# caomw/BundleAdjustmentMatlab

Hardware: AMD Instinct MI355X
Metric: LM iterations/sec + observations/sec, 1000-cam/500k-pt synthetic (higher is better)
Workload: dtype f64; 1 GPU; cfg3: 1000 cams x 500000 pts x 3000000 obs, fix_calibration (num_a=6), full LM pass per step, one linearisation per step; cameras=1000, points=500000, observations=3000000, parallelism=point-shard x1

## Files before the change

bundleadjustmentmatlab_amd/_lib.py:

```python
from __future__ import annotations

import ctypes
import os

_HERE = os.path.dirname(os.path.abspath(__file__))
LIB_PATH = os.environ.get("VLGBA_LIB") or os.path.join(_HERE, "libvlgba.so")

ABI_VERSION = 6

c_int, c_double, c_ll = ctypes.c_int, ctypes.c_double, ctypes.c_longlong
c_dp = ctypes.POINTER(ctypes.c_double)
c_ip = ctypes.POINTER(ctypes.c_int)
c_up = ctypes.POINTER(ctypes.c_ubyte)


class VlgbaProblem(ctypes.Structure):
    _fields_ = [("m", c_int), ("n", c_int), ("num_a", c_int), ("num_obs", c_ll),
                ("obs_pt", c_ip), ("obs_cam", c_ip), ("obs_x", c_dp), ("K", c_dp),
                ("num_vis", c_double), ("model", c_int)]


MODEL_EUCLIDEAN, MODEL_PROJECTIVE = 0, 1
LOSSES = {"none": 0, "huber": 1, "cauchy": 2}
JACOBIANS = {"fd": 0, "analytic": 1}
COV_METHODS = {"dense": 0, "selected": 1}


class VlgbaOptions(ctypes.Structure):
    _fields_ = [("fix_structure", c_int), ("fix_motion", c_int), ("pivot", c_up),
                ("verbose", c_int), ("max_iter", c_int), ("max_iter2", c_int),
                ("lambda0", c_double), ("device", c_int), ("rank", c_int),
                ("world_size", c_int), ("comm_id", ctypes.c_void_p), ("dense_solve", c_int),
                ("ordered", c_int), ("allreduce", ctypes.c_void_p),
                ("allreduce_user", ctypes.c_void_p), ("schur_kernel", c_int),
                ("semantics", c_int), ("stop_rel", c_double),
                ("on_pass", ctypes.c_void_p), ("on_pass_user", ctypes.c_void_p)]


NKERNELS = 18

ALLREDUCE_FN = ctypes.CFUNCTYPE(c_int, c_dp, c_ll, ctypes.c_void_p)


class VlgbaResectProblem(ctypes.Structure):
    _fields_ = [("nprob", c_int), ("num_a", c_int), ("obs_ptr", ctypes.POINTER(c_ll)),
                ("X", c_dp), ("x", c_dp), ("K", c_dp)]


class VlgbaStats(ctypes.Structure):
    _fields_ = [("iterations", c_int), ("accepted", c_int), ("num_error", c_int),
                ("lambda_", c_double), ("seconds", c_double), ("pinv_passes", c_int),
                ("spin_retries", c_int), ("nd_retries", c_int)]


class VlgbaStepInfo(ctypes.Structure):
    _fields_ = [("old_sse", c_double), ("new_sse", c_double), ("dpg", c_double),
                ("rho", c_double), ("lambda_", c_double), ("accepted", c_int),
                ("chol_failed", c_int), ("pinv", c_int), ("spin_retry", c_int),
                ("nd_retry", c_int)]


class VlgbaSceneSpec(ctypes.Structure):
    _fields_ = [("m", c_int), ("n", c_int), ("track", c_int), ("depth_lo", c_double),
                ("depth_hi", c_double), ("noise", c_double), ("seed", ctypes.c_ulonglong),
                ("keep_first_rotation", c_int), ("width", c_double), ("height", c_double)]


class VlgbaSceneOut(ctypes.Structure):
    _fields_ = [("K", c_dp), ("w", c_dp), ("T", c_dp), ("X", c_dp), ("w0", c_dp), ("T0", c_dp),
                ("X0", c_dp), ("obs_pt", c_ip), ("obs_cam", c_ip), ("obs_x", c_dp),
                ("num_obs_cap", c_ll), ("num_obs", c_ll), ("behind", c_ll)]


ON_PASS_FN = ctypes.CFUNCTYPE(None, c_int, c_int, ctypes.POINTER(VlgbaStepInfo), ctypes.c_void_p)


SIGNATURES = {
    "vlgba_solve": (c_int, [ctypes.POINTER(VlgbaProblem), ctypes.POINTER(VlgbaOptions), c_dp,
                            c_dp, c_dp, c_int, ctypes.POINTER(VlgbaStats)]),
    "vlgba_create": (c_int, [ctypes.POINTER(VlgbaProblem), ctypes.POINTER(VlgbaOptions),
                             ctypes.POINTER(ctypes.c_void_p)]),
    "vlgba_set_params": (c_int, [ctypes.c_void_p, c_dp, c_dp]),
    "vlgba_get_params": (c_int, [ctypes.c_void_p, c_dp, c_dp]),
    "vlgba_step": (c_int, [ctypes.c_void_p, c_int, c_int, ctypes.POINTER(VlgbaStepInfo)]),
    "vlgba_run": (c_int, [ctypes.c_void_p, c_dp, c_int, ctypes.POINTER(VlgbaStats)]),
    "vlgba_run_passes": (c_int, [ctypes.c_void_p, c_int, ctypes.POINTER(VlgbaStepInfo)]),
    "vlgba_get_step": (c_int, [ctypes.c_void_p, c_dp, c_dp]),
    "vlgba_get_reduced_system": (c_int, [ctypes.c_void_p, c_ip, c_dp, c_dp]),
    "vlgba_get_linearization": (c_int, [ctypes.c_void_p, c_dp, c_dp, c_dp, c_dp, c_dp]),
    "vlgba_covariance": (c_int, [ctypes.c_void_p, c_int, c_dp, c_dp, c_dp, c_dp]),
    "vlgba_set_loss": (c_int, [ctypes.c_void_p, c_int, c_double]),
    "vlgba_get_loss": (c_int, [ctypes.c_void_p, c_ip, c_dp]),
    "vlgba_set_covariance_method": (c_int, [ctypes.c_void_p, c_int]),
    "vlgba_get_covariance_method": (c_int, [ctypes.c_void_p, c_ip]),
    "vlgba_get_covariance_blocks": (c_int, [ctypes.c_void_p, c_ip, c_dp]),
    "vlgba_set_jacobian": (c_int, [ctypes.c_void_p, c_int]),
    "vlgba_get_jacobian": (c_int, [ctypes.c_void_p, c_ip]),
    "vlgba_get_residuals": (c_int, [ctypes.c_void_p, c_dp, c_dp, c_dp]),
    "vlgba_sync": (c_int, [ctypes.c_void_p]),
    "vlgba_destroy": (None, [ctypes.c_void_p]),
    "vlgba_set_timing": (c_int, [ctypes.c_void_p, c_int]),
    "vlgba_phase_ms": (c_int, [ctypes.c_void_p, c_dp]),
    "vlgba_kernel_ms": (c_int, [ctypes.c_void_p, c_dp, ctypes.POINTER(c_ll), c_int]),
    "vlgba_kernel_name": (ctypes.c_char_p, [c_int]),
    "vlgba_kernel_flops": (c_int, [ctypes.c_void_p, c_dp]),
    "vlgba_plan_info": (c_int, [ctypes.c_void_p, ctypes.POINTER(c_ll), c_int]),
    "vlgba_mex_bundle_1": (c_int, [c_int, c_int, c_int] + [c_dp] * 14),
    "vlgba_mex_bundle_2": (c_int, [c_int, c_int, c_int] + [c_dp] * 7),
    "vlgba_mex_bundle_3": (c_int, [c_int, c_int, c_int] + [c_dp] * 13),
    "vlgba_mex_bundle_proj_1": (c_int, [c_int, c_int] + [c_dp] * 13),
    "vlgba_mex_bundle_proj_2": (c_int, [c_int, c_int] + [c_dp] * 7),
    "vlgba_mex_bundle_proj_3": (c_int, [c_int, c_int] + [c_dp] * 12),
    "vlgba_resect": (c_int, [ctypes.POINTER(VlgbaResectProblem), ctypes.POINTER(VlgbaOptions),
                             c_dp, c_dp, c_int, c_ip, ctypes.POINTER(VlgbaStats)]),
    "vlgba_triangulate": (c_int, [c_int, c_dp, c_dp, c_dp, c_ll, ctypes.POINTER(c_ll), c_ip, c_dp,
                                  c_int, c_dp, c_ip]),
    "vlgba_intersect": (c_int, [c_int, c_dp, c_dp, c_dp, c_ll, ctypes.POINTER(c_ll), c_ip, c_dp,
                                ctypes.POINTER(VlgbaOptions), c_dp, c_dp, c_int, c_ip,
                                ctypes.POINTER(VlgbaStats)]),
    "vlgba_resect_ex": (c_int, [ctypes.POINTER(VlgbaResectProblem), ctypes.POINTER(VlgbaOptions),
                                c_int, c_int, c_double, c_dp, c_dp, c_int, c_ip, c_dp, c_dp,
                                ctypes.POINTER(VlgbaStats)]),
    "vlgba_intersect_ex": (c_int, [c_int, c_dp, c_dp, c_dp, c_dp, c_ll, ctypes.POINTER(c_ll), c_ip,
                                   c_dp, ctypes.POINTER(VlgbaOptions), c_int, c_int, c_double,
                                   c_dp, c_dp, c_int, c_ip, c_dp, c_dp,
                                   ctypes.POINTER(VlgbaStats)]),
    "vlgba_triangulate_ex": (c_int, [c_int, c_dp, c_dp, c_dp, c_dp, c_ll, ctypes.POINTER(c_ll),
                                     c_ip, c_dp, c_int, c_dp, c_ip]),
    "vlgba_scene_banded": (c_int, [ctypes.POINTER(VlgbaSceneSpec), c_int,
                                   ctypes.POINTER(VlgbaSceneOut)]),
    "vlgba_version": (c_int, [ctypes.c_char_p, c_int]),
    "vlgba_abi_check": (c_int, [c_int, c_ll, c_ll, c_ll, c_ll, c_ll]),
    "vlgba_get_unique_id": (c_int, [ctypes.c_void_p]),
    "vlgba_comm_release": (c_int, [ctypes.c_void_p]),
    "vlgba_device_count": (c_int, []),
    "vlgba_debug_sincos": (c_int, [c_dp, c_dp, c_dp, c_ll]),
    "vlgba_debug_pinv_solve": (c_int, [c_int, c_dp, c_dp, c_dp]),
    "vlgba_debug_force_status": (c_int, [ctypes.c_void_p, c_int, c_int]),
    "vlgba_debug_nd_plan": (c_int, [c_int, c_int, c_ip, c_int, c_ip, c_ip]),
    "vlgba_debug_selinv_plan": (c_int, [c_int, c_ip, c_ip, c_ip]),
    "vlgba_debug_pcg_plan": (c_int, [c_int, c_ip, c_int, c_ip, c_ip]),
    "vlgba_set_pcg": (c_int, [ctypes.c_void_p, c_double, c_int]),
    "vlgba_get_pcg": (c_int, [ctypes.c_void_p, c_dp, c_ip]),
    "vlgba_get_pcg_stats": (c_int, [ctypes.c_void_p, c_ip, c_dp, c_ip, ctypes.POINTER(c_ll)]),
}

ERRORS = {-1001: "bad argument",
          -1002: "num_a must be 6, 7, 9 or 10 (Euclidean) or 12 (projective)",
          -1003: "duplicate (point, camera) observation", -1004: "out of host memory",
          -1005: "RCCL communicator failure",
          -1006: "library / header ABI mismatch",
          -1007: "the undamped reduced camera system is not positive definite (gauge not fixed)"}

_lib = None


class VlgbaError(RuntimeError):
    pass


def lib():
    global _lib
    if _lib is None:
        if not os.path.exists(LIB_PATH):
            raise VlgbaError(f"{LIB_PATH} not built: run __graft_entry__.build() or "
                             "make -C bundleadjustmentmatlab_amd/csrc")
        L = ctypes.CDLL(LIB_PATH)
        for name, (res, args) in SIGNATURES.items():
            if os.environ.get("VLGBA_LIB") and not hasattr(L, name):
                continue
            fn = getattr(L, name)
            fn.restype = res
            fn.argtypes = args
        if hasattr(L, "vlgba_abi_check") or not os.environ.get("VLGBA_LIB"):
            rc = L.vlgba_abi_check(ABI_VERSION, *(ctypes.sizeof(s) for s in (
                VlgbaProblem, VlgbaOptions, VlgbaStats, VlgbaStepInfo, VlgbaResectProblem)))
            if rc != 0:
                raise VlgbaError(f"{LIB_PATH} does not match this binding (ABI {ABI_VERSION}): "
                                 "rebuild it with __graft_entry__.build()")
        _lib = L
    return _lib


def check(rc: int, what: str = "vlgba"):
    if rc != 0:
        msg = ERRORS.get(rc, f"HIP error {-rc}" if -1000 < rc < 0 else f"code {rc}")
        raise VlgbaError(f"{what} failed: {msg} ({rc})")
```

bundleadjustmentmatlab_amd/bundle.py:

```python
from __future__ import annotations

import ctypes
import numpy as np

from ._lib import (ALLREDUCE_FN, COV_METHODS, JACOBIANS, LOSSES, MODEL_EUCLIDEAN, MODEL_PROJECTIVE, NKERNELS, ON_PASS_FN,
                   VlgbaOptions,
                   VlgbaProblem, VlgbaResectProblem, VlgbaStats,
                   VlgbaStepInfo, c_dp, c_ip, c_up, check, lib)

__all__ = ["bundle_euclid", "bundle_euclid_nomex", "bundle_euclid_obs", "BundleAdjuster",
           "bundle_euclid_resect", "bundle_euclid_intersect", "triangulate_points",
           "parse_options", "pivot_mask",
           "mex_bundle_1_XABeUVWeAeB", "mex_bundle_2_Se_", "mex_bundle_3_db_new"]


def _F(a):
    return np.asfortranarray(a, dtype=np.float64)


def _dp(a):
    return a.ctypes.data_as(c_dp)


def pivot_mask(pivot, m):
# ... 269 lines not shown
            pass

    def __enter__(self):
        return self

    def __exit__(self, *exc):
        self.close()

    def set_params(self, a, b):
        a = np.ascontiguousarray(_F(a).reshape(-1, order="F"))
        b = np.ascontiguousarray(_F(b).reshape(-1, order="F"))
        assert a.size == self.num_a * self.m and b.size == 3 * self.n
        check(self._L.vlgba_set_params(self._h, _dp(a), _dp(b)), "vlgba_set_params")

    def get_params(self):
        a = np.zeros(self.num_a * self.m)
        b = np.zeros(3 * self.n)
        check(self._L.vlgba_get_params(self._h, _dp(a), _dp(b)), "vlgba_get_params")
        return a.reshape(self.num_a, self.m, order="F"), b.reshape(3, self.n, order="F")

    def force_status(self, word, passes=1):
        check(self._L.vlgba_debug_force_status(self._h, int(word), int(passes)),
              "vlgba_debug_force_status")

    def step(self, relinearize=True, update_lm=True):
        info = VlgbaStepInfo()
        check(self._L.vlgba_step(self._h, int(relinearize), int(update_lm), ctypes.byref(info)),
              "vlgba_step")
        return info

    def passes(self, n):
        info = VlgbaStepInfo()
        check(self._L.vlgba_run_passes(self._h, int(n), ctypes.byref(info)), "vlgba_run_passes")
        return info

    def run(self):
        err = np.zeros(self.max_iter + 1)
        st = VlgbaStats()
        check(self._L.vlgba_run(self._h, _dp(err), err.size, ctypes.byref(st)), "vlgba_run")
        assert st.num_error <= err.size
        return err[: st.num_error].copy(), st

    def last_step(self):
        da = np.zeros(self.num_a * self.m)
        db = np.zeros(3 * self.n)
        check(self._L.vlgba_get_step(self._h, _dp(da), _dp(db)), "vlgba_get_step")
        return da.reshape(self.num_a, self.m, order="F"), db.reshape(3, self.n, order="F")

    def reduced_system(self, dense=True):
        nb = self.plan_info()["blocks"]
        na = self.num_a
        jk = np.zeros(2 * nb, dtype=np.int32)
        blocks = np.zeros(na * na * nb)
        e_ = np.zeros(na * self.m)
        check(self._L.vlgba_get_reduced_system(self._h, jk.ctypes.data_as(c_ip), _dp(blocks),
                                               _dp(e_)), "vlgba_get_reduced_system")
        jk = jk.reshape(nb, 2)
        blocks = blocks.reshape(nb, na, na).transpose(0, 2, 1)
        if not dense:
            return jk, blocks, e_
        S = np.zeros((na * self.m, na * self.m))
        for (j, k), B in zip(jk, blocks):
            if j == k:
                S[na * j:na * j + na, na * k:na * k + na] = np.tril(B)
            else:
                S[na * j:na * j + na, na * k:na * k + na] = B
        return S, e_

    def set_covariance_method(self, method="dense"):
        if method not in COV_METHODS:
            raise ValueError(f"method must be one of {sorted(COV_METHODS)}")
        check(self._L.vlgba_set_covariance_method(self._h, COV_METHODS[method]),
              "vlgba_set_covariance_method")

    def get_covariance_method(self):
        kind = ctypes.c_int()
        check(self._L.vlgba_get_covariance_method(self._h, ctypes.byref(kind)),
              "vlgba_get_covariance_method")
        return {v: k for k, v in COV_METHODS.items()}[kind.value]

    def covariance(self, scale=True, full=False, method=None, blocks=False):
        if method is not None and method not in COV_METHODS:
            raise ValueError(f"method must be one of {sorted(COV_METHODS)}")
        prev = None
        if method is not None and method != self.get_covariance_method():
            prev = self.get_covariance_method()
            self.set_covariance_method(method)
        try:
            na, ld = self.num_a, self.num_a * self.m
            cam = np.zeros((na, na, self.m), order="F")
            pts = np.zeros((3, 3, self.n), order="F")
            S = np.zeros((ld, ld), order="F") if full else None
            info = np.zeros(8)
            check(self._L.vlgba_covariance(self._h, int(bool(scale)), _dp(cam),
                                           _dp(S) if full else None, _dp(pts), _dp(info)),
                  "vlgba_covariance")
            out = dict(cam=cam, pts=pts, sse=float(info[0]), dof=float(info[1]),
                       sigma2=float(info[2]), fixed_rows=int(info[3]),
                       ms=(float(info[4]), float(info[5])), scratch_bytes=int(info[6]))
            if full:
                out["full"] = S
            if blocks:
                nb = self.plan_info()["blocks"]
                jk = np.zeros(2 * nb, dtype=np.int32)
                blk = np.zeros(na * na * nb)
                check(self._L.vlgba_get_covariance_blocks(self._h, jk.ctypes.data_as(c_ip),
                                                          _dp(blk)),
                      "vlgba_get_covariance_blocks")
                out["blk_jk"] = jk.reshape(nb, 2)
                out["blocks"] = blk.reshape(nb, na, na).transpose(0, 2, 1)
            return out
        finally:
            if prev is not None:
                self.set_covariance_method(prev)

    def sync(self):
        check(self._L.vlgba_sync(self._h), "vlgba_sync")

    def linearization(self):
        na, m, n, N = self.num_a, self.m, self.n, self.num_obs
        U = np.zeros((na, na, m), order="F")
        eA = np.zeros((na, m), order="F")
        V = np.zeros((3, 3, n), order="F")
        eB = np.zeros((3, n), order="F")
        W = np.zeros((na, 3, N), order="F")
        check(self._L.vlgba_get_linearization(self._h, _dp(U), _dp(eA), _dp(V), _dp(eB),
                                              _dp(W)), "vlgba_get_linearization")
        return dict(U=U, eA=eA, V=V, eB=eB, W=W)

    def set_timing(self, on=True):
        check(self._L.vlgba_set_timing(self._h, int(on)), "vlgba_set_timing")

    def kernel_ms(self, reset=True):
        n = NKERNELS
        ms = np.zeros(n)
        calls = (ctypes.c_longlong * n)()
        check(self._L.vlgba_kernel_ms(self._h, _dp(ms), calls, int(reset)), "vlgba_kernel_ms")
        return {self._L.vlgba_kernel_name(k).decode(): (float(ms[k]), int(calls[k]))
                for k in range(n) if calls[k] > 0}

    PLAN_KEYS = ("obs", "points", "cameras", "num_a", "chunks", "chunk_slots",
                 "chunk_eslots", "groups", "group_slots", "group_eslots", "blocks",
                 "tiles", "cr_levels", "cr_elim", "cr_keep", "ordered", "schur_terms",
                 "blob_words", "mfma", "cr_rows", "mfma_groups", "reordered", "long_points",
                 "nd_arcs", "nd_sep_tiles", "solve_flops_factor", "solve_flops_syrk",
                 "solve_flops_back", "env_runner_runs", "vinv_fold", "camupd_fold", "pcg",
                 "solve_bytes")

    def plan_info(self):
        n = len(self.PLAN_KEYS)
        buf = (ctypes.c_longlong * n)()
        rc = self._L.vlgba_plan_info(self._h, buf, n)
        check(min(rc, 0), "vlgba_plan_info")
        return dict(zip(self.PLAN_KEYS, [int(v) for v in buf]))

    def phase_ms(self):
        ms = np.zeros(7)
        check(self._L.vlgba_phase_ms(self._h, _dp(ms)), "vlgba_phase_ms")
        return dict(zip(["linearize", "camera_reduce", "damp_y", "schur", "assemble",
                         "cholesky_solve", "update"], ms.tolist()))


def euclid_obs_adjuster(K, m, n, obs_pt, obs_cam, obs_x, *varargin, num_vis=0.0, device=0,
                        rank=0, world_size=1, comm_id=None, semantics="mex", loss="none",
                        loss_scale=0.0, jacobian=None, radial=False, **solver):
    o = parse_options(m, n, varargin, nomex=semantics == "nomex")
    if radial:
        o["num_variableK"] = RADIAL_NVK
    ba = BundleAdjuster(K, obs_pt, obs_cam, obs_x, n, 6 + o["num_variableK"],
                        fix_structure=o["fix_structure"], fix_motion=o["fix_motion"],
                        pivot=o["pivot"] if o["fix_pivot"] else None, verbose=o["verbose"],
                        num_vis=num_vis, device=device, rank=rank, world_size=world_size,
                        comm_id=comm_id, semantics=semantics, loss=loss, loss_scale=loss_scale,
                        jacobian=jacobian, **solver)
    ba.fingerprint = _adjuster_fingerprint(K, m, n, obs_pt, obs_cam, obs_x, o, num_vis,
                                           semantics, rank, world_size, device, comm_id,
                                           loss, loss_scale, ba.get_jacobian())
    return ba


def _adjuster_fingerprint(K, m, n, obs_pt, obs_cam, obs_x, o, num_vis, semantics, rank,
                          world_size, device, comm_id, loss="none", loss_scale=0.0,
                          jacobian="fd"):
    try:
        import xxhash
        h = xxhash.xxh3_128()
    except ImportError:
        import hashlib
        h = hashlib.blake2b(digest_size=16)
    for arr, dt in ((obs_pt, np.int32), (obs_cam, np.int32), (obs_x, np.float64),
                    (K, np.float64)):
        h.update(memoryview(np.ascontiguousarray(arr, dtype=dt)).cast("B"))
    piv = o["pivot"] if o["fix_pivot"] else None
    if piv is not None:
        h.update(np.asarray(piv, dtype=bool).tobytes())
    if comm_id is not None:
        h.update(bytes(comm_id))
    return (int(m), int(n), int(o["num_variableK"]), bool(o["fix_structure"]),
            bool(o["fix_motion"]), bool(o["fix_pivot"]), bool(o["verbose"]), float(num_vis),
            semantics, int(rank), int(world_size), int(device), comm_id is not None,
            h.hexdigest(), str(loss), float(loss_scale) if loss != "none" else 0.0,
            str(jacobian))


def bundle_euclid_obs(K, Te, w, Xe, obs_pt, obs_cam, obs_x, *varargin, num_vis=0.0, device=0,
                      rank=0, world_size=1, comm_id=None, return_stats=False,
                      semantics="mex", adjuster=None, return_covariance=False, loss="none",
                      loss_scale=0.0, jacobian=None, covariance_method=None, radial=None,
                      **solver):
    K, Te, w, Xe = _F(K), _F(Te), _F(w), _F(Xe)
    m, n = w.shape[1], Xe.shape[1]
    nomex = semantics == "nomex"
    o = parse_options(m, n, varargin, nomex=nomex)
    if radial is not None:
        if jacobian == "fd":
            raise ValueError("radial distortion has analytic Jacobians only")
        o["num_variableK"] = RADIAL_NVK
    nvk = o["num_variableK"]
    a = pack_a(K, Te, w, nvk, radial)
    b = _F(Xe[0:3])
    if adjuster is not None:
        if solver:
            raise ValueError("bundle_euclid_obs: solver options belong to the prebuilt adjuster")
        ba = adjuster.result() if hasattr(adjuster, "result") else adjuster
        want = _adjuster_fingerprint(K, m, n, obs_pt, obs_cam, obs_x, o, num_vis, semantics,
                                     rank, world_size, device, comm_id, loss, loss_scale,
                                     jacobian if jacobian is not None else
                                     ba.get_jacobian())
        if getattr(ba, "fingerprint", None) != want:
            ba.close()
            raise ValueError("bundle_euclid_obs: the prebuilt adjuster is for another problem "
                             "or other options (make it with euclid_obs_adjuster)")
    else:
        ba = euclid_obs_adjuster(K, m, n, obs_pt, obs_cam, obs_x, *varargin, num_vis=num_vis,
                                 device=device, rank=rank, world_size=world_size,
                                 comm_id=comm_id, semantics=semantics, loss=loss,
                                 loss_scale=loss_scale, jacobian=jacobian,
                                 radial=radial is not None, **solver)
    with ba:
        ba.set_params(a, b)
        err, st = ba.run()
        a, b = ba.get_params()
        if return_covariance:
            ba.set_params(a, b)
            cov = ba.covariance(scale=loss == "none", method=covariance_method)
    out = unpack(K, a, b, np.ones((1, n)) if nomex else Xe[3:4], nvk) + (err,)
    out = out + (st,) if return_stats else out
    out = out + (cov,) if return_covariance else out
    return out + (a[7:9].copy(order="F"),) if radial is not None else out


def bundle_euclid(K, Te, w, Xe, x, *varargin, device=0, return_stats=False, semantics="mex",
                  return_covariance=False, loss="none", loss_scale=0.0, covariance_method=None,
                  **solver):
    x = _F(x)
    m, n = np.shape(w)[1], x.shape[1]
    o = parse_options(m, n, varargin, x=x, nomex=semantics == "nomex")
    vis = o["visible"]
    num_vis = float(vis.sum())
    pt, cam = np.nonzero(vis)
    obs_x = np.stack([x[0, pt, cam], x[1, pt, cam]], axis=1)
    rest, k = [], 0
    while k < len(varargin):
        nm = varargin[k].lower() if isinstance(varargin[k], str) else varargin[k]
        if nm == "visibility":
            k += 2
            continue
        if nm == "fix_pivot":
            rest += [varargin[k], varargin[k + 1]]
            k += 2
            continue
        rest.append(varargin[k])
        k += 1
    return bundle_euclid_obs(K, Te, w, Xe, pt, cam, obs_x, *rest, num_vis=num_vis,
                             device=device, return_stats=return_stats, semantics=semantics,
                             return_covariance=return_covariance, loss=loss,
                             loss_scale=loss_scale, covariance_method=covariance_method,
                             **solver)


def bundle_euclid_nomex(K, Te, w, Xe, x, *varargin, device=0, return_stats=False,
                        return_covariance=False, loss="none", loss_scale=0.0,
                        covariance_method=None, **solver):
    return bundle_euclid(K, Te, w, Xe, x, *varargin, device=device,
                         return_stats=return_stats, semantics="nomex",
                         return_covariance=return_covariance, loss=loss,
                         loss_scale=loss_scale, covariance_method=covariance_method, **solver)


def _block_mode(radial, jacobian, loss, loss_scale, return_residuals):
    if jacobian is None:
        jacobian = "fd" if radial is None else "analytic"
    if jacobian not in JACOBIANS:
        raise ValueError(f"jacobian must be one of {sorted(JACOBIANS)}, got {jacobian!r}")
    if loss not in LOSSES:
        raise ValueError(f"loss must be one of {sorted(LOSSES)}, got {loss!r}")
    ex = radial is not None or jacobian != "fd" or loss != "none" or bool(return_residuals)
    return ex, JACOBIANS[jacobian], LOSSES[loss], float(loss_scale)


def _block_solve(name, head, head_ex, mode, x, count, N, residuals, return_stats, device,
                 max_iter, max_iter2, lambda0, stop_rel):
    ex, jac, lk, ls = mode
    cap = (max_iter if max_iter > 0 else 20) + 1
    err = np.zeros((count, cap))
    nerr = np.zeros(count, dtype=np.int32)
    opt = VlgbaOptions()
# ... 146 lines not shown
```

bundleadjustmentmatlab_amd/csrc/ba_internal.h:

```cpp
#pragma once
#include <hip/hip_runtime.h>
#include <cstddef>
#include <cstdint>
#include "ba_limits.h"

struct ba_chol;
struct ba_pcg;

#define VLGBA_CHECK(x)                                                              \
    do {                                                                            \
        hipError_t err__ = (x);                                                     \
        if (err__ != hipSuccess) return -(int)err__;                                \
    } while (0)

enum {
    KT_ROT, KT_LIN, KT_CAMRED, KT_DAMP, KT_SCHUR, KT_SCHUR_CHUNK, KT_SCHUR_RED,
    KT_ASSEMBLE, KT_FACTOR, KT_SYRK, KT_BACKWARD, KT_CAMUPD, KT_PTUPD, KT_CR_FACTOR,
    KT_CR_UPDATE, KT_CR_BACK, KT_SCHUR_MF, KT_LIN_UPD, KT_N
};
#define KT_MAX_EV 8192
struct ba_ktimer {
    int on;
    int nev;
    int ncreated;
    hipEvent_t ev[KT_MAX_EV];
    int kid[KT_MAX_EV / 2];
    double ms[KT_N];
    long long calls[KT_N];
    double flops[KT_N];
};
void kt_begin(struct ba_ktimer *t, hipStream_t s);
void kt_end(struct ba_ktimer *t, hipStream_t s, int kid);

#define BA_PROJ_NA 12
#define BA_RAD_NA 9

struct ba_flags {
    int fix_structure;
    int fix_motion;
    int has_pivot;
};

struct ba_loss {
    int kind;
    double c;
};

struct ba_camred {
    const int *cam_eptr, *cam_eslots;
    const double *upart;
    int m;
    ba_flags f;
    const unsigned char *pivot;
    double *U, *eA;
    const double *chsse;
    int nch;
    double *sse_out, *sse_out2;
};

struct ba_dev {
    int m, n, na, N, js;
    int device, ncu;
    int *obs_cam, *pt_ptr, *cam_ptr, *cam_obs;
    double *obs_x, *K4;
    unsigned char *pivot;
    double *a, *b, *a_new, *b_new;
    double *rot, *rot_new;
    double *jrec, *W, *U, *eA, *V, *eB;
    double *Vinv, *Y, *t, *db;
    int nb;
    long long T;
    int *blk_jk, *blk_ptr, *term;
    double *sblk, *rhs, *da;
    long long ld;
    long long lds;
    ba_chol *chol;
    ba_pcg *pcg;
    int dense_solve;
    int asm_direct;
    int camupd_fold;
    double *part;
    double *scal;
    int ordered;
    int parity;
    int mfma;
    int no_mfma;
    int loss_kind;
    double loss_scale;
    int jac;
    int ndb;
    int nch;
    int *ch_pt;
    int *ch_eslot;
    int *eslot_optr;
    unsigned short *eslot_obs;
    int *cam_eptr, *cam_eslots;
    double *spart;
    double *epart;
    double *upart;
    double *chsse;
    int fused;
    double *W2, *V2, *eB2, *upart2, *chsse2;
    int ns, nes;
    int ch_max_terms, ch_max_slots;
    long long nterm_fast;
    long long blob_words;
    int ngrp, ngs, nge;
    int grp_max_s, grp_max_e;
    unsigned *blob;
    int *ch_blob, *ch_obase;
    int *ch_cam;
    unsigned char *obs_lpt;
    int max_blob;
    int ngrp_mf;
    int vinv_fold;
    int nch_reg, nl, p_long;
    int *seg_pt, *seg_long;
    int *long_pt, *long_o0, *long_seg0;
    int *long_ebase;
    int *cam_lptr, *cam_lobs, *cam_ltrk;
    int max_lcam;
    int long_o0_h;
    double *ylong;
    int *lpair_ptr;
    int2 *lpair;
    int *lblk;
    int nlb;
    double *vseg;
    double *dpg_long;
    int mf_max_s, mf_max_e, mf_max_blob;
    int *grp_ch, *grp_gs, *grp_ge;
    unsigned short *cs_g, *ce_g;
    int *blk_gptr, *blk_gslots;
    int *cam_gptr, *cam_gslots;
    double *xh_out;
    double *B_out;
    unsigned char *obs_vis;
    int schur_owner;
    int dpg_lambda;
    struct ba_ktimer *kt;
    hipStream_t stream;
    hipStream_t side;
    hipEvent_t ev_fork, ev_join;
    volatile double *hres;
    double *hres_dev;
    unsigned long long seq;
    unsigned *pub_cnt;
};

#define KT_B(d) \
    do { if ((d)->kt && (d)->kt->on) kt_begin((d)->kt, (d)->stream); } while (0)
#define KT_E(d, id) \
    do { if ((d)->kt && (d)->kt->on) kt_end((d)->kt, (d)->stream, (id)); } while (0)

#define BA_PART_MAX 65536

#define BA_DISPATCH(NAEXPR, CALL)                                                   \
    switch (NAEXPR) {                                                               \
    case 6: { constexpr int NA = 6; CALL; } break;                                  \
    case 7: { constexpr int NA = 7; CALL; } break;                                  \
    case BA_RAD_NA: { constexpr int NA = BA_RAD_NA; CALL; } break;                  \
    case 10: { constexpr int NA = 10; CALL; } break;                                \
    case BA_PROJ_NA: { constexpr int NA = BA_PROJ_NA; CALL; } break;                \
    default: return -1000;                                                          \
    }

int ba_launch_rotations(ba_dev *d, const double *a, double *rot);
int ba_launch_linearize(ba_dev *d, ba_flags f);
ba_camred ba_camred_args(const ba_dev *d, ba_flags f);
int ba_launch_camera_reduce(ba_dev *d, ba_flags f, hipStream_t s);
int ba_launch_damp_point(ba_dev *d, double lambda);
int ba_launch_schur(ba_dev *d, double lambda);
int ba_launch_assemble(ba_dev *d);
int ba_launch_update(ba_dev *d, double lambda, ba_flags f, bool cam_updated, bool publish,
                     bool *published);
int ba_launch_yeb(ba_dev *d);
int ba_launch_obs_residuals(ba_dev *d, double *e, double *w, double *rho);
int ba_launch_publish(ba_dev *d);
void *ba_dmalloc(size_t bytes);
int ba_ensure_dyn_lds(const void *fn, size_t bytes);
void ba_dfree(void *p);
template <typename T>
inline int dalloc(T **p, size_t count)
{
    *p = (T *)ba_dmalloc(sizeof(T) * (count ? count : 1));
    return *p ? 0 : -(int)hipErrorOutOfMemory;
}
template <typename T>
inline int upload(T *dst, const T *src, size_t count, hipStream_t s)
{
    if (count == 0) return 0;
    return -(int)hipMemcpyAsync(dst, src, sizeof(T) * count, hipMemcpyHostToDevice, s);
}
template <typename T>
inline int download(T *dst, const T *src, size_t count, hipStream_t s)
{
    if (count == 0) return 0;
    return -(int)hipMemcpyAsync(dst, src, sizeof(T) * count, hipMemcpyDeviceToHost, s);
}
template <typename T>
class ba_dbuf {
    T *p_ = nullptr;

public:
    ba_dbuf() = default;
    ba_dbuf(ba_dbuf &&o) noexcept : p_(o.p_) { o.p_ = nullptr; }
    ba_dbuf &operator=(ba_dbuf &&o) noexcept
    {
        if (this != &o) {
            ba_dfree(p_);
            p_ = o.p_;
            o.p_ = nullptr;
        }
        return *this;
    }
    ba_dbuf(const ba_dbuf &) = delete;
    ba_dbuf &operator=(const ba_dbuf &) = delete;
    ~ba_dbuf() { ba_dfree(p_); }
    int alloc(size_t count)
    {
        ba_dfree(p_);
        return dalloc(&p_, count);
    }
    T *get() const { return p_; }
    operator T *() const { return p_; }
};
int ba_env_runner_timed_out(ba_dev *d);
int ba_launch_schur_fast(ba_dev *d, double lambda, const ba_camred *fold, bool side_camred);
int ba_launch_long_pairs(ba_dev *d, int fill, int *cnt);
int ba_launch_assemble_plain(ba_dev *d, double *S, long long ld, int lower_only);
int ba_launch_parity_old_sse(ba_dev *d);
int ba_launch_parity_new_sums(ba_dev *d, double lambda);
int ba_chol_setup(ba_dev *d, const int *blk_jk_host, int nb);
void ba_chol_free(ba_dev *d);
int ba_chol_prepare(ba_dev *d);
int ba_assemble_tiles(ba_dev *d);
int ba_fix_diag_plain(ba_dev *d, double *S, long long ld);
int ba_chol_fix_diag(ba_dev *d);
int ba_chol_solve(ba_dev *d, bool *cam_updated, int nospin = 0);
int ba_cr32_factor(ba_dev *d);
int ba_cr32_selinv_sources(const ba_dev *d, int *src);
int ba_cr32_selinv(ba_dev *d, const int *src, double *sig);
int ba_pinv_apply(ba_dev *d, const double *V, const double *ev, long long ld, const double *rhs,
                  double *work, double *da);

int ba_pcg_setup(ba_dev *d, const int *blk_jk_host, int nb);
void ba_pcg_free(ba_dev *d);
int ba_pcg_solve(ba_dev *d);

#define BA_COV_T8 8
#define BA_COV_T64 32
#define BA_COV_LDS 65536
int ba_cov_mark_fixed(ba_dev *d, const double *S, long long ld, unsigned char *fixed);
int ba_cov_finish(ba_dev *d, double *S, long long ld, const unsigned char *fixed, double *blocks);
struct ba_cov_src {
    const double *Sa;
    long long ld;
    const int *rowptr, *col;
    const double *packed;
};
int ba_cov_pack(ba_dev *d, const double *S, long long ld, const int *bj, const int *bk, int nb,
                double *packed);
int ba_cov_mark_fixed_blocks(ba_dev *d, unsigned char *fixed);
int ba_cov_extract(ba_dev *d, const double *sig, const unsigned char *fixed, const int *bj,
// ... 10 lines not shown
```

bundleadjustmentmatlab_amd/csrc/ba_kernels.hip:

```cpp
#include "ba_internal.h"
#include "ba_chol.h"
#include "ba_camera.h"
#include "vlg_math.h"
#include "../../include/vlgba.h"

typedef double d4 __attribute__((ext_vector_type(4)));

#ifdef BA_STAMPS
__device__ unsigned long long g_stamp[32];
#define STAMP_DECL unsigned long long st_prev_ = __builtin_amdgcn_s_memtime()
#define STAMP(i)                                                                    \
    do {                                                                            \
        if (threadIdx.x == 0) {                                                     \
            const unsigned long long t_ = __builtin_amdgcn_s_memtime();             \
            atomicAdd(&g_stamp[i], t_ - st_prev_);                                  \
            st_prev_ = t_;                                                          \
        }                                                                           \
    } while (0)
extern "C" int vlgba_debug_stamps(unsigned long long *out, int reset)
{
    if (hipMemcpyFromSymbol(out, HIP_SYMBOL(g_stamp), sizeof(g_stamp)) != hipSuccess) return -1;
    if (reset) {
        unsigned long long z[32] = {};
        if (hipMemcpyToSymbol(HIP_SYMBOL(g_stamp), z, sizeof(z)) != hipSuccess) return -1;
    }
    return 0;
}
#define BA_MFST_WG 4096
__device__ unsigned long long g_mfst[BA_MFST_WG * 4 * 8];
#define MF_CLK(v)                                                                   \
    do {                                                                            \
        __builtin_amdgcn_sched_barrier(0);                                          \
        v = __builtin_amdgcn_s_memtime();                                           \
        __builtin_amdgcn_sched_barrier(0);                                          \
    } while (0)
extern "C" int vlgba_debug_mf_stamps(unsigned long long *out, int nwords)
{
    const size_t nb = sizeof(unsigned long long) * (size_t)nwords;
    if (nb > sizeof(g_mfst)) return -1;
    if (hipMemcpyFromSymbol(out, HIP_SYMBOL(g_mfst), nb) != hipSuccess) return -1;
    return 0;
}
#else
#define STAMP_DECL
#define STAMP(i)
#define MF_CLK(v)
#endif

typedef double v2d __attribute__((ext_vector_type(2)));

template <int BS>
__device__ __forceinline__ void block_sum_to(double v, double *out)
{
    __shared__ double red[BS / 64];
#pragma unroll
    for (int off = 32; off > 0; off >>= 1) v += __shfl_down(v, off, 64);
    const int lane = threadIdx.x & 63, wid = threadIdx.x >> 6;
    if (lane == 0) red[wid] = v;
    __syncthreads();
    if (threadIdx.x == 0) {
        double s = red[0];
#pragma unroll
        for (int k = 1; k < BS / 64; k++) s += red[k];
        *out = s;
    }
}


__device__ __forceinline__ void fd_columns_6(const cam_view<6> &cv, const double b[3],
                                             const double xh[2], int half, double *row)
{
    const double *t0 = cv.a0 + 3;
#pragma unroll
    for (int t = 0; t < 3; t++) {
        const double *Rs = cv.R + 9 * (half ? 0 : 1 + t);
        double Rk[9], tt[3], bb[3], x1[2], S[3];
#pragma unroll
        for (int q = 0; q < 9; q++) Rk[q] = Rs[q];
#pragma unroll
        for (int c = 0; c < 3; c++) {
            tt[c] = half ? t0[c] : t0[c] + H_FD * 0.0;
            bb[c] = half ? b[c] + H_FD * ((c == t) ? 1.0 : 0.0) : b[c];
        }
        vlg_rot_b(Rk, bb, S);
        vlg_project_s(cv.Kc, S, tt, x1);
        const int col = half ? 6 + t : t;
        row[2 * col] = vlg_fd_quot(x1[0] - xh[0]);
        row[2 * col + 1] = vlg_fd_quot(x1[1] - xh[1]);
    }
    double S[3], R4[9];
    const double *Rs4 = cv.R + 36;
#pragma unroll
    for (int q = 0; q < 9; q++) R4[q] = Rs4[q];
    vlg_rot_b(R4, b, S);
#pragma unroll
    for (int u = 0; u < 2; u++) {
        const int k = 3 + 2 * u + half;
        if (k < 6) {
            double tt[3], x1[2];
#pragma unroll
            for (int c = 0; c < 3; c++) tt[c] = t0[c] + H_FD * ((3 + c == k) ? 1.0 : 0.0);
            vlg_project_s(cv.Kc, S, tt, x1);
            row[2 * k] = vlg_fd_quot(x1[0] - xh[0]);
            row[2 * k + 1] = vlg_fd_quot(x1[1] - xh[1]);
        }
    }
}

template <int NA>
__global__ void k_rotations(const double *__restrict__ a, double *__restrict__ rot, int m)
{
    const int j = blockIdx.x * blockDim.x + threadIdx.x;
    if (j >= m) return;
    const double *aj = a + (size_t)NA * j;
    const double w[3] = {aj[0], aj[1], aj[2]};
    rotations5(w, rot + 45 * (size_t)j);
}

template <int NA>
__global__ void k_rotations_jac(const double *__restrict__ a, double *__restrict__ rot, int m)
{
    const int j = blockIdx.x * blockDim.x + threadIdx.x;
    if (j >= m) return;
    const double *aj = a + (size_t)NA * j;
    const double w[3] = {aj[0], aj[1], aj[2]};
    rotations5_jac(w, rot + 45 * (size_t)j);
}

__global__ void k_sincos(const double *__restrict__ x, double *__restrict__ s,
                         double *__restrict__ c, long long n)
{
    const long long i = (long long)blockIdx.x * blockDim.x + threadIdx.x;
    if (i >= n) return;
    const double v = x[i];
    s[i] = vlg_lm_sin(v);
    c[i] = vlg_lm_cos(v);
}

extern "C" int vlgba_debug_sincos(const double *x, double *s, double *c, long long n)
{
    if (n < 0 || (n > 0 && (!x || !s || !c))) return VLGBA_E_ARG;
    if (n == 0) return 0;
    double *d = nullptr;
    VLGBA_CHECK(hipMalloc(&d, sizeof(double) * 3 * (size_t)n));
    int rc = 0;
    do {
        if (hipMemcpy(d, x, sizeof(double) * n, hipMemcpyHostToDevice) != hipSuccess) { rc = -1; break; }
        const long long nb = (n + 255) / 256;
        hipLaunchKernelGGL(k_sincos, dim3((unsigned)nb), dim3(256), 0, 0, d, d + n, d + 2 * n, n);
        if (hipGetLastError() != hipSuccess) { rc = -1; break; }
        if (hipMemcpy(s, d + n, sizeof(double) * n, hipMemcpyDeviceToHost) != hipSuccess ||
            hipMemcpy(c, d + 2 * n, sizeof(double) * n, hipMemcpyDeviceToHost) != hipSuccess)
            rc = -1;
    } while (0);
    (void)hipFree(d);
    return rc;
}

template <int NA>
__global__ __launch_bounds__(256) void k_linearize(
    const int *__restrict__ pt_ptr, const int *__restrict__ obs_cam,
    const double *__restrict__ obs_x, const double *__restrict__ K4,
    const double *__restrict__ a, const double *__restrict__ rot,
    const double *__restrict__ b, int n, ba_flags f, const unsigned char *__restrict__ pivot,
    double *__restrict__ jrec, double *__restrict__ W, double *__restrict__ V,
    double *__restrict__ eB, double *__restrict__ part_sse, double *__restrict__ xh_out,
    double *__restrict__ B_out)
{
    constexpr int JS = 2 * NA + 2;
    double sse = 0.0;
    for (int i = blockIdx.x * blockDim.x + threadIdx.x; i < n; i += gridDim.x * blockDim.x) {
        const double bi[3] = {b[3 * (size_t)i], b[3 * (size_t)i + 1], b[3 * (size_t)i + 2]};
        double v[9], eb[3];
#pragma unroll
        for (int q = 0; q < 9; q++) v[q] = 0.0;
        eb[0] = eb[1] = eb[2] = 0.0;
        const int o_end = pt_ptr[i + 1];
        for (int o = pt_ptr[i]; o < o_end; o++) {
            const int j = obs_cam[o];
            cam_view<NA> cv(a, K4, rot, j);
            double xh[2];
            cv.project(bi, xh);
            double A[2 * NA], B[6];
#pragma unroll
            for (int k = 0; k < NA; k++) {
                double x1[2];
                cv.project_dcam(k, bi, x1);
                A[2 * k] = vlg_fd_quot(x1[0] - xh[0]);
                A[2 * k + 1] = vlg_fd_quot(x1[1] - xh[1]);
            }
#pragma unroll
            for (int k = 0; k < 3; k++) {
                double b1[3], x1[2];
#pragma unroll
                for (int c = 0; c < 3; c++) b1[c] = bi[c] + H_FD * ((c == k) ? 1.0 : 0.0);
                cv.project(b1, x1);
                B[2 * k] = vlg_fd_quot(x1[0] - xh[0]);
                B[2 * k + 1] = vlg_fd_quot(x1[1] - xh[1]);
            }
            const double e0 = obs_x[2 * (size_t)o] - xh[0];
            const double e1 = obs_x[2 * (size_t)o + 1] - xh[1];
            double *rec = jrec + (size_t)JS * o;
#pragma unroll
            for (int q = 0; q < 2 * NA; q += 2) {
                double2 p = {A[q], A[q + 1]};
                *reinterpret_cast<double2 *>(rec + q) = p;
            }
            *reinterpret_cast<double2 *>(rec + 2 * NA) = double2{e0, e1};
            if (xh_out) {
                xh_out[2 * (size_t)o] = xh[0];
                xh_out[2 * (size_t)o + 1] = xh[1];
            }
            if (B_out) {
#pragma unroll
                for (int q = 0; q < 6; q++) B_out[6 * (size_t)o + q] = B[q];
            }
            const bool wzero = f.fix_structure || f.fix_motion || (f.has_pivot && pivot[j]);
            double *wo = W + (size_t)3 * NA * o;
#pragma unroll
            for (int c = 0; c < 3; c++)
#pragma unroll
                for (int r = 0; r < NA; r++)
                    wo[r + NA * c] =
                        wzero ? 0.0 : 0.0 + (A[2 * r] * B[2 * c] + A[2 * r + 1] * B[2 * c + 1]);
#pragma unroll
            for (int c = 0; c < 3; c++)
#pragma unroll
                for (int r = 0; r < 3; r++)
                    v[r + 3 * c] += B[2 * r] * B[2 * c] + B[2 * r + 1] * B[2 * c + 1];
#pragma unroll
            for (int r = 0; r < 3; r++) eb[r] += B[2 * r] * e0 + B[2 * r + 1] * e1;
            sse += e0 * e0 + e1 * e1;
        }
        if (f.fix_structure) {
#pragma unroll
            for (int q = 0; q < 9; q++) v[q] = 0.0;
            eb[0] = eb[1] = eb[2] = 0.0;
        }
#pragma unroll
        for (int q = 0; q < 9; q++) V[9 * (size_t)i + q] = v[q];
#pragma unroll
        for (int q = 0; q < 3; q++) eB[3 * (size_t)i + q] = eb[q];
    }
    block_sum_to<256>(sse, part_sse + blockIdx.x);
}

#define BA_LIN_CAMS 10
#define BA_LIN_WAVES (BA_LIN_CAMS > 0 ? 6 : 7)

struct ba_upd {
    const double *W_old, *da, *eB_old, *Vinv, *b_old;
    int ndb;
    double lambda;
    double *db, *b_new, *part_dpg;
    const int *seg_long, *long_o0;
    const double *dpg_long;
};

template <int NA, bool UPD, bool LOSS, bool JAC = false>
__device__ __forceinline__ void linearize_chunk_body(
    const int *__restrict__ ch_pt, const int *__restrict__ ch_obase,
    const int *__restrict__ ch_eslot, const int *__restrict__ eslot_optr,
    const unsigned short *__restrict__ eslot_obs, const int *__restrict__ pt_ptr,
    const int *__restrict__ obs_cam, const unsigned char *__restrict__ obs_lpt,
    const double *__restrict__ obs_x, const double *__restrict__ K4,
    const double *__restrict__ a, const double *__restrict__ rot,
    const double *__restrict__ b, ba_flags f, const unsigned char *__restrict__ pivot,
    double *__restrict__ W, double *__restrict__ V, double *__restrict__ eB,
    double *__restrict__ upart, double *__restrict__ part_sse, int nch_reg,
    const int *__restrict__ seg_pt, double *__restrict__ vseg, const int *__restrict__ ch_cam,
    ba_upd u, int ch, ba_loss ls)
{
    constexpr int NC0 = (NA + 4) / 2;
    static_assert(!LOSS || 2 * BA_CH_OBS >= 256, "one lane pair per LDS row");
    constexpr int RS = 2 * NA + 8;
    constexpr int NU = NA * (NA + 1) / 2;
    static_assert(BA_CH_OBS + 1 <= 256 && BA_CH_PTS + 1 <= 256, "one metadata word per lane");
    constexpr int LW = BA_CH_OBS * 3 * NA;
    constexpr int NROWS = (UPD && LW + 3 * BA_CH_PTS > BA_CH_OBS * RS) ? LW + 3 * BA_CH_PTS
                                                                        : BA_CH_OBS * RS;
    static_assert(NA != 6 || NROWS == BA_CH_OBS * RS, "fused update must not grow NA = 6 LDS");
    __shared__ __attribute__((aligned(16))) double rows[NROWS];
    __shared__ int lptr_raw[64 * (BA_CH_PTS / 64 + 1)];
    __shared__ int eoff_raw[64 * (BA_CH_OBS / 64 + 1)];
    __shared__ unsigned short eobl[BA_CH_OBS];
    __shared__ unsigned char wz[BA_CH_OBS];
    __shared__ double dpl[UPD ? BA_CH_PTS : 1];
    static_assert(BA_CH_PTS <= 64, "the point lanes are wave 0");
    constexpr int NCAMS = (NA == 6 && BA_LIN_CAMS > 0) ? BA_LIN_CAMS : 0;
    __shared__ __attribute__((aligned(16))) double camr[NCAMS > 0 ? 45 * NCAMS : 1];
    const int tid = threadIdx.x;
    const bool seg = ch >= nch_reg;
    const int p0 = seg ? seg_pt[ch - nch_reg] : ch_pt[ch];
    const int np = seg ? 1 : ch_pt[ch + 1] - p0;
    const int obase = ch_obase[ch], nobs = ch_obase[ch + 1] - obase;
    const int e0 = ch_eslot[ch], nes = ch_eslot[ch + 1] - e0;
    STAMP_DECL;
    const int u0 = eslot_optr[e0], nu = eslot_optr[e0 + nes] - u0;
    {
        const int wv = tid >> 6;
        if (wv <= (nes >> 6))
            __builtin_amdgcn_global_load_lds(eslot_optr + e0 + min(tid, nes), eoff_raw + 64 * wv,
                                             4, 0, 0);
        if (!seg && wv <= (np >> 6))
            __builtin_amdgcn_global_load_lds(pt_ptr + p0 + min(tid, np), lptr_raw + 64 * wv, 4, 0,
                                             0);
    }
    const int cam_lo = ch_cam[2 * ch], cam_n = ch_cam[2 * ch + 1] - cam_lo + 1;
    const bool camst = NCAMS > 0 && nobs > 0 && cam_n <= NCAMS;
    if (NCAMS > 0 && camst) {
#if defined(__HIP_DEVICE_COMPILE__)
        const int lane = tid & 63;
        auto stage = [&](const double *src, int ndw, double *dst) {
            const char *s8 = reinterpret_cast<const char *>(src);
            for (int q = tid >> 6; 64 * q < ndw; q += 4)
                if (64 * q + lane < ndw)
                    __builtin_amdgcn_global_load_lds(s8 + 4 * (64 * q + lane),
                                                     reinterpret_cast<int *>(dst) + 64 * q, 4, 0,
                                                     0);
        };
        stage(rot + 45 * (size_t)cam_lo, 90 * cam_n, &camr[0]);
#endif
        if constexpr (!UPD) __syncthreads();
    }
    int m_eobl = 0;
    STAMP(16);
    double bu[3] = {0.0, 0.0, 0.0};
    if constexpr (UPD) {
        if (seg) {
            if (tid == 0)
                dpl[0] = obase == u.long_o0[u.seg_long[ch - nch_reg]]
                             ? __hip_atomic_load(u.dpg_long + u.seg_long[ch - nch_reg],
                                                 __ATOMIC_RELAXED, __HIP_MEMORY_SCOPE_AGENT)
                             : 0.0;
        } else {
            const int ne = nobs * 3 * NA;
            const double *wsrc = u.W_old + (size_t)3 * NA * obase;
            double dl[NA];
            const int ocam = nobs > 0 ? obs_cam[obase + min(tid, nobs - 1)] : 0;
            const int clo = cam_lo, span = cam_n;
            const bool dstage = NA == 6 && span * NA <= NROWS - LW;
            if (dstage && nobs > 0) {
#if defined(__HIP_DEVICE_COMPILE__)
                const int nb = 8 * NA * span;
                if ((tid >> 6) < ((nb + 1023) >> 10))
                    __builtin_amdgcn_global_load_lds(
                        reinterpret_cast<const char *>(u.da + (size_t)NA * clo) +
                            min((tid >> 6) * 1024 + 16 * (tid & 63), nb - 16),
                        &rows[LW + 128 * (tid >> 6)], 16, 0, 0);
#endif
            }
            if (nobs > 0) {
                if constexpr (NA == 6) {
#if defined(__HIP_DEVICE_COMPILE__)
                    const int nbytes = 8 * ne, ninst = (nbytes + 1023) >> 10;
                    const char *src = reinterpret_cast<const char *>(wsrc);
                    for (int q = tid >> 6; q < ninst; q += 4)
                        __builtin_amdgcn_global_load_lds(
                            src + min(q * 1024 + 16 * (tid & 63), nbytes - 16), &rows[128 * q],
                            16, 0, 2);
#endif
                } else {
                    constexpr int MAXE = (LW + 255) / 256;
#pragma unroll
                    for (int q = 0; q < MAXE; q++) {
                        const int e = tid + 256 * q;
                        if (e < ne) rows[e] = __builtin_nontemporal_load(wsrc + e);
                    }
                }
                if (!dstage) {
                    const double *dd = u.da + (size_t)NA * ocam;
#pragma unroll
                    for (int k = 0; k < NA; k++) dl[k] = dd[k];
                }
            }
            const int ip = np > 0 ? p0 + min(tid, np - 1) : 0;
            double pe[3] = {0.0, 0.0, 0.0}, pv[9] = {}, pb[3] = {0.0, 0.0, 0.0};
            if (__builtin_amdgcn_readfirstlane(tid >> 6) == 0) {
#pragma unroll
                for (int r = 0; r < 3; r++) pe[r] = u.eB_old[3 * (size_t)ip + r];
#pragma unroll
                for (int r = 0; r < 9; r++) pv[r] = u.Vinv[9 * (size_t)ip + r];
#pragma unroll
                for (int r = 0; r < 3; r++) pb[r] = u.b_old[3 * (size_t)ip + r];
            }
            __syncthreads();
            if (tid < nobs) {
                double *wo = rows + 3 * NA * tid;
                if (dstage) {
#pragma unroll
                    for (int k = 0; k < NA; k++) dl[k] = rows[LW + NA * (ocam - clo) + k];
                }
#pragma unroll
                for (int k = 0; k < NA; k++)
                    if (k >= u.ndb) dl[k] = 0.0;
#pragma unroll
                for (int r = 0; r < 3; r++) {
                    double *w = wo + NA * r;
                    double t = w[0] * dl[0] + w[1] * dl[1] + w[2] * dl[2] + w[3] * dl[3] +
                               w[4] * dl[4] + w[5] * dl[5];
#pragma unroll
                    for (int k = 6; k < NA; k++)
                        if (k < u.ndb) t = t + w[k] * dl[k];
                    w[0] = t;
                }
            }
            __syncthreads();
            if (tid < np) {
                const int i = p0 + tid;
                double rhs[3] = {pe[0], pe[1], pe[2]};
                const int lo1 = lptr_raw[tid + 1] - obase;
                for (int lo = lptr_raw[tid] - obase; lo < lo1; lo++) {
#pragma unroll
                    for (int r = 0; r < 3; r++) rhs[r] -= rows[3 * NA * lo + NA * r];
                }
                double dpg = 0.0;
#pragma unroll
                for (int r = 0; r < 3; r++) {
                    const double dbr = pv[r] * rhs[0] + pv[r + 3] * rhs[1] + pv[r + 6] * rhs[2];
                    const double bnr = pb[r] + dbr;
                    u.db[3 * (size_t)i + r] = dbr;
                    u.b_new[3 * (size_t)i + r] = bnr;
                    rows[LW + 3 * tid + r] = bnr;
                    dpg += dbr * (u.lambda * dbr + pe[r]);
                }
                dpl[tid] = dpg;
            }
        }
        __syncthreads();
        if (!seg && nobs > 0) {
            const int lp = obs_lpt[obase + min(min(tid >> 1, BA_CH_OBS - 1), nobs - 1)];
#pragma unroll
            for (int c = 0; c < 3; c++) bu[c] = rows[LW + 3 * lp + c];
        } else if (nobs > 0) {
#pragma unroll
            for (int c = 0; c < 3; c++) bu[c] = b[3 * (size_t)p0 + c];
        }
        __syncthreads();
        STAMP(23);
    }
    double sse = 0.0;
    if (nobs > 0) {
        m_eobl = __hip_atomic_load(eslot_obs + u0 + min(tid, nu - 1), __ATOMIC_RELAXED,
                                   __HIP_MEMORY_SCOPE_WORKGROUP);
        const int lo = min(tid >> 1, BA_CH_OBS - 1), half = tid & 1;
        const bool live = (tid >> 1) < nobs;
        {
            const int o = obase + min(lo, nobs - 1);
            const int j = obs_cam[o], i = p0 + obs_lpt[o];
            double bi[3];
#pragma unroll
            for (int c = 0; c < 3; c++) bi[c] = UPD ? bu[c] : b[3 * (size_t)i + c];
            double xh[2];
            double *row = rows + RS * lo;
            if constexpr (JAC && NA == 6) {
                auto proj6 = [&](const double *rt, int jr) {
                    cam_view<NA> cv6(a, K4, rt, jr, j);
                    cv6.project(bi, xh);
                    cv6.jac_columns(bi, half, row);
                };
                if (NCAMS > 0 && camst)
                    proj6(&camr[0], j - cam_lo);
                else
                    proj6(rot, j);
            } else if constexpr (JAC) {
                cam_view<NA> cv(a, K4, rot, j);
                cv.project(bi, xh);
                cv.jac_columns(bi, half, row);
            } else if constexpr (NA == 6) {
                auto proj6 = [&](const double *rt, int jr) {
                    cam_view<NA> cv6(a, K4, rt, jr, j);
                    cv6.project(bi, xh);
                    fd_columns_6(cv6, bi, xh, half, row);
                };
                if (NCAMS > 0 && camst)
                    proj6(&camr[0], j - cam_lo);
                else
                    proj6(rot, j);
            } else {
                cam_view<NA> cv(a, K4, rot, j);
                cv.project(bi, xh);
#pragma unroll 1
                for (int t = 0; t < NC0; t++) {
                    const int col = half ? NC0 + t : t;
                    if (col < NA + 3) {
                        double x1[2];
                        cv.project_col(col, bi, x1);
                        row[2 * col] = vlg_fd_quot(x1[0] - xh[0]);
                        row[2 * col + 1] = vlg_fd_quot(x1[1] - xh[1]);
                    }
                }
            }
            if constexpr (LOSS) {
                const double e0 = obs_x[2 * (size_t)o] - xh[0];
                const double e1 = obs_x[2 * (size_t)o + 1] - xh[1];
                double rho, sw;
                vlg_loss(ls.kind, ls.c, e0 * e0 + e1 * e1, &rho, &sw);
#pragma unroll
                for (int col = 0; col < NA + 3; col++) {
                    const bool lane1 = JAC      ? cam_view<NA>::jac_lane1(col)
                                       : NA == 6 ? (col == 4 || col > 5)
                                                 : col >= NC0;
                    if (lane1 == (half != 0)) {
                        row[2 * col] *= sw;
                        row[2 * col + 1] *= sw;
                    }
                }
                if (!half) {
                    row[2 * NA + 6] = e0 * sw;
                    row[2 * NA + 7] = e1 * sw;
                    if (live) sse = rho;
                    wz[lo] = f.fix_structure || f.fix_motion || (f.has_pivot && pivot[j]);
                }
            } else if (!half) {
                const double e0 = obs_x[2 * (size_t)o] - xh[0];
                const double e1 = obs_x[2 * (size_t)o + 1] - xh[1];
                row[2 * NA + 6] = e0;
                row[2 * NA + 7] = e1;
                if (live) sse = e0 * e0 + e1 * e1;
                wz[lo] = f.fix_structure || f.fix_motion || (f.has_pivot && pivot[j]);
            }
        }
    }
    if (tid < nu) eobl[tid] = (unsigned short)m_eobl;
    __syncthreads();
    STAMP(17);
    if constexpr (UPD) {
        if (tid == 0) {
            double acc = 0.0;
            const int k1 = seg ? 1 : np;
            for (int k = 0; k < k1; k++) acc += dpl[k];
            u.part_dpg[ch] = acc;
        }
    }
    if constexpr (NA % 2 == 0) {
        double2 *wdst = reinterpret_cast<double2 *>(W + (size_t)3 * NA * obase);
        constexpr int NP = 3 * NA / 2;
        for (int q = tid; q < nobs * NP; q += 256) {
            const int lo = q / NP, e = q - NP * lo, c = e / (NA / 2), r = 2 * (e - (NA / 2) * c);
            const double *row = rows + RS * lo;
            const double2 a0 = *reinterpret_cast<const double2 *>(row + 2 * r);
            const double2 a1 = *reinterpret_cast<const double2 *>(row + 2 * r + 2);
            const double2 bc = *reinterpret_cast<const double2 *>(row + 2 * NA + 2 * c);
            const long long keep = wz[lo] ? 0 : -1;
            const double v0 = 0.0 + (a0.x * bc.x + a0.y * bc.y);
            const double v1 = 0.0 + (a1.x * bc.x + a1.y * bc.y);
            const v2d w2 = {__builtin_bit_cast(double, __builtin_bit_cast(long long, v0) & keep),
                            __builtin_bit_cast(double, __builtin_bit_cast(long long, v1) & keep)};
            __builtin_nontemporal_store(w2, reinterpret_cast<v2d *>(wdst) + q);
        }
    } else {
        double *wdst = W + (size_t)3 * NA * obase;
        for (int q = tid; q < nobs * 3 * NA; q += 256) {
            const int lo = q / (3 * NA), e = q - 3 * NA * lo, c = e / NA, r = e - NA * c;
            const double *row = rows + RS * lo;
            const double2 ar = *reinterpret_cast<const double2 *>(row + 2 * r);
            const double2 bc = *reinterpret_cast<const double2 *>(row + 2 * NA + 2 * c);
            wdst[q] = wz[lo] ? 0.0 : 0.0 + (ar.x * bc.x + ar.y * bc.y);
        }
    }
    STAMP(18);
    for (int q = tid; q < np * 12; q += 256) {
        const int pl = q / 12, e = q % 12, i = p0 + pl;
        const int lo0 = seg ? 0 : lptr_raw[pl] - obase;
        const int lo1 = seg ? nobs : lptr_raw[pl + 1] - obase;
        const int r = (e < 9) ? e % 3 : e - 9, c = (e < 9) ? e / 3 : 3;
        double acc = 0.0;
        for (int lo = lo0; lo < lo1; lo++) {
            const double *B = rows + RS * lo + 2 * NA;
            acc += B[2 * r] * B[2 * c] + B[2 * r + 1] * B[2 * c + 1];
        }
        if (f.fix_structure) acc = 0.0;
        if (seg) vseg[12 * (size_t)(ch - nch_reg) + e] = acc;
        else if (e < 9) V[9 * (size_t)i + e] = acc;
        else eB[3 * (size_t)i + e - 9] = acc;
    }
    STAMP(19);
    for (int q = tid; q < nes * (NU + NA); q += 256) {
        const int s = q / (NU + NA), l = q % (NU + NA);
        int r, c;
        if (l < NU) {
            int t = l;
            c = 0;
            while (t >= NA - c) { t -= NA - c; c++; }
            r = c + t;
        } else {
            r = l - NU;
            c = NA;
        }
        const int cc = (c < NA) ? 2 * c : 2 * NA + 6;
        double acc = 0.0;
        int u = eoff_raw[s] - u0;
        const int u1 = eoff_raw[s + 1] - u0;
        for (; u + 3 < u1; u += 4) {
            double p[4];
#pragma unroll
            for (int k = 0; k < 4; k++) {
                const double *rw = rows + RS * eobl[u + k];
                p[k] = rw[2 * r] * rw[cc] + rw[2 * r + 1] * rw[cc + 1];
            }
#pragma unroll
            for (int k = 0; k < 4; k++) acc += p[k];
        }
        for (; u < u1; u++) {
            const double *row = rows + RS * eobl[u];
            acc += row[2 * r] * row[cc] + row[2 * r + 1] * row[cc + 1];
        }
        upart[(size_t)(NU + NA) * (e0 + s) + l] = acc;
    }
    STAMP(20);
    block_sum_to<256>(sse, part_sse + ch);
    STAMP(21);
#ifdef BA_STAMPS
    if (tid == 0) atomicAdd(&g_stamp[22], 1ull);
#endif
}

#define BA_LIN_ARGS                                                                        \
    const int *__restrict__ ch_pt, const int *__restrict__ ch_obase,                       \
        const int *__restrict__ ch_eslot, const int *__restrict__ eslot_optr,              \
        const unsigned short *__restrict__ eslot_obs, const int *__restrict__ pt_ptr,      \
        const int *__restrict__ obs_cam, const unsigned char *__restrict__ obs_lpt,        \
        const double *__restrict__ obs_x, const double *__restrict__ K4,                   \
        const double *__restrict__ a, const double *__restrict__ rot,                      \
        const double *__restrict__ b, ba_flags f, const unsigned char *__restrict__ pivot, \
        double *__restrict__ W, double *__restrict__ V, double *__restrict__ eB,           \
        double *__restrict__ upart, double *__restrict__ part_sse, int nch_reg,            \
        const int *__restrict__ seg_pt, double *__restrict__ vseg,                         \
        const int *__restrict__ ch_cam
#define BA_LIN_PASS                                                                        \
    ch_pt, ch_obase, ch_eslot, eslot_optr, eslot_obs, pt_ptr, obs_cam, obs_lpt, obs_x, K4, a, \
        rot, b, f, pivot, W, V, eB, upart, part_sse, nch_reg, seg_pt, vseg, ch_cam

template <int NA>
__global__ __launch_bounds__(256, (NA == 6) ? BA_LIN_WAVES : 1) void k_linearize_chunk(BA_LIN_ARGS)
{
    linearize_chunk_body<NA, false, false>(BA_LIN_PASS, ba_upd{}, blockIdx.x, ba_loss{});
}

template <int NA>
__global__ __launch_bounds__(256, (NA == 6) ? BA_LIN_WAVES : 1) void k_linearize_chunk_loss(
    BA_LIN_ARGS, ba_loss ls)
{
    linearize_chunk_body<NA, false, true>(BA_LIN_PASS, ba_upd{}, blockIdx.x, ls);
}

template <int NA>
__global__ __launch_bounds__(256, (NA == 6) ? BA_LIN_WAVES : 1) void k_update_linearize(BA_LIN_ARGS,
                                                                             ba_upd u)
{
    linearize_chunk_body<NA, true, false>(BA_LIN_PASS, u, blockIdx.x, ba_loss{});
}

template <int NA>
__global__ __launch_bounds__(256, (NA == 6) ? BA_LIN_WAVES : 1) void k_update_linearize_loss(
    BA_LIN_ARGS, ba_upd u, ba_loss ls)
{
    linearize_chunk_body<NA, true, true>(BA_LIN_PASS, u, blockIdx.x, ls);
}

template <int NA, bool LOSS>
__global__ __launch_bounds__(256, (NA == 6) ? BA_LIN_WAVES : 1) void k_linearize_chunk_jac(
    BA_LIN_ARGS, ba_loss ls)
{
    linearize_chunk_body<NA, false, LOSS, true>(BA_LIN_PASS, ba_upd{}, blockIdx.x, ls);
}

template <int NA, bool LOSS>
__global__ __launch_bounds__(256, (NA == 6) ? BA_LIN_WAVES : 1) void k_update_linearize_jac(
    BA_LIN_ARGS, ba_upd u, ba_loss ls)
{
    linearize_chunk_body<NA, true, LOSS, true>(BA_LIN_PASS, u, blockIdx.x, ls);
}

template <int NA>
__device__ __forceinline__ void camera_reduce_wg(int j, const ba_camred &a)
{
    const int *__restrict__ cam_eptr = a.cam_eptr;
    const int *__restrict__ cam_eslots = a.cam_eslots;
    const double *__restrict__ upart = a.upart;
    const int m = a.m, nch = a.nch;
    const ba_flags f = a.f;
    const unsigned char *__restrict__ pivot = a.pivot;
    double *__restrict__ U = a.U;
    double *__restrict__ eA = a.eA;
    const double *__restrict__ chsse = a.chsse;
    double *__restrict__ sse_out = a.sse_out;
    double *__restrict__ sse_out2 = a.sse_out2;
    constexpr int NU = NA * (NA + 1) / 2;
    constexpr int NT = NU + NA;
    constexpr int P = 256 / NT;
    __shared__ double part[P][NT];
    const int tid = threadIdx.x;
    if (j == m) {
        double v[8] = {0.0, 0.0, 0.0, 0.0, 0.0, 0.0, 0.0, 0.0};
        int q = tid;
        for (; q + 7 * 256 < nch; q += 8 * 256) {
#pragma unroll
            for (int u = 0; u < 8; u++) v[u] += chsse[q + 256 * u];
        }
        for (; q < nch; q += 256) v[0] += chsse[q];
        block_sum_to<256>(((v[0] + v[1]) + (v[2] + v[3])) + ((v[4] + v[5]) + (v[6] + v[7])),
                          sse_out);
        if (tid == 0) sse_out2[0] = sse_out[0];
        return;
    }
    const int l = tid % NT, p = tid / NT;
    if (p < P) {
        const int q0 = cam_eptr[j], q1 = cam_eptr[j + 1];
        double acc = 0.0;
        int q = q0 + p;
        for (; q + 3 * P < q1; q += 4 * P) {
            int ix[4];
            double v[4];
#pragma unroll
            for (int k = 0; k < 4; k++) ix[k] = cam_eslots[q + k * P];
#pragma unroll
            for (int k = 0; k < 4; k++) v[k] = upart[(size_t)NT * ix[k] + l];
#pragma unroll
            for (int k = 0; k < 4; k++) acc += v[k];
        }
        for (; q < q1; q += P) acc += upart[(size_t)NT * cam_eslots[q] + l];
        part[p][l] = acc;
    }
    __syncthreads();
    if (tid >= NT) return;
    double acc = 0.0;
#pragma unroll
    for (int k = 0; k < P; k++) acc += part[k][tid];
    if (f.fix_motion || (f.has_pivot && pivot[j])) acc = 0.0;
    if (tid < NU) {
        int t = tid, c = 0;
        while (t >= NA - c) { t -= NA - c; c++; }
        const int r = c + t;
        U[(size_t)NA * NA * j + r + NA * c] = acc;
        U[(size_t)NA * NA * j + c + NA * r] = acc;
    } else {
        eA[(size_t)NA * j + tid - NU] = acc;
    }
}

template <int NA>
__global__ __launch_bounds__(256) void k_camera_reduce_chunks(ba_camred a)
{
    camera_reduce_wg<NA>(blockIdx.x, a);
}

template <int NA>
__global__ void k_camera_reduce(const int *__restrict__ cam_ptr, const int *__restrict__ cam_obs,
                                const double *__restrict__ jrec, int m, ba_flags f,
                                const unsigned char *__restrict__ pivot, double *__restrict__ U,
                                double *__restrict__ eA)
{
    constexpr int JS = 2 * NA + 2;
    constexpr int NU = NA * (NA + 1) / 2;
    const int j = blockIdx.x;
    const int l = threadIdx.x;
    if (j >= m || l >= NU + NA) return;
    int r, c;
    if (l < NU) {
        int q = l;
        c = 0;
        while (q >= NA - c) { q -= NA - c; c++; }
        r = c + q;
// ... 235 lines not shown
#pragma unroll
            for (int c = 0; c < 3; c++)
                y[NA * c] = fma(w2, vi[2 + 3 * c], fma(w1, vi[1 + 3 * c], w0 * vi[3 * c]));
        }
        __syncthreads();
        STAMP(2);
        for (int q = tid; q < ns * IT * 2; q += 256) {
            const int par = q & 1, qq = q >> 1;
            const int s = qq / IT, rh = (qq % IT) / NCP, c0c = 2 * (qq % NCP);
            const int r0 = rh * NR, nr = (rh == 0) ? NR : NA - NR;
            const bool two = c0c + 1 < NA;
            const int c1c = two ? c0c + 1 : c0c;
            double acc0[NR], acc1[NR];
#pragma unroll
            for (int r = 0; r < NR; r++) acc0[r] = acc1[r] = 0.0;
            const int u1 = (int)soff[s + 1];
            for (int u = (int)soff[s] + par; u < u1; u += 2) {
                const unsigned tw = terml[u];
                const double *y = Yl + WS * (tw & 0xffffu) + r0;
                const double *w = Wl + WS * (tw >> 16);
                const double wa0 = w[c0c], wa1 = w[c0c + NA], wa2 = w[c0c + 2 * NA];
                const double wb0 = w[c1c], wb1 = w[c1c + NA], wb2 = w[c1c + 2 * NA];
#pragma unroll
                for (int r = 0; r < NR; r++) {
                    if (r < nr) {
                        const double y0 = y[r], y1 = y[r + NA], y2 = y[r + 2 * NA];
                        acc0[r] = fma(y2, wa2, fma(y1, wa1, fma(y0, wa0, acc0[r])));
                        acc1[r] = fma(y2, wb2, fma(y1, wb1, fma(y0, wb0, acc1[r])));
                    }
                }
            }
#pragma unroll
            for (int r = 0; r < NR; r++) {
                acc0[r] += __shfl_xor(acc0[r], 1, 64);
                acc1[r] += __shfl_xor(acc1[r], 1, 64);
            }
            if (par) continue;
            double *dst = direct ? spart + (size_t)NA * NA * (gs0 + s)
                                 : gacc + NA * NA * sgl[s];
#pragma unroll
            for (int r = 0; r < NR; r++) {
                if (r < nr) {
                    double *d0 = dst + (r0 + r) + NA * c0c;
                    *d0 = direct ? acc0[r] : *d0 + acc0[r];
                    if (two) {
                        double *d1 = dst + (r0 + r) + NA * (c0c + 1);
                        *d1 = direct ? acc1[r] : *d1 + acc1[r];
                    }
                }
            }
        }
        for (int q = 255 - tid; q < nes * NA; q += 256) {
            const int s = q / NA, r = q % NA;
            double acc = 0.0;
            const int u1 = (int)eoff[s + 1];
            for (int u = (int)eoff[s]; u < u1; u++) {
                const int lo = (int)eobl[u];
                const double *y = Yl + WS * lo;
                const double *eb = El + 3 * lpt[lo];
                acc = fma(y[r + 2 * NA], eb[2], fma(y[r + NA], eb[1], fma(y[r], eb[0], acc)));
            }
            if (direct) epart[(size_t)NA * (ge0 + s) + r] = acc;
            else geacc[NA * egl[s] + r] += acc;
        }
        STAMP(3);
        __syncthreads();
        STAMP(4);
    }
    if (!direct) {
        for (int q = tid; q < ngs * NA * NA; q += 256) spart[(size_t)NA * NA * gs0 + q] = gacc[q];
        for (int q = tid; q < nge * NA; q += 256) epart[(size_t)NA * ge0 + q] = geacc[q];
    }
    STAMP(5);
    if (tid == 0) {
#ifdef BA_STAMPS
        atomicAdd(&g_stamp[6], (unsigned long long)nc);
        atomicAdd(&g_stamp[7], 1ull);
#endif
    }
}

typedef __attribute__((address_space(3))) double lds_double;
__device__ __forceinline__ void point_vinv_range(const double *V, double *Vinv, int p0, int p1,
                                                 double lambda, lds_double *stage)
{
    const int tid = threadIdx.x;
    double t[9];
    auto rows = [&](int i0) {
        const int cnt = 9 * min(256, p1 - i0);
        const double *src = V + 9 * (size_t)i0;
#pragma unroll
        for (int u = 0; u < 9; u++) t[u] = tid + 256 * u < cnt ? src[tid + 256 * u] : 0.0;
    };
    if (p0 < p1) rows(p0);
    for (int i0 = p0; i0 < p1; i0 += 256) {
        const int cnt = 9 * min(256, p1 - i0);
#pragma unroll
        for (int u = 0; u < 9; u++) stage[tid + 256 * u] = t[u];
        __syncthreads();
        if (i0 + 256 < p1) rows(i0 + 256);
        if (i0 + tid < p1) {
            double vs[9], vi[9];
#pragma unroll
            for (int q = 0; q < 9; q++) vs[q] = stage[9 * tid + q];
#pragma unroll
            for (int c = 0; c < 3; c++) vs[4 * c] = (1 + lambda) * vs[4 * c];
            vlg_pinv3(vs, vi);
#pragma unroll
            for (int q = 0; q < 9; q++) stage[9 * tid + q] = vi[q];
        }
        __syncthreads();
        double *dst = Vinv + 9 * (size_t)i0;
#pragma unroll
        for (int u = 0; u < 9; u++)
            if (tid + 256 * u < cnt) dst[tid + 256 * u] = stage[tid + 256 * u];
        __syncthreads();
    }
}

template <int NA>
__global__ __launch_bounds__(256) void k_point_vinv(const double *__restrict__ V, int n,
                                                    double lambda, double *__restrict__ Vinv)
{
    __shared__ double vsh[256 * 9];
    const int i0 = blockIdx.x * 256;
    point_vinv_range(V, Vinv, i0, min(i0 + 256, n), lambda, (lds_double *)vsh);
}

#define BA_MF_KB 5
template <int RG> __device__ __forceinline__ double row4_bcast_c(double v)
{
    constexpr int pat = 0x13 | ((RG << 2) << 5);
    const long long u = __builtin_bit_cast(long long, v);
    const int lo = __builtin_amdgcn_ds_swizzle((int)(u & 0xffffffffLL), pat);
    const int hi = __builtin_amdgcn_ds_swizzle((int)(u >> 32), pat);
    return __builtin_bit_cast(double, ((long long)hi << 32) | (unsigned int)lo);
}
__device__ __forceinline__ double row4_bcast(double v, int rg)
{
    switch (rg) {
    case 0: return row4_bcast_c<0>(v);
    case 1: return row4_bcast_c<1>(v);
    case 2: return row4_bcast_c<2>(v);
    default: return row4_bcast_c<3>(v);
    }
}
template <int Q> __device__ __forceinline__ double row16_bcast_c(double v)
{
    const long long u = __builtin_bit_cast(long long, v);
    const long long r = __builtin_amdgcn_mov_dpp(u, 0x150 + Q, 0xf, 0xf, true);
    return __builtin_bit_cast(double, r);
}
#define BA_MF_WAVES 3
template <int NA>
__global__ __launch_bounds__(256, (NA == 6) ? BA_MF_WAVES : 1) void k_schur_mfma(
    const int *__restrict__ grp_ch, const int *__restrict__ grp_gs,
    const int *__restrict__ grp_ge, const int *__restrict__ ch_pt,
    const int *__restrict__ ch_obase, const int *__restrict__ ch_blob,
    const unsigned *__restrict__ blob, const double *__restrict__ W,
    double *Vinv, const double *__restrict__ eB, int nobs_all, int n_all,
    int gcap, int ecap, double *__restrict__ spart, double *__restrict__ epart, int ngrp,
    ba_camred cred, const double *__restrict__ Vdamp, double lambda)
{
    if ((int)blockIdx.x >= ngrp) {
        camera_reduce_wg<NA>((int)blockIdx.x - ngrp, cred);
        return;
    }
    constexpr int WS = 3 * NA;
    constexpr int RT = BA_MF_RT(NA);
    constexpr int NTL = RT * (RT + 1) / 2;
    extern __shared__ __attribute__((aligned(16))) double sm[];
    double *gacc = sm;
    double *geacc = gacc + gcap * NA * NA;
    unsigned *rec = (unsigned *)(geacc + ecap * NA);
    __shared__ int4 chd[BA_GROUP_CH + 1];
    const int g = ngrp - 1 - (int)blockIdx.x;
    const int tid = threadIdx.x, lane = tid & 63, wv = tid >> 6;
    const int li = lane & 15, lk = lane >> 4;
    const int c0 = grp_ch[g], nc = grp_ch[g + 1] - c0;
    const int gs0 = grp_gs[g], ngs = grp_gs[g + 1] - gs0;
    const int ge0 = grp_ge[g], nge = grp_ge[g + 1] - ge0;
    const int rb0 = ch_blob[c0], nrw = ch_blob[c0 + nc] - rb0;
    if (Vdamp) {
        point_vinv_range(Vdamp, Vinv, ch_pt[c0], ch_pt[c0 + nc], lambda, (lds_double *)sm);
    }
    for (int q = tid; q < ngs * NA * NA; q += 256) gacc[q] = 0.0;
    for (int q = tid; q < nge * NA; q += 256) geacc[q] = 0.0;
    for (int q = tid; q < nrw; q += 256) rec[q] = blob[rb0 + q];
    for (int q = tid; q <= nc; q += 256) {
        const int i0 = ch_pt[c0 + q], bo = ch_blob[c0 + q] - rb0;
        const int np = q < nc ? ch_pt[c0 + q + 1] - i0 : 0;
        chd[q] = int4{i0, ch_obase[c0 + q], bo, np << 16};
    }
    __syncthreads();
    for (int q = tid; q < nc; q += 256) {
        const unsigned *r = rec + chd[q].z;
        const unsigned h1 = r[1];
        const int C = (int)(h1 & 0xffu), np = chd[q].w >> 16;
        unsigned bad = np == BA_MF_PTS ? 0u : 1u;
        if (!bad) {
            const unsigned *tw = r + 2 + C + C * (C + 1) / 2;
            for (int c = 0; c < C; c++)
#pragma unroll
                for (int w = BA_MF_PTS / 4 * c; w < BA_MF_PTS / 4 * (c + 1); w++)
                    bad |= tw[w] ^ (0x03020100u + 0x04040404u * (unsigned)w);
        }
        chd[q].w |= (int)(h1 & 0xffffu) | (bad ? 0 : 1 << 24);
    }
    __syncthreads();
    int ccs[RT], crr[RT];
#pragma unroll
    for (int t = 0; t < RT; t++) {
        ccs[t] = (16 * t + li) / NA;
        crr[t] = (16 * t + li) % NA;
    }
    auto load = [&](int i0, int ob, int bo, unsigned hw, double (&wf)[4][RT], double &vg,
                    double &v4) {
        const int C = (int)(hw & 0xffu), np = (int)((hw >> 16) & 0xffu);
        const double *wbase = W + (size_t)WS * ob;
        const double *vbase = Vinv + 9 * (size_t)i0;
        const double *ebase = eB + 3 * (size_t)i0;
        const int wz = WS * (nobs_all - ob), vz = 9 * (n_all - i0), ez = 3 * (n_all - i0);
        const int pA = BA_MF_KB * wv + lk, p4 = BA_MF_KB * wv + 4;
        const bool pvA = pA < np, pv4 = lk < 3 && p4 < np;
        const int vo = li + (li >= 3 ? 1 : 0) + (li >= 5 ? 2 : 0);
        const double *src = li < 6   ? vbase + (pvA ? 9 * pA + vo : vz)
                            : li < 9 ? ebase + (pvA ? 3 * pA + li - 6 : ez)
                                     : ebase + (pv4 ? 3 * p4 + lk : ez);
        vg = *src;
        const bool dv = p4 < np && li < 3 && lk < 3;
        v4 = vbase[dv ? 9 * p4 + lk + 3 * li : vz];
        int oA[RT], o4[RT];
        if (hw >> 24) {
#pragma unroll
            for (int t = 0; t < RT; t++) {
                const bool cv = ccs[t] < C;
                oA[t] = (cv ? WS * (pA * C + ccs[t]) : wz) + crr[t];
                o4[t] = (cv && lk < 3 ? WS * (p4 * C + ccs[t]) + NA * lk : wz) + crr[t];
            }
        } else {
            const unsigned *r = rec + bo;
            const unsigned char *tab = (const unsigned char *)(r + 2 + C + C * (C + 1) / 2);
#pragma unroll
            for (int t = 0; t < RT; t++) {
                const bool cvA = pvA && ccs[t] < C, cv4 = pv4 && ccs[t] < C;
                const int iA = tab[cvA ? pA * C + ccs[t] : 0];
                const int i4 = tab[cv4 ? p4 * C + ccs[t] : 0];
                oA[t] = (cvA && iA != 0xff ? WS * iA : wz) + crr[t];
                o4[t] = (cv4 && i4 != 0xff ? WS * i4 + NA * lk : wz) + crr[t];
            }
        }
#pragma unroll
        for (int t = 0; t < RT; t++) {
#pragma unroll
            for (int s = 0; s < 3; s++) wf[s][t] = wbase[oA[t] + NA * s];
            wf[3][t] = wbase[o4[t]];
        }
    };
    d4 accS[NTL];
    double eacc[RT];
#pragma unroll
    for (int u = 0; u < NTL; u++) accS[u] = d4{0.0, 0.0, 0.0, 0.0};
#pragma unroll
    for (int t = 0; t < RT; t++) eacc[t] = 0.0;
#ifdef BA_STAMPS
    unsigned long long st_ph[4] = {0, 0, 0, 0}, st_fm[3] = {0, 0, 0}, st_t0, st_t1, st_t2, st_t3;
#endif
    auto process = [&](int bo, unsigned hw, const double (&wc)[4][RT], double vg, double v4) {
        const double vc[6] = {row16_bcast_c<0>(vg), row16_bcast_c<1>(vg), row16_bcast_c<2>(vg),
                              row16_bcast_c<3>(vg), row16_bcast_c<4>(vg), row16_bcast_c<5>(vg)};
        const double ec[4] = {row16_bcast_c<6>(vg), row16_bcast_c<7>(vg), row16_bcast_c<8>(vg),
                              row16_bcast_c<9>(vg)};
        const unsigned *r = rec + bo;
        const int C = (int)(hw & 0xffu), fl = (int)((hw >> 8) & 0xffu), Rc = NA * C;
        double y4[RT];
        const double va = row4_bcast(v4, 0);
        MF_CLK(st_t2);
#pragma unroll
        for (int ti = 0; ti < RT; ti++)
            y4[ti] = __builtin_amdgcn_mfma_f64_4x4x4f64(va, wc[3][ti], 0.0, 0, 0, 0);
#pragma unroll
        for (int ti = 0; ti < RT; ti++) {
            {
                double y[4];
                y[3] = y4[ti];
                y[0] = fma(wc[2][ti], vc[2], fma(wc[1][ti], vc[1], wc[0][ti] * vc[0]));
                y[1] = fma(wc[2][ti], vc[4], fma(wc[1][ti], vc[3], wc[0][ti] * vc[1]));
                y[2] = fma(wc[2][ti], vc[5], fma(wc[1][ti], vc[4], wc[0][ti] * vc[2]));
                eacc[ti] = fma(y[3], ec[3], fma(y[2], ec[2], fma(y[1], ec[1],
                                                                 fma(y[0], ec[0], eacc[ti]))));
                if (NA == 6 && ti == RT - 1) {
#pragma unroll
                    for (int rg = 0; rg < 4; rg++) {
                        if (16 * ti + 4 * rg >= Rc) continue;
                        double ya[4];
#pragma unroll
                        for (int s = 0; s < 4; s++) ya[s] = row4_bcast(y[s], rg);
                        __builtin_amdgcn_sched_barrier(0);
#pragma unroll
                        for (int s = 0; s < 4; s++) {
#pragma unroll
                            for (int tj = 0; tj <= ti; tj++) {
                                d4 &t = accS[ti * (ti + 1) / 2 + tj];
                                t[rg] = __builtin_amdgcn_mfma_f64_4x4x4f64(ya[s], wc[s][tj], t[rg],
                                                                           0, 0, 0);
                            }
                        }
                    }
                } else {
#pragma unroll
                    for (int s = 0; s < 4; s++) {
#pragma unroll
                        for (int tj = 0; tj <= ti; tj++)
                            accS[ti * (ti + 1) / 2 + tj] = __builtin_amdgcn_mfma_f64_16x16x4f64(
                                y[s], wc[s][tj], accS[ti * (ti + 1) / 2 + tj], 0, 0, 0);
                    }
                }
            }
        }
        MF_CLK(st_t3);
        if (fl & 2) {
            const unsigned *ge = r + 2;
            const unsigned *pair = ge + C;
            double ecol[RT];
#pragma unroll
            for (int t = 0; t < RT; t++) {
                const double v0 = __shfl(eacc[t], li, 64), v1 = __shfl(eacc[t], li + 16, 64);
                const double v2 = __shfl(eacc[t], li + 32, 64), v3 = __shfl(eacc[t], li + 48, 64);
                ecol[t] = ((v0 + v1) + v2) + v3;
                eacc[t] = 0.0;
            }
            int fi = li, fk = lk;
            asm volatile("" : "+v"(fi), "+v"(fk));
            lds_double *gp[NTL][4], *ep[RT];
            unsigned gm[(4 * NTL + 31) / 32] = {};
#pragma unroll
            for (int ti = 0; ti < RT; ti++)
#pragma unroll
                for (int tj = 0; tj <= ti; tj++) {
                    const int col = 16 * tj + fi;
#pragma unroll
                    for (int q = 0; q < 4; q++) {
                        const int u = ti * (ti + 1) / 2 + tj;
                        const int rr = 16 * ti + fk + 4 * q;
                        const bool in = rr < Rc && col < Rc && rr >= col;
                        const int cr = rr / NA, cc = col / NA;
                        const unsigned gsl = pair[in ? cr * (cr + 1) / 2 + cc : 0];
                        const bool ok = in && gsl != 0xffffffffu;
                        gp[u][q] = (lds_double *)gacc +
                                   (ok ? (int)gsl * (NA * NA) + (rr - NA * cr) + NA * (col - NA * cc)
                                       : 0);
                        gm[(4 * u + q) >> 5] |= ok ? 1u << ((4 * u + q) & 31) : 0u;
                    }
                }
#pragma unroll
            for (int t = 0; t < RT; t++) {
                const int col = 16 * t + fi;
                const bool ok = fk == 0 && col < Rc;
                const int cs = col / NA;
                const unsigned gel = ge[ok ? cs : 0];
                ep[t] = (lds_double *)geacc + (ok ? (int)gel * NA + col - NA * cs : 0);
            }
// ... 634 lines not shown
        }
    }
    block_sum_to<256>(sse, part_sse + ch);
    __syncthreads();
    block_sum_to<256>(dpg, part_dpg + ch);
}

template <int NA>
__global__ __launch_bounds__(256) void k_point_update_chunk(BA_PUC_ARGS)
{
    point_update_chunk_body<NA, false>(BA_PUC_PASS, ba_loss{});
}

template <int NA>
__global__ __launch_bounds__(256) void k_point_update_chunk_loss(BA_PUC_ARGS, ba_loss ls)
{
    point_update_chunk_body<NA, true>(BA_PUC_PASS, ls);
}

template <int NA>
__global__ __launch_bounds__(256) void k_obs_residuals(
    const int *__restrict__ pt_ptr, const int *__restrict__ obs_cam,
    const double *__restrict__ obs_x, const double *__restrict__ K4,
    const double *__restrict__ a, const double *__restrict__ rot,
    const double *__restrict__ b, int n, int N, ba_loss ls, double *__restrict__ e,
    double *__restrict__ w, double *__restrict__ rho)
{
    const int o = blockIdx.x * 256 + threadIdx.x;
    if (o >= N) return;
    int i = 0, hi = n;
    while (hi - i > 1) {
        const int mid = i + ((hi - i) >> 1);
        if (pt_ptr[mid] <= o) i = mid;
        else hi = mid;
    }
    const int j = obs_cam[o];
    double bi[3], xh[2];
#pragma unroll
    for (int c = 0; c < 3; c++) bi[c] = b[3 * (size_t)i + c];
    cam_view<NA> cv(a, K4, rot, j);
    cv.project(bi, xh);
    const double e0 = obs_x[2 * (size_t)o] - xh[0];
    const double e1 = obs_x[2 * (size_t)o + 1] - xh[1];
    double r, sw;
    vlg_loss(ls.kind, ls.c, e0 * e0 + e1 * e1, &r, &sw);
    if (e) {
        e[2 * (size_t)o] = e0;
        e[2 * (size_t)o + 1] = e1;
    }
    if (w) w[o] = sw * sw;
    if (rho) rho[o] = r;
}

__global__ void k_long_vsum(const int *__restrict__ long_pt, const int *__restrict__ long_seg0,
                            const double *__restrict__ vseg, double *__restrict__ V,
                            double *__restrict__ eB)
{
    const int l = blockIdx.x, e = threadIdx.x;
    if (e >= 12) return;
    const int i = long_pt[l];
    double acc = 0.0;
    for (int sg = long_seg0[l]; sg < long_seg0[l + 1]; sg++) acc += vseg[12 * (size_t)sg + e];
    if (e < 9) V[9 * (size_t)i + e] = acc;
    else eB[3 * (size_t)i + e - 9] = acc;
}

template <int NA>
__global__ __launch_bounds__(256) void k_long_y(const int *__restrict__ long_pt,
                                                const int *__restrict__ long_o0,
                                                const int *__restrict__ long_ebase,
                                                const double *__restrict__ W,
                                                const double *__restrict__ Vinv,
                                                const double *__restrict__ eB,
                                                double *__restrict__ ylong,
                                                double *__restrict__ epart)
{
    constexpr int WS = 3 * NA;
    const int tid = threadIdx.x, l = blockIdx.x;
    const int i = long_pt[l], o0 = long_o0[l], k = long_o0[l + 1] - o0, L0 = long_o0[0];
    double vi[9], eb[3];
#pragma unroll
    for (int q = 0; q < 9; q++) vi[q] = Vinv[9 * (size_t)i + q];
#pragma unroll
    for (int q = 0; q < 3; q++) eb[q] = eB[3 * (size_t)i + q];
    for (int q = tid; q < k * WS; q += 256) {
        const int lo = q / WS, e = q - WS * lo, r = e % NA, c = e / NA;
        const double *w = W + (size_t)WS * (o0 + lo);
        ylong[(size_t)WS * (o0 - L0 + lo) + e] =
            w[r] * vi[3 * c] + w[r + NA] * vi[1 + 3 * c] + w[r + 2 * NA] * vi[2 + 3 * c];
    }
    const long long eb0 = long_ebase[l];
    for (int q = tid; q < k * NA; q += 256) {
        const int al = q / NA, r = q - NA * al;
        const double *w = W + (size_t)WS * (o0 + al);
        double y[3];
#pragma unroll
        for (int c = 0; c < 3; c++)
            y[c] = w[r] * vi[3 * c] + w[r + NA] * vi[1 + 3 * c] + w[r + 2 * NA] * vi[2 + 3 * c];
        epart[(size_t)NA * (eb0 + al) + r] = y[0] * eb[0] + y[1] * eb[1] + y[2] * eb[2];
    }
}

template <int NA>
__global__ __launch_bounds__(256) void k_long_db(
    const int *__restrict__ long_pt, const int *__restrict__ long_o0,
    const int *__restrict__ obs_cam, const double *__restrict__ W,
    const double *__restrict__ da, const double *__restrict__ eB,
    const double *__restrict__ Vinv, const double *__restrict__ b, int ndb, double lambda,
    double *__restrict__ db, double *__restrict__ b_new, double *__restrict__ dpg_long)
{
    __shared__ double red[3][256];
    const int l = blockIdx.x, tid = threadIdx.x;
    const int i = long_pt[l], o0 = long_o0[l], o1 = long_o0[l + 1];
    double t[3] = {0.0, 0.0, 0.0};
    for (int o = o0 + tid; o < o1; o += 256) {
        const double *d = da + (size_t)NA * obs_cam[o];
        double dl[NA];
#pragma unroll
        for (int kk = 0; kk < NA; kk++) dl[kk] = kk < ndb ? d[kk] : 0.0;
#pragma unroll
        for (int r = 0; r < 3; r++) {
            const double *w = W + (size_t)3 * NA * o + NA * r;
            double v = w[0] * dl[0] + w[1] * dl[1] + w[2] * dl[2] + w[3] * dl[3] + w[4] * dl[4] +
                       w[5] * dl[5];
#pragma unroll
            for (int kk = 6; kk < NA; kk++)
                if (kk < ndb) v = v + w[kk] * dl[kk];
            t[r] += v;
        }
    }
#pragma unroll
    for (int r = 0; r < 3; r++) red[r][tid] = t[r];
    __syncthreads();
    for (int h = 128; h > 0; h >>= 1) {
        if (tid < h)
            for (int r = 0; r < 3; r++) red[r][tid] += red[r][tid + h];
        __syncthreads();
    }
    if (tid == 0) {
        const double rhs[3] = {eB[3 * (size_t)i] - red[0][0], eB[3 * (size_t)i + 1] - red[1][0],
                               eB[3 * (size_t)i + 2] - red[2][0]};
        const double *vi = Vinv + 9 * (size_t)i;
        double dpg = 0.0;
        for (int r = 0; r < 3; r++) {
            const double dbr = vi[r] * rhs[0] + vi[r + 3] * rhs[1] + vi[r + 6] * rhs[2];
            db[3 * (size_t)i + r] = dbr;
            b_new[3 * (size_t)i + r] = b[3 * (size_t)i + r] + dbr;
            dpg += dbr * (lambda * dbr + eB[3 * (size_t)i + r]);
        }
        dpg_long[l] = dpg;
    }
}

struct ba_sum3 {
    const double *part[3];
    int n[3];
    double *out[3];
    const double *scal;
    double *hres;
    double seq;
    unsigned *cnt;
    const double *cam_da, *cam_eA;
    double *cam_part;
    int cam_m, cam_na;
    double cam_lambda;
};

__global__ __launch_bounds__(1024) void k_sum_parts3(ba_sum3 a)
{
    const double *part = a.part[blockIdx.x];
    const int nparts = a.n[blockIdx.x];
    if (blockIdx.x == 2 && a.cam_da) {
        const int lane = threadIdx.x & 63;
        for (int g = threadIdx.x >> 6; g < nparts; g += 16) {
            const int j = 64 * g + lane;
            double acc = 0.0;
            if (j < a.cam_m) {
                for (int c = 0; c < a.cam_na; c++) {
                    const double d = a.cam_da[(size_t)a.cam_na * j + c];
                    acc += d * (a.cam_lambda * d + a.cam_eA[(size_t)a.cam_na * j + c]);
                }
            }
#pragma unroll
            for (int off = 32; off > 0; off >>= 1) acc += __shfl_down(acc, off, 64);
            if (lane == 0) a.cam_part[g] = acc;
        }
        __syncthreads();
    }
    double v0 = 0.0, v1 = 0.0, v2 = 0.0, v3 = 0.0;
    int q = threadIdx.x;
    for (; q + 3 * 1024 < nparts; q += 4 * 1024) {
        v0 += part[q];
        v1 += part[q + 1024];
        v2 += part[q + 2 * 1024];
        v3 += part[q + 3 * 1024];
    }
    for (; q < nparts; q += 1024) v0 += part[q];
    block_sum_to<1024>((v0 + v1) + (v2 + v3), a.out[blockIdx.x]);
    if (a.hres && threadIdx.x == 0) {
        __threadfence();
        if (atomicAdd(a.cnt, 1u) == 2u) {
            __threadfence();
            const volatile double *sc = a.scal;
            for (int k = 0; k < 6; k++) a.hres[k] = sc[k];
            __threadfence_system();
            *a.cnt = 0u;
            __atomic_store_n((unsigned long long *)(a.hres + 7), __double_as_longlong(a.seq),
                             __ATOMIC_RELEASE);
        }
    }
}

#define BA_SUM_BS 1024
__global__ __launch_bounds__(BA_SUM_BS) void k_sum_parts(const double *__restrict__ part,
                                                         int nparts, double *__restrict__ out)
{
    double v0 = 0.0, v1 = 0.0, v2 = 0.0, v3 = 0.0;
    int q = threadIdx.x;
    for (; q + 3 * BA_SUM_BS < nparts; q += 4 * BA_SUM_BS) {
        v0 += part[q];
        v1 += part[q + BA_SUM_BS];
        v2 += part[q + 2 * BA_SUM_BS];
        v3 += part[q + 3 * BA_SUM_BS];
    }
    for (; q < nparts; q += BA_SUM_BS) v0 += part[q];
    block_sum_to<BA_SUM_BS>((v0 + v1) + (v2 + v3), out);
}

static inline int grid_for(long long work, int bs, int cap)
{
    long long g = (work + bs - 1) / bs;
    if (g < 1) g = 1;
    if (g > cap) g = cap;
    return (int)g;
}

static const int PT_GRID_CAP = 8192;

int ba_launch_rotations(ba_dev *d, const double *a, double *rot)
{
    if (d->na == BA_PROJ_NA) return 0;
    const int g = grid_for(d->m, 64, 1 << 30);
    KT_B(d);
    if (d->jac) {
        BA_DISPATCH(d->na, (k_rotations_jac<NA><<<g, 64, 0, d->stream>>>(a, rot, d->m)));
    } else {
        BA_DISPATCH(d->na, (k_rotations<NA><<<g, 64, 0, d->stream>>>(a, rot, d->m)));
    }
    KT_E(d, KT_ROT);
    return -(int)hipGetLastError();
}

template <int NA>
static void lin_chunk_launch(ba_dev *d, ba_flags f, const double *a, const double *rot,
                             const double *b, double *W, double *V, double *eB, double *upart,
                             double *chsse, const ba_upd *u)
{
    const ba_loss ls{d->loss_kind, d->loss_scale};
#define LIN_GRID <<<d->nch, 256, 0, d->stream>>>
#define LIN_ARGS                                                                           \
    d->ch_pt, d->ch_obase, d->ch_eslot, d->eslot_optr, d->eslot_obs, d->pt_ptr, d->obs_cam, \
        d->obs_lpt, d->obs_x, d->K4, a, rot, b, f, d->pivot, W, V, eB, upart, chsse,       \
        d->nch_reg, d->seg_pt, d->vseg, d->ch_cam
    if (d->jac) {
        if (u && ls.kind) k_update_linearize_jac<NA, true> LIN_GRID(LIN_ARGS, *u, ls);
        else if (u) k_update_linearize_jac<NA, false> LIN_GRID(LIN_ARGS, *u, ls);
        else if (ls.kind) k_linearize_chunk_jac<NA, true> LIN_GRID(LIN_ARGS, ls);
        else k_linearize_chunk_jac<NA, false> LIN_GRID(LIN_ARGS, ls);
    } else if (u && ls.kind) k_update_linearize_loss<NA> LIN_GRID(LIN_ARGS, *u, ls);
    else if (u) k_update_linearize<NA> LIN_GRID(LIN_ARGS, *u);
    else if (ls.kind) k_linearize_chunk_loss<NA> LIN_GRID(LIN_ARGS, ls);
    else k_linearize_chunk<NA> LIN_GRID(LIN_ARGS);
#undef LIN_ARGS
#undef LIN_GRID
}

int ba_launch_linearize(ba_dev *d, ba_flags f)
{
    if (!d->ordered) {
        KT_B(d);
        if (d->nch > 0)
            BA_DISPATCH(d->na, (lin_chunk_launch<NA>(d, f, d->a, d->rot, d->b, d->W, d->V,
                                                     d->eB, d->upart, d->chsse, nullptr)));
        if (d->nl > 0)
            k_long_vsum<<<d->nl, 64, 0, d->stream>>>(d->long_pt, d->long_seg0, d->vseg, d->V,
                                                     d->eB);
        KT_E(d, KT_LIN);
        return -(int)hipGetLastError();
    }
    const int g = grid_for(d->n, 256, PT_GRID_CAP);
    KT_B(d);
    BA_DISPATCH(d->na, (k_linearize<NA><<<g, 256, 0, d->stream>>>(
                           d->pt_ptr, d->obs_cam, d->obs_x, d->K4, d->a, d->rot, d->b, d->n, f,
                           d->pivot, d->jrec, d->W, d->V, d->eB, d->part, d->xh_out,
                           d->B_out)));
    KT_E(d, KT_LIN);
    k_sum_parts<<<1, BA_SUM_BS, 0, d->stream>>>(d->part, g, d->scal + 0);
    return -(int)hipGetLastError();
}

ba_camred ba_camred_args(const ba_dev *d, ba_flags f)
{
    return ba_camred{d->cam_eptr, d->cam_eslots, d->upart, d->m, f, d->pivot,
                     d->U, d->eA, d->chsse, d->nch, d->scal + 0, d->eA + d->ld};
}

int ba_launch_camera_reduce(ba_dev *d, ba_flags f, hipStream_t s)
{
    const int bs = ((d->na * (d->na + 1) / 2 + d->na) + 63) / 64 * 64;
    KT_B(d);
    if (!d->ordered) {
        BA_DISPATCH(d->na, (k_camera_reduce_chunks<NA><<<d->m + 1, 256, 0, s>>>(
                               ba_camred_args(d, f))));
    } else {
        BA_DISPATCH(d->na, (k_camera_reduce<NA><<<d->m, bs, 0, s>>>(
                               d->cam_ptr, d->cam_obs, d->jrec, d->m, f, d->pivot, d->U,
                               d->eA)));
    }
    KT_E(d, KT_CAMRED);
    return -(int)hipGetLastError();
}

int ba_launch_damp_point(ba_dev *d, double lambda)
{
    const int g = grid_for(d->n, 256, PT_GRID_CAP);
    KT_B(d);
    BA_DISPATCH(d->na, (k_damp_point<NA><<<g, 256, 0, d->stream>>>(
                           d->pt_ptr, d->V, d->eB, d->W, d->n, lambda, d->Vinv, d->Y, d->t)));
    KT_E(d, KT_DAMP);
    return -(int)hipGetLastError();
}

int ba_launch_schur(ba_dev *d, double lambda)
{
    const int bs = ((d->na * d->na + d->na) + 63) / 64 * 64;
    KT_B(d);
    BA_DISPATCH(d->na, (k_schur<NA><<<d->nb, bs, 0, d->stream>>>(
                           d->blk_jk, d->blk_ptr, d->term, d->Y, d->W, d->t, d->U, d->eA, d->nb,
                           lambda, d->schur_owner, d->sblk, d->rhs)));
    KT_E(d, KT_SCHUR);
    return -(int)hipGetLastError();
}

template <int NA>
static int launch_schur_fast(ba_dev *d, double lambda, const ba_camred *fold, bool side_camred)
{
    const bool two = d->ngrp_mf > 0 && d->ngrp > d->ngrp_mf && d->side &&
                     !(d->kt && d->kt->on);
    if (d->ngrp_mf > 0) {
        if (!d->vinv_fold) {
            KT_B(d);
            k_point_vinv<NA><<<(d->n + 255) / 256, 256, 0, d->stream>>>(d->V, d->n, lambda,
                                                                        d->Vinv);
            KT_E(d, KT_DAMP);
        }
        if (two) VLGBA_CHECK(hipEventRecord(d->ev_fork, d->stream));
        size_t sm2 = sizeof(double) * (d->mf_max_s * NA * NA + d->mf_max_e * NA) +
                     sizeof(unsigned) * (size_t)d->mf_max_blob;
        if (d->vinv_fold && sm2 < sizeof(double) * 256 * 9)
            sm2 = sizeof(double) * 256 * 9;
        TRY_RC(ba_ensure_dyn_lds((const void *)k_schur_mfma<NA>, sm2));
        const int ncr = fold ? d->m + 1 : 0;
        KT_B(d);
        k_schur_mfma<NA><<<d->ngrp_mf + ncr, 256, sm2, d->stream>>>(
            d->grp_ch, d->grp_gs, d->grp_ge, d->ch_pt, d->ch_obase, d->ch_blob, d->blob, d->W,
            d->Vinv, d->eB, d->N, d->n, d->mf_max_s, d->mf_max_e, d->spart, d->epart,
            d->ngrp_mf, fold ? *fold : ba_camred{}, d->vinv_fold ? d->V : nullptr, lambda);
        KT_E(d, KT_SCHUR_MF);
    }
    if (d->ngrp > d->ngrp_mf) {
        const int gcap = d->grp_max_s, ecap = d->grp_max_e, bcap = d->max_blob;
        size_t smem = sizeof(double) * (2 * BA_CH_OBS * 3 * NA + BA_CH_PTS * 12 +
                                        gcap * NA * NA + ecap * NA) +
                      sizeof(unsigned) * bcap;
        smem = (smem + 15) & ~(size_t)15;
        TRY_RC(ba_ensure_dyn_lds((const void *)k_schur_group<NA>, smem));
        if (two) VLGBA_CHECK(hipStreamWaitEvent(d->side, d->ev_fork, 0));
        KT_B(d);
        k_schur_group<NA><<<d->ngrp - d->ngrp_mf, 256, smem, two ? d->side : d->stream>>>(
            d->grp_ch + d->ngrp_mf, d->grp_gs + d->ngrp_mf, d->grp_ge + d->ngrp_mf, d->ch_pt,
            d->ch_obase, d->ch_blob, d->blob, d->V, d->eB, d->W, lambda, bcap, gcap, ecap,
            d->Vinv, d->spart, d->epart);
        KT_E(d, KT_SCHUR_CHUNK);
        if (two) VLGBA_CHECK(hipEventRecord(d->ev_join, d->side));
    }
    if (d->nl > 0) {
        KT_B(d);
        if (d->ngrp_mf == 0)
            k_point_vinv<NA><<<(d->n - d->p_long + 255) / 256, 256, 0, d->stream>>>(
                d->V + 9 * (size_t)d->p_long, d->n - d->p_long, lambda,
                d->Vinv + 9 * (size_t)d->p_long);
        k_long_y<NA><<<d->nl, 256, 0, d->stream>>>(d->long_pt, d->long_o0, d->long_ebase, d->W,
                                                   d->Vinv, d->eB, d->ylong, d->epart);
        KT_E(d, KT_SCHUR_CHUNK);
    }
    const int bs = ((NA * NA + NA) + 63) / 64 * 64;
    if (side_camred || two) VLGBA_CHECK(hipStreamWaitEvent(d->stream, d->ev_join, 0));
    KT_B(d);
    ba_longs lg{};
    if (d->nl > 0 && !d->nlb) {
        lg.pair_ptr = d->lpair_ptr;
        lg.pair = d->lpair;
        lg.ylong = d->ylong;
        lg.W = d->W;
        lg.L0 = d->long_o0_h;
    }
    ba_direct dir{nullptr, 0, nullptr};
    if (d->asm_direct) dir = ba_direct{d->chol->S, d->lds, d->scal + 4};
    const size_t lsh = lg.pair_ptr ? sizeof(double) * 2 * BA_LMATCH_BATCH * 3 * NA : 0;
    k_schur_reduce<NA><<<d->nb, bs, lsh, d->stream>>>(
        d->blk_jk, d->blk_gptr, d->blk_gslots, d->cam_gptr, d->cam_gslots, d->spart, d->epart,
        d->U, d->eA, d->nb, lambda, d->schur_owner, d->sblk, d->rhs, lg, dir);
    if (d->nl > 0 && d->nlb)
        k_schur_long_acc<NA><<<(4 * d->nlb + 255) / 256, 256, 0, d->stream>>>(
            d->lblk, d->nlb, d->lpair_ptr, d->lpair, d->ylong, d->W, d->long_o0_h, d->sblk);
    KT_E(d, KT_SCHUR_RED);
    return -(int)hipGetLastError();
}

int ba_launch_long_pairs(ba_dev *d, int fill, int *cnt)
{
    k_long_pairs<<<d->nb, 64, 0, d->stream>>>(d->blk_jk, d->nb, d->cam_lptr, d->cam_lobs,
                                              d->cam_ltrk, fill, cnt, d->lpair_ptr, d->lpair);
    return -(int)hipGetLastError();
}

int ba_launch_schur_fast(ba_dev *d, double lambda, const ba_camred *fold, bool side_camred)
{
    if (fold && d->ngrp_mf <= 0) return -1000;
    int rc = 0;
    BA_DISPATCH(d->na, rc = launch_schur_fast<NA>(d, lambda, fold, side_camred));
    return rc;
}

__global__ void k_publish(const double *__restrict__ scal, double *hres, double seq)
{
    if (threadIdx.x < 6) hres[threadIdx.x] = scal[threadIdx.x];
    __threadfence_system();
    __syncthreads();
    if (threadIdx.x == 0) {
        __atomic_store_n((unsigned long long *)(hres + 7), __double_as_longlong(seq),
                         __ATOMIC_RELEASE);
    }
}

int ba_launch_publish(ba_dev *d)
{
    d->seq++;
    k_publish<<<1, 64, 0, d->stream>>>(d->scal, d->hres_dev, (double)d->seq);
    return -(int)hipGetLastError();
}

int ba_launch_yeb(ba_dev *d)
{
    const int g = grid_for(d->n, 256, 1 << 30);
    BA_DISPATCH(d->na, (k_point_yeb<NA><<<g, 256, 0, d->stream>>>(d->pt_ptr, d->Y, d->eB, d->n,
                                                                    d->t)));
    return -(int)hipGetLastError();
}

int ba_launch_assemble(ba_dev *d)
{
    if (d->asm_direct) return 0;
    KT_B(d);
    TRY_RC(ba_assemble_tiles(d));
    KT_E(d, KT_ASSEMBLE);
    return 0;
}

static int launch_camera_update(ba_dev *d, int gc, double lam_dpg, bool folded)
{
    if (folded) return 0;
    KT_B(d);
    if (d->jac) {
        BA_DISPATCH(d->na, (k_camera_update_jac<NA><<<gc, 320, 0, d->stream>>>(
                               d->a, d->da, d->eA, d->m, lam_dpg, d->a_new, d->rot_new,
                               d->part)));
    } else {
        BA_DISPATCH(d->na, (k_camera_update<NA><<<gc, 320, 0, d->stream>>>(
                               d->a, d->da, d->eA, d->m, lam_dpg, d->a_new, d->rot_new,
                               d->part)));
    }
    KT_E(d, KT_CAMUPD);
    return 0;
}

static int launch_long_db(ba_dev *d, double lambda)
{
    if (d->nl > 0)
        BA_DISPATCH(d->na, (k_long_db<NA><<<d->nl, 256, 0, d->stream>>>(
                               d->long_pt, d->long_o0, d->obs_cam, d->W, d->da, d->eB,
                               d->Vinv, d->b, d->ndb, lambda, d->db, d->b_new,
                               d->dpg_long)));
    return 0;
}

static int launch_final_sums(ba_dev *d, const double *sse_part, const double *dpg_part, int gc,
                             double lam_dpg, bool folded, bool publish)
{
    ba_sum3 s3 = {{sse_part, dpg_part, d->part},
                  {d->nch, d->nch, gc},
                  {d->scal + 1, d->scal + 3, d->scal + 2},
                  d->scal, nullptr, 0.0, d->pub_cnt};
    if (folded) {
        s3.cam_da = d->da;
        s3.cam_eA = d->eA;
        s3.cam_part = d->part;
        s3.cam_m = d->m;
        s3.cam_na = d->na;
        s3.cam_lambda = lam_dpg;
    }
    if (publish) {
        d->seq++;
        s3.hres = d->hres_dev;
        s3.seq = (double)d->seq;
    }
    k_sum_parts3<<<3, 1024, 0, d->stream>>>(s3);
    return -(int)hipGetLastError();
}

int ba_launch_update(ba_dev *d, double lambda, ba_flags f, bool cam_updated, bool publish,
                     bool *published)
{
    const bool chunked = !d->ordered && d->nch > 0 && !d->obs_vis && !d->xh_out;
    const bool folded = cam_updated && (d->fused || chunked);
    publish = publish && (d->fused || chunked);
    if (published) *published = publish;
    const int gc = (d->m + 63) / 64;
    const double lam_dpg = d->dpg_lambda ? lambda : 0.0;
    TRY_RC(launch_camera_update(d, gc, lam_dpg, folded));
    if (d->fused) {
        KT_B(d);
        TRY_RC(launch_long_db(d, lambda));
        const ba_upd u{d->W, d->da, d->eB, d->Vinv, d->b, d->ndb, lambda, d->db, d->b_new,
                       d->chsse2 + 2 * (size_t)d->nch, d->seg_long, d->long_o0, d->dpg_long};
        BA_DISPATCH(d->na, (lin_chunk_launch<NA>(d, f, d->a_new, d->rot_new, d->b_new, d->W2,
                                                 d->V2, d->eB2, d->upart2, d->chsse2, &u)));
        if (d->nl > 0)
            k_long_vsum<<<d->nl, 64, 0, d->stream>>>(d->long_pt, d->long_seg0, d->vseg, d->V2,
                                                     d->eB2);
        KT_E(d, KT_LIN_UPD);
        return launch_final_sums(d, d->chsse2, d->chsse2 + 2 * (size_t)d->nch, gc, lam_dpg,
                                 folded, publish);
    }
    if (chunked) {
        KT_B(d);
        TRY_RC(launch_long_db(d, lambda));
        if (d->loss_kind) {
            const ba_loss ls{d->loss_kind, d->loss_scale};
            BA_DISPATCH(d->na, (k_point_update_chunk_loss<NA><<<d->nch, 256, 0, d->stream>>>(
                                   d->ch_pt, d->ch_obase, d->pt_ptr, d->obs_cam, d->obs_lpt,
                                   d->obs_x, d->K4, d->W, d->da, d->eB, d->Vinv, d->b,
                                   d->a_new, d->rot_new, d->ndb, lambda, d->db, d->b_new,
                                   d->chsse + d->nch, d->chsse + 2 * (size_t)d->nch,
                                   d->nch_reg, d->seg_pt, d->seg_long, d->long_o0,
                                   d->dpg_long, ls)));
        } else {
            BA_DISPATCH(d->na, (k_point_update_chunk<NA><<<d->nch, 256, 0, d->stream>>>(
                                   d->ch_pt, d->ch_obase, d->pt_ptr, d->obs_cam, d->obs_lpt,
                                   d->obs_x, d->K4, d->W, d->da, d->eB, d->Vinv, d->b,
                                   d->a_new, d->rot_new, d->ndb, lambda, d->db, d->b_new,
                                   d->chsse + d->nch, d->chsse + 2 * (size_t)d->nch,
                                   d->nch_reg, d->seg_pt, d->seg_long, d->long_o0,
                                   d->dpg_long)));
        }
        KT_E(d, KT_PTUPD);
        return launch_final_sums(d, d->chsse + d->nch, d->chsse + 2 * (size_t)d->nch, gc,
                                 lam_dpg, folded, publish);
    }
    k_sum_parts<<<1, BA_SUM_BS, 0, d->stream>>>(d->part, gc, d->scal + 2);
    const int g = grid_for(d->n, 256, PT_GRID_CAP);
    KT_B(d);
    BA_DISPATCH(d->na, (k_point_update<NA><<<g, 256, 0, d->stream>>>(
                           d->pt_ptr, d->obs_cam, d->obs_x, d->K4, d->W, d->da, d->eB, d->Vinv,
                           d->b, d->a_new, d->rot_new, d->n, d->ndb, lambda, d->db, d->b_new,
                           d->part + BA_PART_MAX, d->part + 2 * BA_PART_MAX, d->obs_vis,
                           d->xh_out)));
    KT_E(d, KT_PTUPD);
    k_sum_parts<<<1, BA_SUM_BS, 0, d->stream>>>(d->part + BA_PART_MAX, g, d->scal + 1);
    k_sum_parts<<<1, BA_SUM_BS, 0, d->stream>>>(d->part + 2 * BA_PART_MAX, g, d->scal + 3);
    return -(int)hipGetLastError();
}

int ba_launch_obs_residuals(ba_dev *d, double *e, double *w, double *rho)
{
    if (d->N <= 0) return 0;
    const ba_loss ls{d->loss_kind, d->loss_scale};
    BA_DISPATCH(d->na, (k_obs_residuals<NA><<<(d->N + 255) / 256, 256, 0, d->stream>>>(
                           d->pt_ptr, d->obs_cam, d->obs_x, d->K4, d->a, d->rot, d->b, d->n,
                           d->N, ls, e, w, rho)));
    return -(int)hipGetLastError();
}

template <int NA>
__global__ void k_seq_old_sse(const int *__restrict__ cam_ptr, const int *__restrict__ cam_obs,
                              const double *__restrict__ jrec, int m, double *__restrict__ out)
{
    if (threadIdx.x != 0) return;
    constexpr int JS = 2 * NA + 2;
    double s = 0.0;
    for (int j = 0; j < m; j++)
        for (int q = cam_ptr[j]; q < cam_ptr[j + 1]; q++) {
            const double *e = jrec + (size_t)JS * cam_obs[q] + 2 * NA;
            s = s + e[0] * e[0];
            s = s + e[1] * e[1];
        }
    *out = s;
}

__global__ void k_seq_new_sums(const int *__restrict__ cam_ptr, const int *__restrict__ cam_obs,
                               const double *__restrict__ obs_x, const double *__restrict__ xh,
                               int m, const double *__restrict__ da,
                               const double *__restrict__ eA, long long ld,
                               const double *__restrict__ db, const double *__restrict__ eB,
                               int n, double lambda, double *__restrict__ scal)
{
    if (threadIdx.x != 0) return;
    double s = 0.0;
    for (int j = 0; j < m; j++)
        for (int q = cam_ptr[j]; q < cam_ptr[j + 1]; q++) {
            const int o = cam_obs[q];
            const double d0 = obs_x[2 * (size_t)o] - xh[2 * (size_t)o];
            const double d1 = obs_x[2 * (size_t)o + 1] - xh[2 * (size_t)o + 1];
            s = s + d0 * d0;
            s = s + d1 * d1;
        }
    double g = 0.0;
    for (long long k = 0; k < ld; k++) g = g + da[k] * (lambda * da[k] + eA[k]);
    for (long long k = 0; k < 3 * (long long)n; k++) g = g + db[k] * (lambda * db[k] + eB[k]);
    scal[1] = s;
    scal[2] = g;
    scal[3] = 0.0;
}

int ba_launch_parity_old_sse(ba_dev *d)
{
    BA_DISPATCH(d->na, (k_seq_old_sse<NA><<<1, 64, 0, d->stream>>>(d->cam_ptr, d->cam_obs,
                                                                   d->jrec, d->m, d->scal + 0)));
    return -(int)hipGetLastError();
}

int ba_launch_parity_new_sums(ba_dev *d, double lambda)
{
    k_seq_new_sums<<<1, 64, 0, d->stream>>>(d->cam_ptr, d->cam_obs, d->obs_x, d->xh_out, d->m,
                                            d->da, d->eA, d->ld, d->db, d->eB, d->n, lambda,
                                            d->scal);
    return -(int)hipGetLastError();
}

int ba_launch_assemble_plain(ba_dev *d, double *S, long long ld, int lower_only)
{
    VLGBA_CHECK(hipMemsetAsync(S, 0, sizeof(double) * ld * ld, d->stream));
    const long long work = (long long)d->nb * d->na * d->na;
    const int g = (int)((work + 255) / 256);
    if (g > 0)
        BA_DISPATCH(d->na, (k_assemble<NA><<<g, 256, 0, d->stream>>>(d->blk_jk, d->sblk, d->nb,
                                                                       ld, lower_only, S)));
    return -(int)hipGetLastError();
}
```

bundleadjustmentmatlab_amd/csrc/ba_limits.h:

```cpp
#pragma once

#define BA_TILE 64
#define BA_TILE32 32
#ifndef BA_ND_MAX
#define BA_ND_MAX 8
#endif
#define BA_ND_MAX_PAIRS 16384LL
#define BA_ND_MAX_SETUP (1LL << 26)
#define BA_CR_MAXLEV 30

#ifndef BA_CH_OBS
#define BA_CH_OBS 128
#endif
#define BA_CH_PTS 64
#define BA_CH_TERMS 4096
#define BA_GACC 4096
#define BA_GE_CAP 128
#define BA_GROUPS 2048
#define BA_MF_GROUPS 768
#define BA_GROUP_CH 64
#define BA_MF_PTS 20
#define BA_MF_RT(na) ((na) == 6 ? 3 : 4)
#define BA_MF_CMAX(na) ((16 * BA_MF_RT(na)) / (na))
#define BA_MF_GACC 1536
#define BA_MF_GE_CAP 24
#define BA_LONG_OBS 65535
#define BA_LONG_TERMS (1LL << 26)
#define BA_LCAM_LDS 256
#define BA_LMATCH_BATCH 48
```

bundleadjustmentmatlab_amd/csrc/ba_plan.cpp:

```cpp
#include "ba_plan.h"

#include <unistd.h>

#include <algorithm>
#include <chrono>
#include <climits>
#include <condition_variable>
#include <cstdio>
#include <cstdlib>
#include <functional>
#include <mutex>
#include <numeric>
#include <thread>
#include <vector>

int sort_obs(const vlgba_problem *p, host_obs &h)
{
    const long long N = p->num_obs;
    bool sorted = true;
    for (long long o = 0; o < N && sorted; o++) {
        const int i = p->obs_pt[o], j = p->obs_cam[o];
        if (i < 0 || i >= p->n || j < 0 || j >= p->m) return VLGBA_E_ARG;
        if (o > 0) {
            const int i0 = p->obs_pt[o - 1], j0 = p->obs_cam[o - 1];
// ... 766 lines not shown
                *B++ = (unsigned)(t1 - t0);
                *B++ = (unsigned)(u1 - u0);
                for (int s = s0; s <= s1; s++) *B++ = (unsigned)(P.slot_tptr[s] - t0);
                for (int e = e0; e <= e1; e++) *B++ = (unsigned)(P.eslot_optr[e] - u0);
                for (int s = s0; s < s1; s++) *B++ = P.cs_g[s];
                for (int e = e0; e < e1; e++) *B++ = P.ce_g[e];
                for (int i = p0; i < p1; i++)
                    for (int o = lptr[i]; o < lptr[i + 1]; o++) *B++ = (unsigned)(i - p0);
                for (int t = t0; t < t1; t++)
                    *B++ = (unsigned)P.slot_term[2 * t] | ((unsigned)P.slot_term[2 * t + 1] << 16);
                for (int u = u0; u < u1; u++) *B++ = P.eslot_obs[u];
            }
        }, &boff);
    }
    PLAN_T("blobs");
    for (size_t l = 0; l < P.long_pt.size(); l++)
        for (int o = P.long_o0[l]; o < P.long_o0[l + 1]; o += BA_CH_OBS) {
            P.ch_blob.push_back(P.ch_blob.back());
            P.ch_obase.push_back(std::min(o + BA_CH_OBS, P.long_o0[l + 1]));
        }
    return true;
}
}

int track_kind(long long k, int cmax)
{
    if (k <= cmax) return 0;
    if (k <= BA_CH_OBS && k * (k + 1) / 2 <= BA_CH_TERMS) return 1;
    return 2;
}

void order_points_by_kind(int cmax, host_obs &h, std::vector<int> &pt_ptr, int p0, int p1,
                          std::vector<int> &pperm, std::vector<int> &operm)
{
    const int n = p1 - p0;
    int cnt[3] = {0, 0, 0};
    long long lterms = 0;
    for (int i = p0; i < p1; i++) {
        const long long k = pt_ptr[i + 1] - pt_ptr[i];
        const int kind = track_kind(k, cmax);
        cnt[kind]++;
        if (kind == 2) {
            if (k > BA_LONG_OBS) return;
            lterms += k * (k + 1) / 2;
        }
    }
    if (lterms > BA_LONG_TERMS) return;
    if ((cnt[0] == 0) + (cnt[1] == 0) + (cnt[2] == 0) >= 2) return;
    pperm.assign(n, 0);
    {
        int at[3] = {0, cnt[0], cnt[0] + cnt[1]};
        for (int i = 0; i < n; i++) pperm[at[track_kind(pt_ptr[p0 + i + 1] - pt_ptr[p0 + i], cmax)]++] = i;
    }
    const int o0 = pt_ptr[p0];
    const size_t N = (size_t)(pt_ptr[p1] - o0);
    std::vector<int> cam2(N);
    std::vector<double> x2(2 * N);
    operm.resize(N);
    std::vector<int> ptr2(n + 1, 0);
    size_t q = 0;
    for (int i2 = 0; i2 < n; i2++) {
        const int i = p0 + pperm[i2];
        for (int o = pt_ptr[i]; o < pt_ptr[i + 1]; o++, q++) {
            cam2[q] = h.cam[o];
            x2[2 * q] = h.x[2 * (size_t)o];
            x2[2 * q + 1] = h.x[2 * (size_t)o + 1];
            operm[q] = o - o0;
        }
        ptr2[i2 + 1] = (int)q;
    }
    if (o0 == 0 && N == h.cam.size()) {
        h.cam.swap(cam2);
        h.x.swap(x2);
    } else {
        std::copy(cam2.begin(), cam2.end(), h.cam.begin() + o0);
        std::copy(x2.begin(), x2.end(), h.x.begin() + 2 * (size_t)o0);
    }
    for (int i2 = 0; i2 < n; i2++) {
        pt_ptr[p0 + i2 + 1] = o0 + ptr2[i2 + 1];
        for (int o = ptr2[i2]; o < ptr2[i2 + 1]; o++) h.pt[o0 + o] = p0 + i2;
    }
}

void plan_host(int m, int na, int n, const std::vector<int> &lptr, const std::vector<int> &lcam,
               const std::vector<int> &pt_ptr_all, const std::vector<int> &cam_all, int p0,
               int p1, long long o0, bool lower_blocks, bool all_diag, bool no_mfma, bool &fast,
               int &p_long, host_blocks &hb, host_plan &plan, void (*mark)(const char *))
{
    p_long = n;
    if (fast) {
        while (p_long > 0 && track_kind(lptr[p_long] - lptr[p_long - 1], BA_MF_CMAX(na)) == 2)
            p_long--;
        long long lterms = 0;
        for (int i = 0; fast && i < n; i++) {
            const long long k = lptr[i + 1] - lptr[i];
            const bool lng = track_kind(k, BA_MF_CMAX(na)) == 2;
            if (lng != (i >= p_long) || k > BA_LONG_OBS) fast = false;
            if (lng) lterms += k * (k + 1) / 2;
        }
        if (lterms > BA_LONG_TERMS) fast = false;
    }
    build_blocks(m, pt_ptr_all, cam_all, p0, p1, o0, lower_blocks, all_diag, !fast, hb);
    if (mark) mark("blocks");
    if (fast) {
        int p_split = 0;
        if (!no_mfma)
            while (p_split < p_long && lptr[p_split + 1] - lptr[p_split] <= BA_MF_CMAX(na))
                p_split++;
        if (!build_plan(m, na, lptr, lcam, hb, plan, BA_MF_CMAX(na), p_split, p_long)) {
            fast = false;
            hb = host_blocks();
            build_blocks(m, pt_ptr_all, cam_all, p0, p1, o0, lower_blocks, all_diag, true, hb);
        }
    }
}
bool plan_mfma_groups_tile_points(const host_plan &plan, int n)
{
    const int ngrp = (int)plan.grp_ch.size() - 1;
    bool tile = plan.ngrp_mf > 0 && ngrp == plan.ngrp_mf && plan.long_pt.empty();
    int at = 0;
    for (int g = 0; tile && g < plan.ngrp_mf; g++) {
        tile = plan.ch_pt[plan.grp_ch[g]] == at &&
               plan.ch_pt[plan.grp_ch[g + 1]] >= at;
        at = plan.ch_pt[plan.grp_ch[g + 1]];
    }
    return tile && at == n;
}

void plan_obs_local_point(const host_plan &plan, const std::vector<int> &lptr,
                          std::vector<unsigned char> &lpt)
{
    lpt.assign(std::max(lptr.back(), 1), 0);
    for (size_t ch = 0; ch + 1 < plan.ch_pt.size(); ch++)
        for (int i = plan.ch_pt[ch]; i < plan.ch_pt[ch + 1]; i++)
            for (int o = lptr[i]; o < lptr[i + 1]; o++)
                lpt[o] = (unsigned char)(i - plan.ch_pt[ch]);
}

void plan_chunk_cameras(const host_plan &plan, const std::vector<int> &lcam,
                        std::vector<int> &ccam)
{
    const size_t nchk = plan.ch_obase.size() - 1;
    ccam.assign(2 * std::max<size_t>(nchk, 1), 0);
    for (size_t ch = 0; ch < nchk; ch++) {
        int lo = INT_MAX, hi = -1;
        for (int o = plan.ch_obase[ch]; o < plan.ch_obase[ch + 1]; o++) {
            lo = std::min(lo, lcam[o]);
            hi = std::max(hi, lcam[o]);
        }
        ccam[2 * ch] = hi < 0 ? 0 : lo;
        ccam[2 * ch + 1] = hi < 0 ? 0 : hi;
    }
}
```

bundleadjustmentmatlab_amd/csrc/ba_plan.h:

```cpp
#pragma once
#include "ba_limits.h"
#include "../../include/vlgba.h"

#include <stddef.h>
#include <utility>
#include <vector>

#pragma GCC visibility push(hidden)

struct host_obs {
    std::vector<int> pt, cam;
    std::vector<double> x;
};
int sort_obs(const vlgba_problem *p, host_obs &h);

struct host_blocks {
    std::vector<int> jk, ptr, term;
    int m = 0;
    bool dense_tab = true;
    std::vector<int> tab;
    std::vector<std::vector<std::pair<int, int>>> rows;
    void reset()
    {
        if (dense_tab && !tab.empty())
            for (size_t q = 0; q + 1 < jk.size(); q += 2) tab[(size_t)jk[q] * m + jk[q + 1]] = -1;
        jk.clear();
        ptr.clear();
        term.clear();
        m = 0;
        dense_tab = true;
        rows.clear();
    }
    int find(int j, int k) const
    {
        if (dense_tab) return tab[(size_t)j * m + k];
        for (auto &pr : rows[j])
            if (pr.first == k) return pr.second;
        return -1;
    }
    int insert(int j, int k)
    {
        int id = find(j, k);
        if (id >= 0) return id;
        id = (int)jk.size() / 2;
        jk.push_back(j);
        jk.push_back(k);
        if (dense_tab) tab[(size_t)j * m + k] = id;
        else rows[j].push_back({k, id});
        return id;
    }
};
void build_blocks(int m, const std::vector<int> &pt_ptr_all, const std::vector<int> &cam_all,
                  int p0, int p1, long long obs_base, bool lower, bool all_diag, bool need_terms,
                  host_blocks &hb);

struct host_plan {
    std::vector<int> ch_pt, ch_slot, ch_eslot, slot_blk, slot_tptr, eslot_optr;
    std::vector<unsigned short> slot_term, eslot_obs;
    std::vector<int> cam_eptr, cam_eslots;
    int max_terms = 0, max_slots = 0;
    long long n_terms = 0;
    std::vector<int> grp_ch, grp_gs, grp_ge;
    std::vector<unsigned short> cs_g, ce_g;
    std::vector<int> gslot_blk, gecam;
    std::vector<int> blk_gptr, blk_gslots, cam_gptr, cam_gslots;
    int grp_max_s = 0, grp_max_e = 0;
    int mf_max_s = 0, mf_max_e = 0;
    int nch_mf = 0, ngrp_mf = 0;
    int nch_reg = 0, nseg = 0;
    std::vector<int> seg_pt, seg_long;
    std::vector<int> long_pt, long_o0, long_seg0;
    std::vector<int> long_ebase;
    std::vector<int> cam_lptr, cam_lobs, cam_ltrk;
    int max_lcam = 0;
    std::vector<unsigned> blob;
    std::vector<int> ch_blob, ch_obase;
    int max_blob = 0;
    int mf_max_blob = 0;
    void reset()
    {
        for (std::vector<int> *v :
             {&ch_pt, &ch_slot, &ch_eslot, &slot_blk, &slot_tptr, &eslot_optr,
              &cam_eptr, &cam_eslots, &grp_ch, &grp_gs, &grp_ge, &gslot_blk, &gecam,
              &blk_gptr, &blk_gslots, &cam_gptr, &cam_gslots, &seg_pt, &seg_long, &long_pt,
              &long_o0, &long_seg0, &long_ebase, &cam_lptr, &cam_lobs, &cam_ltrk, &ch_blob,
              &ch_obase})
            v->clear();
        for (std::vector<unsigned short> *v : {&slot_term, &eslot_obs, &cs_g, &ce_g}) v->clear();
        blob.clear();
        max_terms = max_slots = 0;
        n_terms = 0;
        grp_max_s = grp_max_e = mf_max_s = mf_max_e = nch_mf = ngrp_mf = 0;
        nch_reg = nseg = max_lcam = max_blob = mf_max_blob = 0;
    }
};
int track_kind(long long k, int cmax);
void order_points_by_kind(int cmax, host_obs &h, std::vector<int> &pt_ptr, int p0, int p1,
                          std::vector<int> &pperm, std::vector<int> &operm);
void plan_host(int m, int na, int n, const std::vector<int> &lptr, const std::vector<int> &lcam,
               const std::vector<int> &pt_ptr_all, const std::vector<int> &cam_all, int p0,
               int p1, long long o0, bool lower_blocks, bool all_diag, bool no_mfma, bool &fast,
               int &p_long, host_blocks &hb, host_plan &plan,
               void (*mark)(const char *) = nullptr);

bool plan_mfma_groups_tile_points(const host_plan &plan, int n);
void plan_obs_local_point(const host_plan &plan, const std::vector<int> &lptr,
                          std::vector<unsigned char> &lpt);
void plan_chunk_cameras(const host_plan &plan, const std::vector<int> &lcam,
                        std::vector<int> &ccam);

#pragma GCC visibility pop
```

bundleadjustmentmatlab_amd/csrc/ba_solver.cpp:

```cpp
#include "ba_internal.h"
#include "ba_plan.h"
#include "ba_chol.h"
#include "ba_pcg.h"
#include "../../include/vlgba.h"

#include <rccl/rccl.h>
#include <rocsolver/rocsolver.h>

#include <dlfcn.h>
#include <cstdlib>
#include <string>

#include <algorithm>
#include <atomic>
#include <chrono>
#include <cmath>
#include <cstdio>
#include <cstring>
#include <mutex>
#include <unordered_map>
#include <map>
#include <new>
#include <numeric>
#include <vector>
// ... 383 lines not shown
    size_t total = 0;
    template <typename T> void add(T **dst, const std::vector<T> &v)
    {
        items.push_back({(void **)dst, v.data(), sizeof(T) * v.size(), total});
        total += (sizeof(T) * std::max<size_t>(v.size(), 1) + 255) & ~(size_t)255;
    }
    int commit(vlgba_ctx *c, hipStream_t s)
    {
        if (items.empty()) return 0;
        char *dev = nullptr;
        TRY(ctx_alloc(c, &dev, total));
        ba_aux &x = c->aux;
        const size_t need = (total + sizeof(double) - 1) / sizeof(double);
        if (x.pin_cap < need) {
            if (x.pin) (void)hipHostFree(x.pin);
            size_t cap = 1 << 16;
            while (cap < need) cap <<= 1;
            x.pin = nullptr;
            x.pin_cap = 0;
            if (hipHostMalloc((void **)&x.pin, sizeof(double) * cap, hipHostMallocDefault) ==
                hipSuccess)
                x.pin_cap = cap;
        }
        char *stage = x.pin_cap >= need ? (char *)x.pin : nullptr;
        for (const item &it : items) {
            *it.dst = dev + it.off;
            if (it.bytes == 0) continue;
            if (stage)
                std::memcpy(stage + it.off, it.src, it.bytes);
            else
                VLGBA_CHECK(hipMemcpyAsync(dev + it.off, it.src, it.bytes,
                                           hipMemcpyHostToDevice, s));
        }
        if (stage)
            VLGBA_CHECK(hipMemcpyAsync(dev, stage, total, hipMemcpyHostToDevice, s));
        VLGBA_CHECK(hipStreamSynchronize(s));
        return 0;
    }
};

static int ctx_setup(vlgba_ctx *c, const vlgba_problem *p, const host_obs &h,
                     const std::vector<int> &pt_ptr_all, bool lower_blocks, bool all_diag,
                     bool stage_mode)
{
    ba_dev &d = c->d;
    const int na = p->num_a;
    d.device = c->aux.device;
    VLGBA_CHECK(hipDeviceGetAttribute(&d.ncu, hipDeviceAttributeMultiprocessorCount, d.device));
    d.m = p->m;
    d.na = na;
    d.js = 2 * na + 2;
    d.n = c->p1 - c->p0;
    const long long o0 = pt_ptr_all[c->p0], o1 = pt_ptr_all[c->p1];
    d.N = (int)(o1 - o0);
    d.ld = (long long)na * p->m;
    d.lds = ((d.ld + 63) / 64) * 64;
    d.schur_owner = 1;
    d.dpg_lambda = c->rank == 0;
    hipStream_t s = d.stream;

    std::vector<int> lptr(d.n + 1), lcam(h.cam.begin() + o0, h.cam.begin() + o1);
    for (int i = 0; i <= d.n; i++) lptr[i] = pt_ptr_all[c->p0 + i] - (int)o0;
    std::vector<int> cptr(p->m + 1, 0), cobs(d.N);
    for (int o = 0; o < d.N; o++) cptr[lcam[o] + 1]++;
    for (int j = 0; j < p->m; j++) cptr[j + 1] += cptr[j];
    {
        std::vector<int> pos(cptr.begin(), cptr.end() - 1);
        for (int o = 0; o < d.N; o++) cobs[pos[lcam[o]]++] = o;
    }
    bool fast = !d.ordered && !stage_mode;
    int p_long = d.n;
    static thread_local host_blocks hb;
    static thread_local host_plan plan;
    hb.reset();
    plan.reset();
    ST_MARK("lists");
    plan_host(p->m, na, d.n, lptr, lcam, pt_ptr_all, h.cam, c->p0, c->p1, o0, lower_blocks,
              all_diag, d.no_mfma != 0, fast, p_long, hb, plan,
              [](const char *w) { ST_MARK(w); });
    d.mfma = fast && plan.nch_mf > 0;
    if (!fast) d.ordered = 1;
    if (d.ordered) d.jac = VLGBA_JAC_FD;
    ST_MARK("plan");
    d.nb = (int)hb.jk.size() / 2;
    d.T = (long long)hb.term.size() / 2;

    TRY(ctx_alloc(c, &d.obs_cam, d.N));
    TRY(ctx_alloc(c, &d.pt_ptr, d.n + 1));
    TRY(ctx_alloc(c, &d.cam_ptr, p->m + 1));
    TRY(ctx_alloc(c, &d.cam_obs, d.N));
    TRY(ctx_alloc(c, &d.obs_x, 2 * (size_t)d.N));
    TRY(ctx_alloc(c, &d.K4, 4 * (size_t)p->m));
    TRY(ctx_alloc(c, &d.a, (size_t)d.ld));
    TRY(ctx_alloc(c, &d.a_new, (size_t)d.ld));
    TRY(ctx_alloc(c, &d.b, 3 * (size_t)d.n));
    TRY(ctx_alloc(c, &d.b_new, 3 * (size_t)d.n));
    TRY(ctx_alloc(c, &d.rot, 45 * (size_t)p->m));
    TRY(ctx_alloc(c, &d.rot_new, 45 * (size_t)p->m));
    TRY(ctx_alloc(c, &d.W, (size_t)3 * na * (d.N + 1)));
    VLGBA_CHECK(hipMemsetAsync(d.W + (size_t)3 * na * d.N, 0, sizeof(double) * 3 * na, s));
    if (!fast) {
        TRY(ctx_alloc(c, &d.jrec, (size_t)d.js * d.N));
        TRY(ctx_alloc(c, &d.Y, (size_t)3 * na * d.N));
        TRY(ctx_alloc(c, &d.t, (size_t)na * d.N));
    } else {
        d.nch_reg = plan.nch_reg;
        d.nch = plan.nch_reg + plan.nseg;
        d.nl = (int)plan.long_pt.size();
        d.max_lcam = plan.max_lcam;
        d.long_o0_h = plan.long_o0.empty() ? 0 : plan.long_o0[0];
        d.p_long = p_long;
        plan_batch pb;
        if (d.nl > 0) {
            pb.add(&d.seg_pt, plan.seg_pt);
            pb.add(&d.seg_long, plan.seg_long);
            pb.add(&d.long_pt, plan.long_pt);
            pb.add(&d.long_o0, plan.long_o0);
            pb.add(&d.long_seg0, plan.long_seg0);
            pb.add(&d.long_ebase, plan.long_ebase);
            pb.add(&d.cam_lptr, plan.cam_lptr);
            pb.add(&d.cam_lobs, plan.cam_lobs);
            pb.add(&d.cam_ltrk, plan.cam_ltrk);
            TRY(ctx_alloc(c, &d.ylong, (size_t)3 * na * plan.cam_lobs.size()));
            TRY(ctx_alloc(c, &d.vseg, 12 * (size_t)plan.nseg));
            TRY(ctx_alloc(c, &d.dpg_long, (size_t)d.nl));
        }
        d.ns = (int)plan.slot_blk.size();
        d.nes = (int)plan.eslot_optr.size() - 1;
        d.ch_max_terms = plan.max_terms;
        d.ch_max_slots = plan.max_slots;
        d.nterm_fast = plan.n_terms;
        d.blob_words = (long long)plan.blob.size();
        d.ngrp = (int)plan.grp_ch.size() - 1;
        d.ngrp_mf = plan.ngrp_mf;
        d.max_blob = plan.max_blob;
        d.mf_max_blob = plan.mf_max_blob;
        d.mf_max_s = plan.mf_max_s;
        d.mf_max_e = plan.mf_max_e;
        const char *vf = std::getenv("VLGBA_VINV_FOLD");
        d.vinv_fold = plan_mfma_groups_tile_points(plan, d.n) && !(vf && vf[0] == '0');
        pb.add(&d.blob, plan.blob);
        pb.add(&d.ch_blob, plan.ch_blob);
        pb.add(&d.ch_obase, plan.ch_obase);
        std::vector<unsigned char> lpt;
        std::vector<int> ccam;
        plan_obs_local_point(plan, lptr, lpt);
        plan_chunk_cameras(plan, lcam, ccam);
        const char *dse = std::getenv("VLGBA_DA_STAGE");
        if (dse && dse[0] == '0')
            for (size_t ch = 0; ch + 1 < plan.ch_obase.size(); ch++)
                ccam[2 * ch + 1] = ccam[2 * ch] + (1 << 20);
        pb.add(&d.obs_lpt, lpt);
        pb.add(&d.ch_cam, ccam);
        d.grp_max_s = plan.grp_max_s;
        d.grp_max_e = plan.grp_max_e;
        d.ngs = (int)plan.gslot_blk.size();
        d.nge = (int)plan.gecam.size();
        TRY(ctx_alloc(c, &d.spart, (size_t)na * na * d.ngs));
        TRY(ctx_alloc(c, &d.epart, (size_t)na * d.nge));
        pb.add(&d.grp_ch, plan.grp_ch);
        pb.add(&d.grp_gs, plan.grp_gs);
        pb.add(&d.grp_ge, plan.grp_ge);
        pb.add(&d.cs_g, plan.cs_g);
        pb.add(&d.ce_g, plan.ce_g);
        pb.add(&d.blk_gptr, plan.blk_gptr);
        pb.add(&d.blk_gslots, plan.blk_gslots);
        pb.add(&d.cam_gptr, plan.cam_gptr);
        pb.add(&d.cam_gslots, plan.cam_gslots);
        TRY(ctx_alloc(c, &d.upart, (size_t)(na * (na + 1) / 2 + na) * d.nes));
        TRY(ctx_alloc(c, &d.chsse, 3 * (size_t)d.nch));
        pb.add(&d.ch_pt, plan.ch_pt);
        pb.add(&d.ch_eslot, plan.ch_eslot);
        pb.add(&d.eslot_optr, plan.eslot_optr);
        pb.add(&d.eslot_obs, plan.eslot_obs);
        pb.add(&d.cam_eptr, plan.cam_eptr);
        pb.add(&d.cam_eslots, plan.cam_eslots);
        TRY(pb.commit(c, s));
        ST_MARK("plan_upload");
    }
    TRY(ctx_alloc(c, &d.U, (size_t)na * na * p->m + na * (size_t)p->m + 1));
    d.eA = d.U + (size_t)na * na * p->m;
    TRY(ctx_alloc(c, &d.V, 9 * (size_t)d.n));
    TRY(ctx_alloc(c, &d.eB, 3 * (size_t)(d.n + 1)));
    TRY(ctx_alloc(c, &d.Vinv, 9 * (size_t)(d.n + 1)));
    VLGBA_CHECK(hipMemsetAsync(d.eB + 3 * (size_t)d.n, 0, sizeof(double) * 3, s));
    VLGBA_CHECK(hipMemsetAsync(d.Vinv + 9 * (size_t)d.n, 0, sizeof(double) * 9, s));
    TRY(ctx_alloc(c, &d.db, 3 * (size_t)d.n));
    const char *fused_env = std::getenv("VLGBA_FUSED");
    const bool fused_on = !(fused_env && fused_env[0] == '0');
    if (fast && d.nch > 0 && fused_on) {
        TRY(ctx_alloc(c, &d.W2, (size_t)3 * na * (d.N + 1)));
        VLGBA_CHECK(hipMemsetAsync(d.W2 + (size_t)3 * na * d.N, 0, sizeof(double) * 3 * na, s));
        TRY(ctx_alloc(c, &d.V2, 9 * (size_t)d.n));
        TRY(ctx_alloc(c, &d.eB2, 3 * (size_t)(d.n + 1)));
        VLGBA_CHECK(hipMemsetAsync(d.eB2 + 3 * (size_t)d.n, 0, sizeof(double) * 3, s));
        TRY(ctx_alloc(c, &d.upart2, (size_t)(na * (na + 1) / 2 + na) * d.nes));
        TRY(ctx_alloc(c, &d.chsse2, 3 * (size_t)d.nch));
        d.fused = 1;
    }
    TRY(ctx_alloc(c, &d.blk_jk, 2 * (size_t)d.nb));
    TRY(ctx_alloc(c, &d.blk_ptr, (size_t)d.nb + 1));
    TRY(ctx_alloc(c, &d.term, 2 * (size_t)d.T));
    TRY(upload(d.blk_jk, hb.jk.data(), hb.jk.size(), s));
    int *lp_cnt = nullptr;
    if (fast && d.nl > 0) {
        TRY(ctx_alloc(c, &lp_cnt, (size_t)d.nb + 1));
        TRY(ctx_alloc(c, &d.lpair_ptr, (size_t)d.nb + 1));
        TRY(ba_launch_long_pairs(&d, 0, lp_cnt));
    }
    TRY(ctx_alloc(c, &d.sblk, (size_t)na * na * d.nb + d.lds + 1));
    d.rhs = d.sblk + (size_t)na * na * d.nb;
    if (!stage_mode && d.dense_solve == 5) {
        TRY(ctx_alloc(c, &d.da, (size_t)d.lds));
        ST_MARK("allocs");
        TRY(ba_pcg_setup(&d, hb.jk.data(), d.nb));
        ST_MARK("pcg_setup");
    } else if (!stage_mode) {
        TRY(ctx_alloc(c, &d.da, (size_t)d.lds));
        ST_MARK("allocs");
        TRY(ba_chol_setup(&d, hb.jk.data(), d.nb));
        ST_MARK("chol_setup");
        const chol_plan &P = d.chol->plan;
        const char *ad = std::getenv("VLGBA_ASM_DIRECT");
        d.asm_direct = P.asm_direct_ok && !(ad && ad[0] == '0') && fast && !d.ordered &&
                       c->world == 1 && !c->comm && d.nl == 0 && P.cr_nlev > 0 && P.cr32 &&
                       P.nd_np == 0;
        const char *cf = std::getenv("VLGBA_CAMUPD_FOLD");
        d.camupd_fold = !(cf && cf[0] == '0') && fast && !d.ordered && d.nch > 0 &&
                        P.cr_nlev > 0 && P.cr32 && P.cr_fused && d.chol->crflag && P.nd_np == 0 &&
                        na != BA_PROJ_NA && na <= 10 && P.tb32 % na == 0 &&
                        d.ld == (long long)na * p->m;
    } else {
        TRY(ctx_alloc(c, &d.da, (size_t)d.lds));
    }
    TRY(ctx_alloc(c, &d.part, 3 * (size_t)BA_PART_MAX));
    TRY(ctx_alloc(c, &d.scal, 8));
    TRY(upload(d.obs_cam, lcam.data(), d.N, s));
    TRY(upload(d.pt_ptr, lptr.data(), d.n + 1, s));
    TRY(upload(d.cam_ptr, cptr.data(), p->m + 1, s));
    TRY(upload(d.cam_obs, cobs.data(), d.N, s));
    TRY(upload(d.obs_x, h.x.data() + 2 * o0, 2 * (size_t)d.N, s));
    if (p->K) TRY(upload(d.K4, p->K, 4 * (size_t)p->m, s));
    else VLGBA_CHECK(hipMemsetAsync(d.K4, 0, sizeof(double) * 4 * p->m, s));
    TRY(upload(d.blk_ptr, hb.ptr.data(), hb.ptr.size(), s));
    TRY(upload(d.term, hb.term.data(), hb.term.size(), s));
    ST_MARK("uploads");
    if (fast && d.nl > 0) {
        std::vector<int> h((size_t)d.nb + 1, 0);
        TRY(download(h.data(), lp_cnt, (size_t)d.nb, s));
        VLGBA_CHECK(hipStreamSynchronize(s));
        long long tot = 0;
        for (int b = 0; b < d.nb; b++) {
            const int v = h[b];
            h[b] = (int)tot;
            tot += v;
        }
        h[d.nb] = (int)tot;
        if (tot > 0x7fffffffLL) return VLGBA_E_ARG;
        TRY(ctx_alloc(c, &d.lpair, (size_t)tot + 1));
        TRY(upload(d.lpair_ptr, h.data(), (size_t)d.nb + 1, s));
        TRY(ba_launch_long_pairs(&d, 1, nullptr));
        const char *la = std::getenv("VLGBA_LONG_ACC");
        if (!(la && la[0] == '0')) {
            std::vector<int> lb;
            for (int b = 0; b < d.nb; b++)
                if (h[b + 1] > h[b]) lb.push_back(b);
            std::stable_sort(lb.begin(), lb.end(), [&](int x, int y) {
                return h[x + 1] - h[x] > h[y + 1] - h[y];
            });
            d.nlb = (int)lb.size();
            if (d.nlb > 0) {
                TRY(ctx_alloc(c, &d.lblk, lb.size()));
                TRY(upload(d.lblk, lb.data(), lb.size(), s));
            }
        }
        ST_MARK("long_pairs");
    }
    VLGBA_CHECK(hipMemsetAsync(d.scal, 0, 8 * sizeof(double), s));
    TRY(ctx_alloc(c, &d.pub_cnt, 1));
    VLGBA_CHECK(hipMemsetAsync(d.pub_cnt, 0, sizeof(unsigned), s));
    VLGBA_CHECK(hipStreamSynchronize(s));
    return 0;
}

static int ctx_create(const vlgba_problem *p, const vlgba_options *o, vlgba_ctx **out,
                      bool lower_blocks, bool all_diag, bool stage_mode,
                      std::vector<int> *pt_ptr_out = nullptr, host_obs *h_out = nullptr)
{
    *out = nullptr;
    if (!p || p->m < 1 || p->n < 0 || p->num_obs < 0) return VLGBA_E_ARG;
    if (p->model == VLGBA_MODEL_EUCLIDEAN) {
        if (!p->K) return VLGBA_E_ARG;
        if (p->num_a != 6 && p->num_a != 7 && p->num_a != 10 && p->num_a != BA_RAD_NA)
            return VLGBA_E_NUMA;
        if (p->num_a == BA_RAD_NA && stage_mode) return VLGBA_E_NUMA;
        if (p->num_a == BA_RAD_NA && o && o->ordered != 0) return VLGBA_E_ARG;
    } else if (p->model == VLGBA_MODEL_PROJECTIVE) {
        if (p->num_a != BA_PROJ_NA) return VLGBA_E_NUMA;
    } else {
        return VLGBA_E_ARG;
    }
    if (p->num_obs > 0x7fffffffLL) return VLGBA_E_ARG;
    vlgba_ctx *c = new (std::nothrow) vlgba_ctx();
    if (!c) return VLGBA_E_NOMEM;
    std::memset(&c->d, 0, sizeof(c->d));
    vlgba_options defaults;
    std::memset(&defaults, 0, sizeof defaults);
    if (!o) o = &defaults;
    int rc = 0;
    setup_trace trace;
    g_st = &trace;
    struct st_reset { ~st_reset() { g_st = nullptr; } } st_reset_;
    do {
        if (hipSetDevice(o->device) != hipSuccess) { rc = VLGBA_E_ARG; break; }
        if (aux_acquire(o->device, c->aux)) {
            rc = -1;
            break;
        }
        c->has_aux = true;
        c->d.stream = c->aux.stream;
        c->d.side = c->aux.side;
        c->d.ev_fork = c->aux.ev_fork;
        c->d.ev_join = c->aux.ev_join;
        c->d.hres = c->aux.hres_host;
        c->d.hres_dev = c->aux.hres_dev;
        ST_MARK("aux");
        host_obs h;
        rc = sort_obs(p, h);
        if (rc) break;
        ST_MARK("sort");
        std::vector<int> pt_ptr_all(p->n + 1, 0);
        for (size_t q = 0; q < h.pt.size(); q++) pt_ptr_all[h.pt[q] + 1]++;
        for (int i = 0; i < p->n; i++) pt_ptr_all[i + 1] += pt_ptr_all[i];
        c->world = o->world_size > 1 ? o->world_size : 1;
        c->rank = c->world > 1 ? o->rank : 0;
        if (c->world > 1) {
            const long long N = p->num_obs;
            auto bound = [&](int r) -> int {
                const long long target = (N * r) / c->world;
                return (int)(std::lower_bound(pt_ptr_all.begin(), pt_ptr_all.end(), (int)target) -
                             pt_ptr_all.begin());
            };
            c->p0 = c->rank == 0 ? 0 : std::min(bound(c->rank), p->n);
            c->p1 = c->rank == c->world - 1 ? p->n : std::min(bound(c->rank + 1), p->n);
            if (o->comm_id) {
                if (comm_acquire(&c->comm, c->world, o->comm_id, c->rank) != ncclSuccess) {
                    rc = VLGBA_E_COMM;
                    break;
                }
            } else if (o->allreduce) {
                c->host_allreduce = o->allreduce;
                c->host_user = o->allreduce_user;
            } else {
                rc = VLGBA_E_COMM;
                break;
            }
        } else {
            c->p0 = 0;
            c->p1 = p->n;
            if (o->comm_id) {
                if (comm_acquire(&c->comm, 1, o->comm_id, 0) != ncclSuccess) {
                    rc = VLGBA_E_COMM;
                    break;
                }
            }
        }
        if (o->ordered == 0 && !stage_mode)
            order_points_by_kind(o->schur_kernel == 1 ? 0 : BA_MF_CMAX(p->num_a), h, pt_ptr_all,
                                 c->p0, c->p1, c->pperm, c->operm);
        ST_MARK("order");
        c->n_global = p->n;
        c->N_global = p->num_obs;
        c->num_vis = p->num_vis > 0 ? p->num_vis : (double)p->num_obs;
        c->flags.fix_structure = o->fix_structure;
        c->flags.fix_motion = o->fix_motion;
        if (o->semantics != 0 && o->semantics != 1) { rc = VLGBA_E_ARG; break; }
        c->flags.has_pivot = o->pivot != nullptr && o->semantics == 0 &&
                             p->model == VLGBA_MODEL_EUCLIDEAN;
        c->model = p->model;
        c->max_iter = o->max_iter > 0 ? o->max_iter : 20;
        c->max_iter2 = o->max_iter2 > 0 ? o->max_iter2 : 10;
        c->lambda0 = c->lambda = o->lambda0 > 0 ? o->lambda0 : 1e-3;
        c->verbose = o->verbose;
        c->d.dense_solve = o->dense_solve;
        c->d.ordered = o->ordered != 0;
        if (o->dense_solve == 5 && (o->ordered != 0 || stage_mode)) { rc = VLGBA_E_ARG; break; }
        if (o->ordered == 2) {
            if (c->world > 1) { rc = VLGBA_E_ARG; break; }
            c->d.parity = 1;
            c->d.dense_solve = 3;
        } else if (o->ordered < 0 || o->ordered > 2 || o->dense_solve < 0 ||
                   o->dense_solve > 5) {
            rc = VLGBA_E_ARG;
            break;
        }
        c->stop_rel = o->stop_rel > 0 ? o->stop_rel : 1e-3;
        if (const char *ev = std::getenv("VLGBA_DEBUG_SPIN_TIMEOUT")) {
            int r = -1, k = 0;
            if (std::sscanf(ev, "%d:%d", &r, &k) == 2 && r == c->rank) c->debug_timeouts = k;
            if (c->debug_timeouts > 0)
                std::fprintf(stderr, "[vlgba] VLGBA_DEBUG_SPIN_TIMEOUT=%s: rank %d's first %d "
                             "passes report a hand-off timeout (test hook)\n", ev, r, k);
        }
        c->on_pass = o->on_pass;
        c->on_pass_user = o->on_pass_user;
        c->d.no_mfma = o->schur_kernel == 1;
        c->d.ndb = o->semantics == 1 || p->num_a == BA_RAD_NA ? p->num_a : 6;
        c->d.loss_kind = VLGBA_LOSS_NONE;
        c->d.loss_scale = 0.0;
        c->d.jac = VLGBA_JAC_FD;
        if (const char *ev = std::getenv("VLGBA_JACOBIAN")) {
            if (!std::strcmp(ev, "analytic") && o->ordered == 0 && !stage_mode)
                c->d.jac = VLGBA_JAC_ANALYTIC;
        }
        if (p->num_a == BA_RAD_NA) c->d.jac = VLGBA_JAC_ANALYTIC;
        rc = ctx_setup(c, p, h, pt_ptr_all, lower_blocks, all_diag, stage_mode);
        if (rc) break;
        if (p->num_a == BA_RAD_NA && c->d.ordered) { rc = VLGBA_E_ARG; break; }
        if (c->d.pcg && c->d.ordered) { rc = VLGBA_E_ARG; break; }
        ST_MARK("setup_end");
        if (c->d.parity) {
            rc = ctx_alloc(c, &c->d.xh_out, 2 * (size_t)c->d.N + 2);
            if (rc) break;
        }
        if (c->flags.has_pivot) {
            rc = ctx_alloc(c, &c->d.pivot, (size_t)p->m);
            if (rc) break;
            rc = upload(c->d.pivot, o->pivot, (size_t)p->m, c->d.stream);
            if (rc) break;
        }
        if (std::getenv("VLGBA_KTIME_ALL")) {
            rc = vlgba_set_timing(c, 1);
            if (rc) break;
// ... 963 lines not shown
}

int vlgba_get_step(vlgba_ctx *c, double *da, double *db)
{
    if (!c) return VLGBA_E_ARG;
    TRY(ctx_enter(c));
    if (da) TRY(download(da, c->d.da, (size_t)c->d.ld, c->d.stream));
    if (db) TRY(download_points(c, db, c->d.db, 3));
    VLGBA_CHECK(hipStreamSynchronize(c->d.stream));
    return 0;
}

int vlgba_debug_force_status(vlgba_ctx *c, int word, int passes)
{
    if (!c || word < 4 || word > 6 || passes < 0) return VLGBA_E_ARG;
    if (word == 6) {
        if (c->d.chol) c->d.chol->debug_runner_fail = passes;
    } else
        (word == 4 ? c->debug_pivots : c->debug_timeouts) = passes;
    return 0;
}

int vlgba_set_pcg(vlgba_ctx *c, double tol, int max_iter)
{
    if (!c || !c->d.pcg || !std::isfinite(tol) || tol >= 1.0) return VLGBA_E_ARG;
    if (tol > 0.0) c->d.pcg->tol = tol;
    if (max_iter > 0) c->d.pcg->max_iter = max_iter;
    return 0;
}

int vlgba_get_pcg(vlgba_ctx *c, double *tol, int *max_iter)
{
    if (!c || !c->d.pcg) return VLGBA_E_ARG;
    if (tol) *tol = c->d.pcg->tol;
    if (max_iter) *max_iter = c->d.pcg->max_iter;
    return 0;
}

int vlgba_get_pcg_stats(vlgba_ctx *c, int *iterations, double *relres, int *converged,
                        long long *total)
{
    if (!c || !c->d.pcg) return VLGBA_E_ARG;
    const ba_pcg &P = *c->d.pcg;
    if (iterations) *iterations = P.iters;
    if (relres) *relres = P.relres;
    if (converged) *converged = P.conv;
    if (total) *total = P.total;
    return 0;
}

int vlgba_set_timing(vlgba_ctx *c, int on)
{
    if (!c) return VLGBA_E_ARG;
    TRY(ctx_enter(c));
    if (on && !c->ev[0])
        for (auto &e : c->ev) VLGBA_CHECK(hipEventCreate(&e));
    if (on && !c->d.kt) {
        c->d.kt = new (std::nothrow) ba_ktimer();
        if (!c->d.kt) return VLGBA_E_NOMEM;
    }
    c->timing = on;
    if (c->d.kt) c->d.kt->on = on;
    return 0;
}

static std::mutex g_kt_mu;
static double g_kt_ms[KT_N], g_kt_flops[KT_N];
static long long g_kt_calls[KT_N];

static void kt_retire(const ba_ktimer *kt)
{
    std::lock_guard<std::mutex> lk(g_kt_mu);
    for (int k = 0; k < KT_N; k++) {
        g_kt_ms[k] += kt->ms[k];
        g_kt_calls[k] += kt->calls[k];
        g_kt_flops[k] += kt->flops[k];
    }
}

int vlgba_kernel_ms(vlgba_ctx *c, double *ms, long long *calls, int reset)
{
    if (!c) {
        std::lock_guard<std::mutex> lk(g_kt_mu);
        for (int k = 0; k < KT_N; k++) {
            if (ms) ms[k] = g_kt_ms[k];
            if (calls) calls[k] = g_kt_calls[k];
            if (reset) {
                g_kt_ms[k] = 0.0;
                g_kt_calls[k] = 0;
                g_kt_flops[k] = 0.0;
            }
        }
        return 0;
    }
    if (!c->d.kt) return VLGBA_E_ARG;
    for (int k = 0; k < KT_N; k++) {
        if (ms) ms[k] = c->d.kt->ms[k];
        if (calls) calls[k] = c->d.kt->calls[k];
        if (reset) {
            c->d.kt->ms[k] = 0.0;
            c->d.kt->calls[k] = 0;
            c->d.kt->flops[k] = 0.0;
        }
    }
    return 0;
}

int vlgba_kernel_flops(vlgba_ctx *c, double *flops)
{
    if (!flops) return VLGBA_E_ARG;
    if (!c) {
        std::lock_guard<std::mutex> lk(g_kt_mu);
        for (int k = 0; k < KT_N; k++) flops[k] = g_kt_flops[k];
        return 0;
    }
    if (!c->d.kt) return VLGBA_E_ARG;
    for (int k = 0; k < KT_N; k++) flops[k] = c->d.kt->flops[k];
    return 0;
}

const char *vlgba_kernel_name(int k)
{
    static const char *names[KT_N] = {
        "k_rotations", "k_linearize", "k_camera_reduce", "k_damp_point", "k_schur",
        "k_schur_group", "k_schur_reduce", "k_assemble", "k_factor_step", "k_syrk",
        "k_backward", "k_camera_update", "k_point_update", "k_cr_factor", "k_cr_update",
        "k_cr_back", "k_schur_mfma", "k_update_linearize"};
    return (k >= 0 && k < KT_N) ? names[k] : "";
}

int vlgba_plan_info(vlgba_ctx *c, long long *info, int len)
{
    if (!c || !info) return VLGBA_E_ARG;
    const ba_dev &d = c->d;
    static const chol_plan no_plan;
    const chol_plan &P = d.chol ? d.chol->plan : no_plan;
    const long long ne = P.cr_nlev ? P.eptr[P.cr_nlev] : 0;
    const long long nk = P.cr_nlev ? P.kptr[P.cr_nlev] : 0;
    const long long v[VLGBA_NPLAN] = {d.N,   d.n,    d.m,   d.na,         d.nch,  d.ns,
                                      d.nes, d.ngrp, d.ngs, d.nge,        d.nb,   P.nt,
                                      P.cr_nlev, ne, nk,    d.ordered,    d.ordered ? d.T : d.nterm_fast,
                                      d.blob_words, d.mfma,
                                      P.cr_nlev ? (P.cr32 ? P.tb32 : 64) : 0,
                                      d.ngrp_mf, c->pperm.empty() ? 0 : 1, d.nl, P.nd_np,
                                      P.nd_np ? P.nt - P.nd_a0[P.nd_np] : 0,
                                      (long long)P.fl_factor, (long long)P.fl_syrk,
                                      (long long)P.fl_back, d.chol ? d.chol->runner_runs : 0,
                                      d.vinv_fold, d.camupd_fold, d.pcg ? 1 : 0,
                                      d.pcg ? d.pcg->bytes : d.chol ? d.chol->bytes : 0};
    for (int k = 0; k < len && k < VLGBA_NPLAN; k++) info[k] = v[k];
    return VLGBA_NPLAN;
}

int vlgba_phase_ms(vlgba_ctx *c, double *ms7)
{
    if (!c || !ms7) return VLGBA_E_ARG;
    for (int q = 0; q < 7; q++) ms7[q] = c->phase_ms[q];
    return 0;
}

int vlgba_sync(vlgba_ctx *c)
{
    if (!c) return VLGBA_E_ARG;
    TRY(ctx_enter(c));
    VLGBA_CHECK(hipStreamSynchronize(c->d.stream));
    return 0;
}

int vlgba_step(vlgba_ctx *c, int relinearize, int update_lm, vlgba_step_info *info)
{
    if (!c) return VLGBA_E_ARG;
    TRY(ctx_enter(c));
    vlgba_step_info tmp;
    if (!info) info = &tmp;
    TRY(lm_pass(c, relinearize, info));
    if (update_lm) lm_apply(c, info);
    return 0;
}

int vlgba_run_passes(vlgba_ctx *c, int npass, vlgba_step_info *info)
{
    if (!c || npass < 0) return VLGBA_E_ARG;
    TRY(ctx_enter(c));
    vlgba_step_info tmp;
    if (!info) info = &tmp;
    std::memset(info, 0, sizeof *info);
    for (int q = 0; q < npass; q++) TRY(lm_pass(c, 1, info));
    return 0;
}

int vlgba_run(vlgba_ctx *c, double *error_out, int error_cap, vlgba_stats *stats)
{
    if (!c || (error_out && error_cap < 0)) return VLGBA_E_ARG;
    TRY(ctx_enter(c));
    auto t0 = std::chrono::steady_clock::now();
    c->lambda = c->lambda0;
    c->nu = 2.0;
    c->lin_valid = 0;
    std::vector<double> err;
    int iter = 1, iter2 = 0, passes = 0, acc = 0;
    const int pinv0 = c->pinv_used, retry0 = c->spin_retries, nd0 = c->nd_retries;
    for (;;) {
        if (!(iter < c->max_iter && iter2 < c->max_iter2)) break;
        if (iter >= 3) {
            const double e1 = err[iter - 1], e0 = err[iter - 2];
            if (!(e1 > 1e-20 && e0 - e1 > c->stop_rel * e0)) break;
        }
        vlgba_step_info info;
        TRY(lm_pass(c, 0, &info));
        passes++;
        if (info.accepted) {
            const bool proj = c->model == VLGBA_MODEL_PROJECTIVE;
            const double olde = proj ? 1 / c->num_vis * info.old_sse : info.old_sse / c->num_vis;
            const double newe = proj ? 1 / c->num_vis * info.new_sse : info.new_sse / c->num_vis;
            if (c->verbose && c->rank == 0)
                std::printf("iter %d: error= %.5g -> %.5g\n", iter, olde, newe);
            if ((int)err.size() < iter) err.push_back(olde);
            else err[iter - 1] = olde;
            iter++;
            err.push_back(newe);
            iter2 = 0;
            acc++;
        } else {
            iter2++;
        }
        lm_apply(c, &info);
        if (c->on_pass && c->rank == 0) c->on_pass(passes, iter, &info, c->on_pass_user);
    }
    VLGBA_CHECK(hipStreamSynchronize(c->d.stream));
    if (error_out)
        for (size_t q = 0; q < err.size() && q < (size_t)error_cap; q++) error_out[q] = err[q];
    if (stats) {
        stats->iterations = passes;
        stats->accepted = acc;
        stats->num_error = (int)err.size();
        stats->lambda = c->lambda;
        stats->pinv_passes = c->pinv_used - pinv0;
        stats->spin_retries = c->spin_retries - retry0;
        stats->nd_retries = c->nd_retries - nd0;
        stats->seconds =
            std::chrono::duration<double>(std::chrono::steady_clock::now() - t0).count();
    }
    return 0;
}

int vlgba_solve(const vlgba_problem *prob, const vlgba_options *opt, double *a, double *b,
                double *error_out, int error_cap, vlgba_stats *stats)
{
    if (!a || !b) return VLGBA_E_ARG;
    vlgba_ctx *c = nullptr;
    TRY(vlgba_create(prob, opt, &c));
    int rc = vlgba_set_params(c, a, b);
    if (!rc) rc = vlgba_run(c, error_out, error_cap, stats);
    if (!rc) rc = vlgba_get_params(c, a, b);
    vlgba_destroy(c);
    return rc;
}

static void obs_from_vis(int m, int n, const double *vis, std::vector<int> &pt,
                         std::vector<int> &cam)
{
    for (int i = 0; i < n; i++)
        for (int j = 0; j < m; j++)
            if (vis[i + (size_t)n * j] != 0.0) {
                pt.push_back(i);
                cam.push_back(j);
            }
}

static int mex1_impl(int model, int m, int n, int num_a, const double *K, const double *a,
                     const double *b, const double *X, const double *vis, double *X_hat,
                     double *A, double *B, double *e, double *U, double *V, double *W,
                     double *eA, double *eB)
{
    if (m < 1 || n < 0 || (!K && model == VLGBA_MODEL_EUCLIDEAN) || !a || !b || !X || !vis)
        return VLGBA_E_ARG;
    std::vector<int> pt, cam;
    obs_from_vis(m, n, vis, pt, cam);
    const long long N = (long long)pt.size();
    std::vector<double> ox(2 * N);
    for (long long q = 0; q < N; q++) {
        const size_t p = (size_t)pt[q] + (size_t)n * cam[q];
        ox[2 * q] = X[2 * p];
        ox[2 * q + 1] = X[2 * p + 1];
    }
    vlgba_problem pr = {m, n, num_a, N, pt.data(), cam.data(), ox.data(), K, 0.0, model};
    vlgba_ctx *c = nullptr;
    TRY(ctx_create(&pr, nullptr, &c, true, true, true));
    ba_dev &d = c->d;
    int rc = 0;
    std::vector<double> jr((size_t)d.js * N), hW((size_t)3 * num_a * N), xh(2 * N), hB(6 * N);
    do {
        if ((rc = ctx_alloc(c, &d.xh_out, 2 * (size_t)N))) break;
        if ((rc = ctx_alloc(c, &d.B_out, 6 * (size_t)N))) break;
        if ((rc = upload(d.a, a, (size_t)d.ld, d.stream))) break;
        if ((rc = upload(d.b, b, 3 * (size_t)n, d.stream))) break;
        ba_flags f = {0, 0, 0};
        if ((rc = ba_launch_rotations(&d, d.a, d.rot))) break;
        if ((rc = ba_launch_linearize(&d, f))) break;
        if ((rc = ba_launch_camera_reduce(&d, f, d.stream))) break;
        if ((rc = download(jr.data(), d.jrec, jr.size(), d.stream))) break;
        if ((rc = download(hW.data(), d.W, hW.size(), d.stream))) break;
        if ((rc = download(xh.data(), d.xh_out, xh.size(), d.stream))) break;
        if ((rc = download(hB.data(), d.B_out, hB.size(), d.stream))) break;
        if ((rc = download(U, d.U, (size_t)num_a * num_a * m, d.stream))) break;
        if ((rc = download(eA, d.eA, (size_t)num_a * m, d.stream))) break;
// ... 247 lines not shown
```

include/vlgba.h:

```cpp
#ifndef VLGBA_H
#define VLGBA_H

#ifdef __cplusplus
extern "C" {
#endif

#define VLGBA_E_ARG (-1001)
#define VLGBA_E_NUMA (-1002)
#define VLGBA_E_ORDER (-1003)
#define VLGBA_E_NOMEM (-1004)
#define VLGBA_E_COMM (-1005)
#define VLGBA_E_ABI (-1006)
#define VLGBA_E_SINGULAR (-1007)

#define VLGBA_ABI_VERSION 6

#define VLGBA_MODEL_EUCLIDEAN 0
#define VLGBA_MODEL_PROJECTIVE 1

typedef struct {
    int m;
    int n;
    int num_a;
    long long num_obs;
    const int *obs_pt;
    const int *obs_cam;
    const double *obs_x;
    const double *K;
    double num_vis;
    int model;
} vlgba_problem;

struct vlgba_step_info;

typedef struct {
    int fix_structure;
    int fix_motion;
    const unsigned char *pivot;
    int verbose;
    int max_iter;
    int max_iter2;
    double lambda0;
    int device;
    int rank;
    int world_size;
    const void *comm_id;
    int dense_solve;
    int ordered;
    int (*allreduce)(double *buf, long long count, void *user);
    void *allreduce_user;
    int schur_kernel;
    int semantics;
    double stop_rel;
    void (*on_pass)(int pass, int iter, const struct vlgba_step_info *info, void *user);
    void *on_pass_user;
} vlgba_options;

typedef struct {
    int iterations;
    int accepted;
    int num_error;
    double lambda;
    double seconds;
    int pinv_passes;
    int spin_retries;
    int nd_retries;
} vlgba_stats;

typedef struct vlgba_step_info {
    double old_sse;
    double new_sse;
    double dpg;
    double rho;
    double lambda;
    int accepted;
    int chol_failed;
    int pinv;
    int spin_retry;
    int nd_retry;
} vlgba_step_info;

typedef struct vlgba_ctx vlgba_ctx;

int vlgba_solve(const vlgba_problem *prob, const vlgba_options *opt, double *a, double *b,
                double *error_out, int error_cap, vlgba_stats *stats);

int vlgba_create(const vlgba_problem *prob, const vlgba_options *opt, vlgba_ctx **out);
int vlgba_set_params(vlgba_ctx *ctx, const double *a, const double *b);
int vlgba_get_params(vlgba_ctx *ctx, double *a, double *b);
int vlgba_step(vlgba_ctx *ctx, int relinearize, int update_lm, vlgba_step_info *info);
int vlgba_get_linearization(vlgba_ctx *ctx, double *U, double *eA, double *V, double *eB,
                            double *W);
int vlgba_run(vlgba_ctx *ctx, double *error_out, int error_cap, vlgba_stats *stats);
int vlgba_run_passes(vlgba_ctx *ctx, int npass, vlgba_step_info *info);
int vlgba_get_step(vlgba_ctx *ctx, double *da, double *db);
int vlgba_get_reduced_system(vlgba_ctx *ctx, int *blk_jk, double *blocks, double *e_);
int vlgba_covariance(vlgba_ctx *ctx, int scale, double *cov_a, double *cov_a_full,
                     double *cov_b, double *info);
#define VLGBA_COV_DENSE 0
#define VLGBA_COV_SELECTED 1
int vlgba_set_covariance_method(vlgba_ctx *ctx, int kind);
int vlgba_get_covariance_method(vlgba_ctx *ctx, int *kind);
int vlgba_get_covariance_blocks(vlgba_ctx *ctx, int *blk_jk, double *blocks);
#define VLGBA_LOSS_NONE 0
#define VLGBA_LOSS_HUBER 1
#define VLGBA_LOSS_CAUCHY 2
int vlgba_set_loss(vlgba_ctx *ctx, int kind, double scale);
int vlgba_get_loss(vlgba_ctx *ctx, int *kind, double *scale);
#define VLGBA_JAC_FD 0
#define VLGBA_JAC_ANALYTIC 1
int vlgba_set_jacobian(vlgba_ctx *ctx, int kind);
int vlgba_get_jacobian(vlgba_ctx *ctx, int *kind);
int vlgba_set_pcg(vlgba_ctx *ctx, double tol, int max_iter);
int vlgba_get_pcg(vlgba_ctx *ctx, double *tol, int *max_iter);
int vlgba_get_pcg_stats(vlgba_ctx *ctx, int *iterations, double *relres, int *converged,
                        long long *total);
int vlgba_get_residuals(vlgba_ctx *ctx, double *e, double *w, double *rho);
int vlgba_sync(vlgba_ctx *ctx);
void vlgba_destroy(vlgba_ctx *ctx);
int vlgba_set_timing(vlgba_ctx *ctx, int on);
int vlgba_phase_ms(vlgba_ctx *ctx, double *ms7);
#define VLGBA_NKERNELS 18
int vlgba_kernel_ms(vlgba_ctx *ctx, double *ms, long long *calls, int reset);
int vlgba_kernel_flops(vlgba_ctx *ctx, double *flops);
const char *vlgba_kernel_name(int k);
#define VLGBA_NPLAN 33
int vlgba_plan_info(vlgba_ctx *ctx, long long *info, int len);


int vlgba_mex_bundle_1(int m, int n, int num_a, const double *K, const double *a,
                       const double *b, const double *X, const double *vis,
                       double *X_hat, double *A, double *B, double *e, double *U, double *V,
                       double *W, double *eA, double *eB);

int vlgba_mex_bundle_2(int m, int n, int num_a, const double *Y, const double *W,
                       const double *U, const double *eA, const double *eB, double *S,
                       double *e_);

int vlgba_mex_bundle_3(int m, int n, int num_a, const double *W, const double *da,
                       const double *eB, const double *Vinv, const double *K, const double *a,
                       const double *b, const double *X, const double *vis, double *db,
                       double *a_new, double *b_new, double *X_hat);

int vlgba_mex_bundle_proj_1(int m, int n, const double *a, const double *b, const double *X,
                            const double *vis, double *X_hat, double *A, double *B, double *e,
                            double *U, double *V, double *W, double *eA, double *eB);

int vlgba_mex_bundle_proj_2(int m, int n, const double *Y, const double *W, const double *U,
                            const double *eA, const double *eB, double *S, double *e_);

int vlgba_mex_bundle_proj_3(int m, int n, const double *W, const double *da, const double *eB,
                            const double *Vinv, const double *a, const double *b,
                            const double *X, const double *vis, double *db, double *a_new,
                            double *b_new, double *X_hat);

typedef struct {
    int nprob;
    int num_a;
    const long long *obs_ptr;
    const double *X;
    const double *x;
    const double *K;
} vlgba_resect_problem;

int vlgba_resect(const vlgba_resect_problem *prob, const vlgba_options *opt, double *a,
                 double *error_out, int error_cap, int *num_error, vlgba_stats *stats);


int vlgba_triangulate(int m, const double *K, const double *T, const double *w,
                      long long n, const long long *obs_ptr, const int *obs_cam,
                      const double *obs_x, int device, double *X ,
                      int *status );

int vlgba_intersect(int m, const double *K, const double *T, const double *w,
                    long long n, const long long *obs_ptr, const int *obs_cam,
                    const double *obs_x, const vlgba_options *opt,
                    double *X ,
                    double *error_out, int error_cap, int *num_error,
                    vlgba_stats *stats);

int vlgba_resect_ex(const vlgba_resect_problem *prob, const vlgba_options *opt,
                    int jacobian , int loss ,
                    double loss_scale , double *a,
                    double *error_out, int error_cap, int *num_error,
                    double *res_out , double *w_out ,
                    vlgba_stats *stats);

int vlgba_intersect_ex(int m, const double *K, const double *T, const double *w,
                       const double *kd ,
                       long long n, const long long *obs_ptr, const int *obs_cam,
                       const double *obs_x, const vlgba_options *opt,
                       int jacobian, int loss, double loss_scale, double *X,
                       double *error_out, int error_cap, int *num_error,
                       double *res_out, double *w_out, vlgba_stats *stats);

int vlgba_triangulate_ex(int m, const double *K, const double *T, const double *w,
                         const double *kd , long long n,
                         const long long *obs_ptr, const int *obs_cam,
                         const double *obs_x, int device, double *X, int *status);

int vlgba_get_unique_id(void *id128);
int vlgba_comm_release(const void *id128);

int vlgba_debug_sincos(const double *x, double *s, double *c, long long n);
int vlgba_debug_pinv_solve(int ld, const double *S, const double *e_, double *da);
int vlgba_debug_force_status(vlgba_ctx *ctx, int word, int passes);
int vlgba_debug_nd_plan(int m, int num_a, const int *blk_jk, int nb, int *bnd, int *crit);
int vlgba_debug_selinv_plan(int ntiles, int *elim, int *eptr, int *src);
int vlgba_debug_pcg_plan(int m, const int *blk_jk, int nb, int *rowptr, int *ent);

int vlgba_version(char *buf, int len);
int vlgba_abi_check(int abi_version, long long sz_problem, long long sz_options,
                    long long sz_stats, long long sz_step_info, long long sz_resect_problem);
#define VLGBA_ABI_CHECK()                                                                    \
    vlgba_abi_check(VLGBA_ABI_VERSION, (long long)sizeof(vlgba_problem),                     \
                    (long long)sizeof(vlgba_options), (long long)sizeof(vlgba_stats),        \
                    (long long)sizeof(vlgba_step_info), (long long)sizeof(vlgba_resect_problem))
int vlgba_device_count(void);

typedef struct {
    int m, n, track;
    double depth_lo, depth_hi;
    double noise;
    unsigned long long seed;
    int keep_first_rotation;
    double width, height;
} vlgba_scene_spec;

typedef struct {
    double *K, *w, *T, *X;
    double *w0, *T0, *X0;
    int *obs_pt, *obs_cam;
    double *obs_x;
    long long num_obs_cap;
    long long num_obs;
    long long behind;
} vlgba_scene_out;

int vlgba_scene_banded(const vlgba_scene_spec *spec, int device, vlgba_scene_out *out);

#ifdef __cplusplus
}
#endif
#endif
```

Baseline: 2000 LM iterations/s.

## Fold final sum reduction into linearize kernel via last-block tickets; precompute chunk direct flags

```diff
diff --git a/bundleadjustmentmatlab_amd/_lib.py b/bundleadjustmentmatlab_amd/_lib.py
--- a/bundleadjustmentmatlab_amd/_lib.py
+++ b/bundleadjustmentmatlab_amd/_lib.py
@@ -105,6 +105,7 @@
     "vlgba_kernel_name": (ctypes.c_char_p, [c_int]),
     "vlgba_kernel_flops": (c_int, [ctypes.c_void_p, c_dp]),
     "vlgba_plan_info": (c_int, [ctypes.c_void_p, ctypes.POINTER(c_ll), c_int]),
+    "vlgba_get_launch_folds": (c_int, [ctypes.c_void_p, c_ip]),
     "vlgba_mex_bundle_1": (c_int, [c_int, c_int, c_int] + [c_dp] * 14),
     "vlgba_mex_bundle_2": (c_int, [c_int, c_int, c_int] + [c_dp] * 7),
     "vlgba_mex_bundle_3": (c_int, [c_int, c_int, c_int] + [c_dp] * 13),
diff --git a/bundleadjustmentmatlab_amd/bundle.py b/bundleadjustmentmatlab_amd/bundle.py
--- a/bundleadjustmentmatlab_amd/bundle.py
+++ b/bundleadjustmentmatlab_amd/bundle.py
@@ -445,7 +445,13 @@
         buf = (ctypes.c_longlong * n)()
         rc = self._L.vlgba_plan_info(self._h, buf, n)
         check(min(rc, 0), "vlgba_plan_info")
-        return dict(zip(self.PLAN_KEYS, [int(v) for v in buf]))
+        info = dict(zip(self.PLAN_KEYS, [int(v) for v in buf]))
+        fold = ctypes.c_int(0)
+        if hasattr(self._L, "vlgba_get_launch_folds"):
+            check(self._L.vlgba_get_launch_folds(self._h, ctypes.byref(fold)),
+                  "vlgba_get_launch_folds")
+        info["finalsum_fold"] = int(fold.value)
+        return info
 
     def phase_ms(self):
         ms = np.zeros(7)
diff --git a/bundleadjustmentmatlab_amd/csrc/ba_internal.h b/bundleadjustmentmatlab_amd/csrc/ba_internal.h
--- a/bundleadjustmentmatlab_amd/csrc/ba_internal.h
+++ b/bundleadjustmentmatlab_amd/csrc/ba_internal.h
@@ -79,6 +79,9 @@
     int dense_solve;
     int asm_direct;
     int camupd_fold;
+    int finalsum_fold;
+    unsigned *fin_cnt;
+    double *fin_wsum;
     double *part;
     double *scal;
     int ordered;
@@ -110,6 +113,7 @@
     unsigned *blob;
     int *ch_blob, *ch_obase;
     int *ch_cam;
+    unsigned char *ch_dir;
     unsigned char *obs_lpt;
     int max_blob;
     int ngrp_mf;
diff --git a/bundleadjustmentmatlab_amd/csrc/ba_kernels.hip b/bundleadjustmentmatlab_amd/csrc/ba_kernels.hip
--- a/bundleadjustmentmatlab_amd/csrc/ba_kernels.hip
+++ b/bundleadjustmentmatlab_amd/csrc/ba_kernels.hip
@@ -49,6 +49,25 @@
 
 typedef double v2d __attribute__((ext_vector_type(2)));
 
+typedef __attribute__((address_space(1))) unsigned long long ba_gu64;
+typedef __attribute__((address_space(1))) unsigned ba_gu32;
+template <bool SC> __device__ __forceinline__ double ldg(const double *p)
+{
+    if constexpr (SC)
+        return __builtin_bit_cast(
+            double, __hip_atomic_load((ba_gu64 *)p, __ATOMIC_RELAXED, __HIP_MEMORY_SCOPE_AGENT));
+    else
+        return *p;
+}
+template <bool SC> __device__ __forceinline__ void stg(double *p, double v)
+{
+    if constexpr (SC)
+        __hip_atomic_store((ba_gu64 *)p, __builtin_bit_cast(unsigned long long, v),
+                           __ATOMIC_RELAXED, __HIP_MEMORY_SCOPE_AGENT);
+    else
+        *p = v;
+}
+
 template <int BS>
 __device__ __forceinline__ void block_sum_to(double v, double *out)
 {
@@ -64,6 +83,119 @@
         for (int k = 1; k < BS / 64; k++) s += red[k];
         *out = s;
     }
+}
+
+struct ba_sum3 {
+    const double *part[3];
+    int n[3];
+    double *out[3];
+    const double *scal;
+    double *hres;
+    double seq;
+    unsigned *cnt;
+    const double *cam_da, *cam_eA;
+    double *cam_part;
+    int cam_m, cam_na;
+    double cam_lambda;
+};
+
+template <int L, bool SC>
+__device__ __forceinline__ double sum_strided_1024(const double *part, int nparts, int t)
+{
+    double v0 = 0.0, v1 = 0.0, v2 = 0.0, v3 = 0.0;
+    if constexpr (!SC) {
+        int q = t;
+        for (; q + 3 * 1024 < nparts; q += 4 * 1024) {
+            v0 += part[q];
+            v1 += part[q + 1024];
+            v2 += part[q + 2 * 1024];
+            v3 += part[q + 3 * 1024];
+        }
+        for (; q < nparts; q += 1024) v0 += part[q];
+    } else {
+        static_assert(L % 4 == 0, "a batch is whole rounds of the four accumulators");
+        const int J = t < nparts ? (nparts - t + 1023) >> 10 : 0;
+        const int J4 = J & ~3;
+        const int Jw = __builtin_amdgcn_readfirstlane(J);
+        const double *p0 = part + (J > 0 ? t : 0);
+        for (int j0 = 0; j0 < Jw; j0 += L) {
+            double x[L];
+#pragma unroll
+            for (int u = 0; u < L; u += 4) {
+                if (j0 + u < Jw) {
+#pragma unroll
+                    for (int k = 0; k < 4; k++)
+                        x[u + k] = ldg<true>(p0 + 1024 * max(min(j0 + u + k, J - 1), 0));
+                } else {
+#pragma unroll
+                    for (int k = 0; k < 4; k++) x[u + k] = 0.0;
+                }
+            }
+#pragma unroll
+            for (int u = 0; u < L; u += 4) {
+                const int j = j0 + u;
+                if (j < J4) {
+                    v0 += x[u];
+                    v1 += x[u + 1];
+                    v2 += x[u + 2];
+                    v3 += x[u + 3];
+                } else {
+                    if (j < J) v0 += x[u];
+                    if (j + 1 < J) v0 += x[u + 1];
+                    if (j + 2 < J) v0 += x[u + 2];
+                }
+            }
+        }
+    }
+    return (v0 + v1) + (v2 + v3);
+}
+
+template <int PBS, int L, bool SC>
+__device__ __forceinline__ double sum_parts_1024(const double *part, int nparts, double *red)
+{
+    static_assert(1024 % PBS == 0 && PBS % 64 == 0, "whole waves of the 1024");
+    const int lane = threadIdx.x & 63, wid = threadIdx.x >> 6;
+#pragma unroll 1
+    for (int k = 0; k < 1024 / PBS; k++) {
+        double v = sum_strided_1024<L, SC>(part, nparts, (int)threadIdx.x + PBS * k);
+#pragma unroll
+        for (int off = 32; off > 0; off >>= 1) v += __shfl_down(v, off, 64);
+        if (lane == 0) red[wid + PBS / 64 * k] = v;
+    }
+    __syncthreads();
+    double s = 0.0;
+    if (threadIdx.x == 0) {
+        s = red[0];
+#pragma unroll
+        for (int k = 1; k < 16; k++) s += red[k];
+    }
+    __syncthreads();
+    return s;
+}
+
+template <int PBS, int L, bool SC>
+__device__ __forceinline__ double sum3_block(const ba_sum3 &a, int b, double *red)
+{
+    const int nparts = a.n[b];
+    if (b == 2 && a.cam_da) {
+        const int lane = threadIdx.x & 63;
+        for (int g = threadIdx.x >> 6; g < nparts; g += PBS / 64) {
+            const int j = 64 * g + lane;
+            double acc = 0.0;
+            if (j < a.cam_m) {
+                for (int c = 0; c < a.cam_na; c++) {
+                    const double d = a.cam_da[(size_t)a.cam_na * j + c];
+                    acc += d * (a.cam_lambda * d + a.cam_eA[(size_t)a.cam_na * j + c]);
+                }
+            }
+#pragma unroll
+            for (int off = 32; off > 0; off >>= 1) acc += __shfl_down(acc, off, 64);
+            if (lane == 0) stg<SC>(a.cam_part + g, acc);
+        }
+        if constexpr (SC) asm volatile("s_waitcnt vmcnt(0)" ::: "memory");
+        __syncthreads();
+    }
+    return sum_parts_1024<PBS, L, SC>(a.part[b], nparts, red);
 }
 
 
@@ -248,6 +380,13 @@
 #define BA_LIN_CAMS 10
 #define BA_LIN_WAVES (BA_LIN_CAMS > 0 ? 6 : 7)
 
+struct ba_finfold {
+    ba_sum3 s;
+    unsigned *cnt;
+    double *wsum;
+    int nch;
+};
+
 struct ba_upd {
     const double *W_old, *da, *eB_old, *Vinv, *b_old;
     int ndb;
@@ -255,7 +394,86 @@
     double *db, *b_new, *part_dpg;
     const int *seg_long, *long_o0;
     const double *dpg_long;
+    ba_finfold fin;
 };
+
+#ifndef BA_FIN_LOADS
+#define BA_FIN_LOADS 24
+#endif
+
+__device__ __forceinline__ void final_sums_fold(const ba_finfold &f, int ch, unsigned tick,
+                                                double *red, int *flag)
+{
+    const int tid = threadIdx.x, lane = tid & 63;
+    const int w = (ch >> 6) & (BA_FIN_CLASSES - 1);
+    ba_gu32 *ct = (ba_gu32 *)f.cnt + BA_FIN_STRIDE * BA_FIN_CLASSES;
+    const unsigned top = (unsigned)BA_FIN_TOP(f.nch);
+    if (tid == 0) {
+        const int won = tick + 1u == (unsigned)BA_FIN_NEED(f.nch, w);
+        if (won)
+            __hip_atomic_store((ba_gu32 *)f.cnt + BA_FIN_STRIDE * w, 0u, __ATOMIC_RELAXED,
+                               __HIP_MEMORY_SCOPE_AGENT);
+        flag[0] = won;
+    }
+    __syncthreads();
+    if (!flag[0] && ch != 0) return;
+    int done = 0;
+    if (flag[0]) {
+        __builtin_amdgcn_fence(__ATOMIC_ACQUIRE, "agent");
+        if (tid < 128) {
+            const int b = tid >> 6;
+            double v = sum_strided_1024<BA_FIN_LOADS, true>(b ? f.s.part[1] : f.s.part[0], f.nch,
+                                                            64 * w + lane);
+#pragma unroll
+            for (int off = 32; off > 0; off >>= 1) v += __shfl_down(v, off, 64);
+            if (lane == 0) stg<true>(f.wsum + BA_FIN_CLASSES * b + w, v);
+            asm volatile("s_waitcnt vmcnt(0)" ::: "memory");
+        }
+        __syncthreads();
+        if (tid == 0)
+            done |= __hip_atomic_fetch_add(ct, 1u, __ATOMIC_RELAXED, __HIP_MEMORY_SCOPE_AGENT) +
+                        1u == top;
+    }
+    if (ch == 0) {
+        const double v = sum3_block<256, 4, false>(f.s, 2, red);
+        if (tid == 0) {
+            stg<true>(f.wsum + 2 * BA_FIN_CLASSES, v);
+            asm volatile("s_waitcnt vmcnt(0)" ::: "memory");
+            done |= __hip_atomic_fetch_add(ct, 1u, __ATOMIC_RELAXED, __HIP_MEMORY_SCOPE_AGENT) +
+                        1u == top;
+        }
+    }
+    if (tid == 0) flag[1] = done;
+    __syncthreads();
+    if (flag[1] && tid < 64) {
+        __builtin_amdgcn_fence(__ATOMIC_ACQUIRE, "agent");
+        const int ncl = (int)top - 1;
+        const bool have = lane < 2 * BA_FIN_CLASSES ? (lane & (BA_FIN_CLASSES - 1)) < ncl
+                                                    : lane == 2 * BA_FIN_CLASSES;
+        const double x = have ? ldg<true>(f.wsum + lane) : 0.0;
+        double s0 = __shfl(x, 0, 64), s1 = __shfl(x, BA_FIN_CLASSES, 64);
+#pragma unroll
+        for (int k = 1; k < BA_FIN_CLASSES; k++) {
+            s0 += __shfl(x, k, 64);
+            s1 += __shfl(x, BA_FIN_CLASSES + k, 64);
+        }
+        const double s2 = __shfl(x, 2 * BA_FIN_CLASSES, 64);
+        if (lane == 0) {
+            *f.s.out[0] = s0;
+            *f.s.out[1] = s1;
+            *f.s.out[2] = s2;
+            __hip_atomic_store(ct, 0u, __ATOMIC_RELAXED, __HIP_MEMORY_SCOPE_AGENT);
+            if (f.s.hres) {
+                const volatile double *sc = f.s.scal;
+#pragma unroll
+                for (int k = 0; k < 6; k++) f.s.hres[k] = sc[k];
+                __threadfence_system();
+                __atomic_store_n((unsigned long long *)(f.s.hres + 7),
+                                 __double_as_longlong(f.s.seq), __ATOMIC_RELEASE);
+            }
+        }
+    }
+}
 
 template <int NA, bool UPD, bool LOSS, bool JAC = false>
 __device__ __forceinline__ void linearize_chunk_body(
@@ -287,6 +505,8 @@
     __shared__ unsigned char wz[BA_CH_OBS];
     __shared__ double dpl[UPD ? BA_CH_PTS : 1];
     static_assert(BA_CH_PTS <= 64, "the point lanes are wave 0");
+    __shared__ double ssw[4];
+    __shared__ int fin_flag[2];
     constexpr int NCAMS = (NA == 6 && BA_LIN_CAMS > 0) ? BA_LIN_CAMS : 0;
     __shared__ __attribute__((aligned(16))) double camr[NCAMS > 0 ? 45 * NCAMS : 1];
     const int tid = threadIdx.x;
@@ -523,14 +743,31 @@
         }
     }
     if (tid < nu) eobl[tid] = (unsigned short)m_eobl;
+#pragma unroll
+    for (int off = 32; off > 0; off >>= 1) sse += __shfl_down(sse, off, 64);
+    if ((tid & 63) == 0) ssw[tid >> 6] = sse;
     __syncthreads();
     STAMP(17);
-    if constexpr (UPD) {
-        if (tid == 0) {
+    unsigned tick = 0;
+    if (tid == 0) {
+        const double s = ((ssw[0] + ssw[1]) + ssw[2]) + ssw[3];
+        if constexpr (UPD) {
             double acc = 0.0;
             const int k1 = seg ? 1 : np;
             for (int k = 0; k < k1; k++) acc += dpl[k];
-            u.part_dpg[ch] = acc;
+            if (u.fin.cnt) {
+                stg<true>(u.part_dpg + ch, acc);
+                stg<true>(part_sse + ch, s);
+                asm volatile("s_waitcnt vmcnt(0)" ::: "memory");
+                tick = __hip_atomic_fetch_add(
+                    (ba_gu32 *)u.fin.cnt + BA_FIN_STRIDE * ((ch >> 6) & (BA_FIN_CLASSES - 1)), 1u,
+                    __ATOMIC_RELAXED, __HIP_MEMORY_SCOPE_AGENT);
+            } else {
+                u.part_dpg[ch] = acc;
+                part_sse[ch] = s;
+            }
+        } else {
+            part_sse[ch] = s;
         }
     }
     if constexpr (NA % 2 == 0) {
@@ -609,7 +846,9 @@
         upart[(size_t)(NU + NA) * (e0 + s) + l] = acc;
     }
     STAMP(20);
-    block_sum_to<256>(sse, part_sse + ch);
+    if constexpr (UPD) {
+        if (u.fin.cnt) final_sums_fold(u.fin, ch, tick, rows, fin_flag);
+    }
     STAMP(21);
 #ifdef BA_STAMPS
     if (tid == 0) atomicAdd(&g_stamp[22], 1ull);
@@ -1151,6 +1390,9 @@
     return __builtin_bit_cast(double, r);
 }
 #define BA_MF_WAVES 3
+#ifndef BA_MF_DIRECT_SETUP
+#define BA_MF_DIRECT_SETUP 1
+#endif
 template <int NA>
 __global__ __launch_bounds__(256, (NA == 6) ? BA_MF_WAVES : 1) void k_schur_mfma(
     const int *__restrict__ grp_ch, const int *__restrict__ grp_gs,
@@ -1159,7 +1401,8 @@
     const unsigned *__restrict__ blob, const double *__restrict__ W,
     double *Vinv, const double *__restrict__ eB, int nobs_all, int n_all,
     int gcap, int ecap, double *__restrict__ spart, double *__restrict__ epart, int ngrp,
-    ba_camred cred, const double *__restrict__ Vdamp, double lambda)
+    ba_camred cred, const double *__restrict__ Vdamp, double lambda,
+    const unsigned char *__restrict__ ch_dir)
 {
     if ((int)blockIdx.x >= ngrp) {
         camera_reduce_wg<NA>((int)blockIdx.x - ngrp, cred);
@@ -1186,6 +1429,15 @@
     for (int q = tid; q < ngs * NA * NA; q += 256) gacc[q] = 0.0;
     for (int q = tid; q < nge * NA; q += 256) geacc[q] = 0.0;
     for (int q = tid; q < nrw; q += 256) rec[q] = blob[rb0 + q];
+#if BA_MF_DIRECT_SETUP
+    for (int q = tid; q <= nc; q += 256) {
+        const int i0 = ch_pt[c0 + q], bo = ch_blob[c0 + q] - rb0;
+        const int np = q < nc ? ch_pt[c0 + q + 1] - i0 : 0;
+        const int hw = q < nc ? (int)(blob[rb0 + bo + 1] & 0xffffu) | (int)ch_dir[c0 + q] << 24 : 0;
+        chd[q] = int4{i0, ch_obase[c0 + q], bo, np << 16 | hw};
+    }
+    __syncthreads();
+#else
     for (int q = tid; q <= nc; q += 256) {
         const int i0 = ch_pt[c0 + q], bo = ch_blob[c0 + q] - rb0;
         const int np = q < nc ? ch_pt[c0 + q + 1] - i0 : 0;
@@ -1207,6 +1459,7 @@
         chd[q].w |= (int)(h1 & 0xffffu) | (bad ? 0 : 1 << 24);
     }
     __syncthreads();
+#endif
     int ccs[RT], crr[RT];
 #pragma unroll
     for (int t = 0; t < RT; t++) {
@@ -2147,51 +2400,11 @@
     }
 }
 
-struct ba_sum3 {
-    const double *part[3];
-    int n[3];
-    double *out[3];
-    const double *scal;
-    double *hres;
-    double seq;
-    unsigned *cnt;
-    const double *cam_da, *cam_eA;
-    double *cam_part;
-    int cam_m, cam_na;
-    double cam_lambda;
-};
-
 __global__ __launch_bounds__(1024) void k_sum_parts3(ba_sum3 a)
 {
-    const double *part = a.part[blockIdx.x];
-    const int nparts = a.n[blockIdx.x];
-    if (blockIdx.x == 2 && a.cam_da) {
-        const int lane = threadIdx.x & 63;
-        for (int g = threadIdx.x >> 6; g < nparts; g += 16) {
-            const int j = 64 * g + lane;
-            double acc = 0.0;
-            if (j < a.cam_m) {
-                for (int c = 0; c < a.cam_na; c++) {
-                    const double d = a.cam_da[(size_t)a.cam_na * j + c];
-                    acc += d * (a.cam_lambda * d + a.cam_eA[(size_t)a.cam_na * j + c]);
-                }
-            }
-#pragma unroll
-            for (int off = 32; off > 0; off >>= 1) acc += __shfl_down(acc, off, 64);
-            if (lane == 0) a.cam_part[g] = acc;
-        }
-        __syncthreads();
-    }
-    double v0 = 0.0, v1 = 0.0, v2 = 0.0, v3 = 0.0;
-    int q = threadIdx.x;
-    for (; q + 3 * 1024 < nparts; q += 4 * 1024) {
-        v0 += part[q];
-        v1 += part[q + 1024];
-        v2 += part[q + 2 * 1024];
-        v3 += part[q + 3 * 1024];
-    }
-    for (; q < nparts; q += 1024) v0 += part[q];
-    block_sum_to<1024>((v0 + v1) + (v2 + v3), a.out[blockIdx.x]);
+    __shared__ double red[16];
+    const double s = sum3_block<1024, 4, false>(a, (int)blockIdx.x, red);
+    if (threadIdx.x == 0) *a.out[blockIdx.x] = s;
     if (a.hres && threadIdx.x == 0) {
         __threadfence();
         if (atomicAdd(a.cnt, 1u) == 2u) {
@@ -2360,7 +2573,8 @@
         k_schur_mfma<NA><<<d->ngrp_mf + ncr, 256, sm2, d->stream>>>(
             d->grp_ch, d->grp_gs, d->grp_ge, d->ch_pt, d->ch_obase, d->ch_blob, d->blob, d->W,
             d->Vinv, d->eB, d->N, d->n, d->mf_max_s, d->mf_max_e, d->spart, d->epart,
-            d->ngrp_mf, fold ? *fold : ba_camred{}, d->vinv_fold ? d->V : nullptr, lambda);
+            d->ngrp_mf, fold ? *fold : ba_camred{}, d->vinv_fold ? d->V : nullptr, lambda,
+            d->ch_dir);
         KT_E(d, KT_SCHUR_MF);
     }
     if (d->ngrp > d->ngrp_mf) {
@@ -2490,8 +2704,8 @@
     return 0;
 }
 
-static int launch_final_sums(ba_dev *d, const double *sse_part, const double *dpg_part, int gc,
-                             double lam_dpg, bool folded, bool publish)
+static ba_sum3 final_sums_args(ba_dev *d, const double *sse_part, const double *dpg_part, int gc,
+                               double lam_dpg, bool folded, bool publish)
 {
     ba_sum3 s3 = {{sse_part, dpg_part, d->part},
                   {d->nch, d->nch, gc},
@@ -2510,7 +2724,14 @@
         s3.hres = d->hres_dev;
         s3.seq = (double)d->seq;
     }
-    k_sum_parts3<<<3, 1024, 0, d->stream>>>(s3);
+    return s3;
+}
+
+static int launch_final_sums(ba_dev *d, const double *sse_part, const double *dpg_part, int gc,
+                             double lam_dpg, bool folded, bool publish)
+{
+    k_sum_parts3<<<3, 1024, 0, d->stream>>>(
+        final_sums_args(d, sse_part, dpg_part, gc, lam_dpg, folded, publish));
     return -(int)hipGetLastError();
 }
 
@@ -2527,14 +2748,20 @@
     if (d->fused) {
         KT_B(d);
         TRY_RC(launch_long_db(d, lambda));
-        const ba_upd u{d->W, d->da, d->eB, d->Vinv, d->b, d->ndb, lambda, d->db, d->b_new,
-                       d->chsse2 + 2 * (size_t)d->nch, d->seg_long, d->long_o0, d->dpg_long};
+        ba_upd u{d->W, d->da, d->eB, d->Vinv, d->b, d->ndb, lambda, d->db, d->b_new,
+                 d->chsse2 + 2 * (size_t)d->nch, d->seg_long, d->long_o0, d->dpg_long};
+        const bool fin = d->finalsum_fold && publish;
+        if (fin)
+            u.fin = ba_finfold{final_sums_args(d, d->chsse2, d->chsse2 + 2 * (size_t)d->nch, gc,
+                                               lam_dpg, folded, publish),
+                               d->fin_cnt, d->fin_wsum, d->nch};
         BA_DISPATCH(d->na, (lin_chunk_launch<NA>(d, f, d->a_new, d->rot_new, d->b_new, d->W2,
                                                  d->V2, d->eB2, d->upart2, d->chsse2, &u)));
         if (d->nl > 0)
             k_long_vsum<<<d->nl, 64, 0, d->stream>>>(d->long_pt, d->long_seg0, d->vseg, d->V2,
                                                      d->eB2);
         KT_E(d, KT_LIN_UPD);
+        if (fin) return -(int)hipGetLastError();
         return launch_final_sums(d, d->chsse2, d->chsse2 + 2 * (size_t)d->nch, gc, lam_dpg,
                                  folded, publish);
     }
diff --git a/bundleadjustmentmatlab_amd/csrc/ba_limits.h b/bundleadjustmentmatlab_amd/csrc/ba_limits.h
--- a/bundleadjustmentmatlab_amd/csrc/ba_limits.h
+++ b/bundleadjustmentmatlab_amd/csrc/ba_limits.h
@@ -24,6 +24,13 @@
 #define BA_MF_CMAX(na) ((16 * BA_MF_RT(na)) / (na))
 #define BA_MF_GACC 1536
 #define BA_MF_GE_CAP 24
+#define BA_FIN_CLASSES 16
+#define BA_FIN_STRIDE 16
+#define BA_FIN_REM(nch, w) ((nch) % 1024 - 64 * (w))
+#define BA_FIN_NEED(nch, w) \
+    ((nch) / 1024 * 64 +    \
+     (BA_FIN_REM(nch, w) < 0 ? 0 : BA_FIN_REM(nch, w) > 64 ? 64 : BA_FIN_REM(nch, w)))
+#define BA_FIN_TOP(nch) ((((nch) + 63) / 64 < BA_FIN_CLASSES ? ((nch) + 63) / 64 : BA_FIN_CLASSES) + 1)
 #define BA_LONG_OBS 65535
 #define BA_LONG_TERMS (1LL << 26)
 #define BA_LCAM_LDS 256
diff --git a/bundleadjustmentmatlab_amd/csrc/ba_plan.cpp b/bundleadjustmentmatlab_amd/csrc/ba_plan.cpp
--- a/bundleadjustmentmatlab_amd/csrc/ba_plan.cpp
+++ b/bundleadjustmentmatlab_amd/csrc/ba_plan.cpp
@@ -942,3 +942,26 @@
         ccam[2 * ch + 1] = hi < 0 ? 0 : hi;
     }
 }
+
+void plan_final_tickets(int nch, std::vector<int> &need)
+{
+    need.clear();
+    for (int w = 0; w < BA_FIN_CLASSES; w++) need.push_back(BA_FIN_NEED(nch, w));
+    need.push_back(BA_FIN_TOP(nch));
+}
+
+void plan_chunk_direct(const host_plan &plan, std::vector<unsigned char> &dir)
+{
+    const size_t nchk = plan.ch_blob.empty() ? 0 : plan.ch_blob.size() - 1;
+    dir.assign(std::max<size_t>(nchk, 1), 0);
+    for (int ch = 0; ch < plan.nch_mf; ch++) {
+        if (plan.ch_pt[ch + 1] - plan.ch_pt[ch] != BA_MF_PTS) continue;
+        const unsigned *r = plan.blob.data() + plan.ch_blob[ch];
+        const int C = (int)(r[1] & 0xffu);
+        const unsigned *tw = r + 2 + C + C * (C + 1) / 2;
+        unsigned bad = 0u;
+        for (int w = 0; w < BA_MF_PTS / 4 * C; w++)
+            bad |= tw[w] ^ (0x03020100u + 0x04040404u * (unsigned)w);
+        dir[ch] = bad ? 0 : 1;
+    }
+}
diff --git a/bundleadjustmentmatlab_amd/csrc/ba_plan.h b/bundleadjustmentmatlab_amd/csrc/ba_plan.h
--- a/bundleadjustmentmatlab_amd/csrc/ba_plan.h
+++ b/bundleadjustmentmatlab_amd/csrc/ba_plan.h
@@ -108,5 +108,7 @@
                           std::vector<unsigned char> &lpt);
 void plan_chunk_cameras(const host_plan &plan, const std::vector<int> &lcam,
                         std::vector<int> &ccam);
+void plan_chunk_direct(const host_plan &plan, std::vector<unsigned char> &dir);
+void plan_final_tickets(int nch, std::vector<int> &need);
 
 #pragma GCC visibility pop
diff --git a/bundleadjustmentmatlab_amd/csrc/ba_solver.cpp b/bundleadjustmentmatlab_amd/csrc/ba_solver.cpp
--- a/bundleadjustmentmatlab_amd/csrc/ba_solver.cpp
+++ b/bundleadjustmentmatlab_amd/csrc/ba_solver.cpp
@@ -559,6 +559,9 @@
                 ccam[2 * ch + 1] = ccam[2 * ch] + (1 << 20);
         pb.add(&d.obs_lpt, lpt);
         pb.add(&d.ch_cam, ccam);
+        std::vector<unsigned char> cdir;
+        plan_chunk_direct(plan, cdir);
+        pb.add(&d.ch_dir, cdir);
         d.grp_max_s = plan.grp_max_s;
         d.grp_max_e = plan.grp_max_e;
         d.ngs = (int)plan.gslot_blk.size();
@@ -686,6 +689,15 @@
     VLGBA_CHECK(hipMemsetAsync(d.scal, 0, 8 * sizeof(double), s));
     TRY(ctx_alloc(c, &d.pub_cnt, 1));
     VLGBA_CHECK(hipMemsetAsync(d.pub_cnt, 0, sizeof(unsigned), s));
+    const char *ff = std::getenv("VLGBA_FINALSUM_FOLD");
+    d.finalsum_fold = (ff && ff[0] == '1') && fast && !d.ordered && d.fused && d.nch > 0 &&
+                      d.nl == 0 && c->world == 1 && !c->comm;
+    if (d.finalsum_fold) {
+        const size_t nw = (size_t)BA_FIN_STRIDE * (BA_FIN_CLASSES + 1);
+        TRY(ctx_alloc(c, &d.fin_cnt, nw));
+        VLGBA_CHECK(hipMemsetAsync(d.fin_cnt, 0, sizeof(unsigned) * nw, s));
+        TRY(ctx_alloc(c, &d.fin_wsum, 2 * BA_FIN_CLASSES + 8));
+    }
     VLGBA_CHECK(hipStreamSynchronize(s));
     return 0;
 }
@@ -1955,6 +1967,13 @@
     return VLGBA_NPLAN;
 }
 
+int vlgba_get_launch_folds(vlgba_ctx *c, int *finalsum_fold)
+{
+    if (!c) return VLGBA_E_ARG;
+    if (finalsum_fold) *finalsum_fold = c->d.finalsum_fold;
+    return 0;
+}
+
 int vlgba_phase_ms(vlgba_ctx *c, double *ms7)
 {
     if (!c || !ms7) return VLGBA_E_ARG;
diff --git a/include/vlgba.h b/include/vlgba.h
--- a/include/vlgba.h
+++ b/include/vlgba.h
@@ -126,6 +126,7 @@
 const char *vlgba_kernel_name(int k);
 #define VLGBA_NPLAN 33
 int vlgba_plan_info(vlgba_ctx *ctx, long long *info, int len);
+int vlgba_get_launch_folds(vlgba_ctx *ctx, int *finalsum_fold);
 
 
 int vlgba_mex_bundle_1(int m, int n, int num_a, const double *K, const double *a,
```

After: 1996 LM iterations/s. No clear change (-0.2%).
